# wolearyc/ramannoodle

Hardware: AMD Instinct MI355X
Metric: structures/sec (GNN polarizability eval) (higher is better)
Workload: dtype f32

## Files before the change

include/rn_potgnn.h:

```cpp
#ifndef RN_POTGNN_H
#define RN_POTGNN_H

#include <stddef.h>
#include <stdint.h>

#ifdef __cplusplus
extern "C" {
#endif

typedef enum rn_status {
  RN_OK = 0,
  RN_ERR_INVALID_ARGUMENT = -1,
  RN_ERR_UNSUPPORTED = -2,
  RN_ERR_NO_DEVICE = -3,
  RN_ERR_HIP = -4,
  RN_ERR_OUT_OF_MEMORY = -5
} rn_status;

typedef struct rn_potgnn rn_potgnn;

typedef struct rn_potgnn_config {
  int32_t num_atoms;
  int32_t num_edges;
  int32_t num_atom_types;
// ... 106 lines not shown
int rn_potgnn_gradient_buffer(rn_potgnn *h, void **device_ptr, size_t *count);
int rn_potgnn_adam_step(rn_potgnn *h, double lr, double beta1, double beta2, double eps,
                        double weight_decay, int64_t step);
int rn_potgnn_get_weights(rn_potgnn *h, float *weights, size_t num_weights);

int rn_potgnn_train_forward_f64(rn_potgnn *h, const double *positions, int64_t S, double *vec6,
                                double *batch_mean, double *batch_var);
int rn_potgnn_train_backward_f64(rn_potgnn *h, const double *dvec6, double *grads);

typedef int (*rn_potgnn_reduce_fn)(double *values, int64_t count, void *ctx);
int rn_potgnn_set_stat_reducer(rn_potgnn *h, rn_potgnn_reduce_fn fn, void *ctx);
double rn_potgnn_train_row_count(const rn_potgnn *h);


int rn_md_raman_intensities(const double *alpha, int64_t S, int device, double *intensities,
                            int64_t num_bins);
int rn_md_raman_intensities_device(const double *d_alpha, int64_t S, int device, double *intensities,
                                   int64_t num_bins, void *stream);

int rn_md_raman_polarized(const double *alpha, int64_t S, const double *weights, int64_t K, int device,
                          size_t workspace_limit, double *intensities, int64_t num_bins);
int rn_md_raman_polarized_device(const double *d_alpha, int64_t S, const double *weights, int64_t K, int device,
                                 size_t workspace_limit, double *intensities, int64_t num_bins, void *stream);

int rn_md_raman_partial(const double *increments, int64_t N, int G, const double *weights, int64_t K, int device,
                        size_t workspace_limit, double *intensities, int64_t num_bins);
int rn_md_raman_partial_device(const double *d_increments, int64_t N, int G, const double *weights, int64_t K,
                               int device, size_t workspace_limit, double *intensities, int64_t num_bins, void *stream);

int rn_md_raman_segments(const double *alpha, int64_t S, int64_t segment_steps, int64_t hop, const double *taper,
                         const double *weights, int64_t K, int average, int device, size_t workspace_limit,
                         double *intensities, int64_t num_bins);
int rn_md_raman_segments_device(const double *d_alpha, int64_t S, int64_t segment_steps, int64_t hop, const double *taper,
                                const double *weights, int64_t K, int average, int device, size_t workspace_limit,
                                double *intensities, int64_t num_bins, void *stream);

int rn_md_raman_segments_at(const double *alpha, int64_t S, int64_t segment_steps, const int64_t *starts, int64_t Q,
                            const double *taper, const double *weights, int64_t K, int average, int device,
                            size_t workspace_limit, double *intensities, int64_t num_bins);
int rn_md_raman_segments_at_device(const double *d_alpha, int64_t S, int64_t segment_steps, const int64_t *starts,
                                   int64_t Q, const double *taper, const double *weights, int64_t K, int average,
                                   int device, size_t workspace_limit, double *intensities, int64_t num_bins,
                                   void *stream);

int rn_md_raman_partial_segments(const double *increments, int64_t N, int G, int64_t segment_steps,
                                 const int64_t *starts, int64_t Q, const double *taper, const double *weights,
                                 int64_t K, int average, int device, size_t workspace_limit, double *intensities,
                                 int64_t num_bins);
int rn_md_raman_partial_segments_device(const double *d_increments, int64_t N, int G, int64_t segment_steps,
                                        const int64_t *starts, int64_t Q, const double *taper, const double *weights,
                                        int64_t K, int average, int device, size_t workspace_limit,
                                        double *intensities, int64_t num_bins, void *stream);

int rn_md_vdos(const double *positions, const double *lattices, int64_t num_lattices, int64_t S, int32_t N,
               const double *masses, const int32_t *labels, int G, int64_t segment_steps, const int64_t *starts,
               int64_t Q, const double *taper, int average, int device, size_t workspace_limit, double *densities,
               int64_t num_bins);
int rn_md_vdos_device(const double *d_positions, const double *d_lattices, int64_t num_lattices, int64_t S, int32_t N,
                      const double *masses, const int32_t *labels, int G, int64_t segment_steps, const int64_t *starts,
                      int64_t Q, const double *taper, int average, int device, size_t workspace_limit,
                      double *densities, int64_t num_bins, void *stream);
int rn_md_vdos_set_profiling(int enabled);
int rn_md_vdos_phase_times(double *millis);

int rn_md_mode_vdos(const double *positions, const double *lattices, int64_t num_lattices, int64_t S, int32_t N,
                    const double *masses, const double *vectors, int32_t M, int64_t segment_steps,
                    const int64_t *starts, int64_t Q, const double *taper, int average, int device,
                    size_t workspace_limit, double *densities, int64_t num_bins);
int rn_md_mode_vdos_device(const double *d_positions, const double *d_lattices, int64_t num_lattices, int64_t S,
                           int32_t N, const double *masses, const double *vectors, int32_t M, int64_t segment_steps,
                           const int64_t *starts, int64_t Q, const double *taper, int average, int device,
                           size_t workspace_limit, double *densities, int64_t num_bins, void *stream);
int rn_md_mode_vdos_set_profiling(int enabled);
int rn_md_mode_vdos_phase_times(double *millis);

int rn_potgnn_config_flags(const rn_potgnn *h);

int rn_potgnn_debug_ps_schedule(const int32_t *rb, const int32_t *re, int32_t num_destinations, int32_t back,
                                int32_t ring_tiles, int32_t *window);

int rn_potgnn_debug_plan(const rn_potgnn_config *cfg, const int32_t *edge_a, const int32_t *edge_b,
                         const int32_t *atom_types, int32_t num_cus, int32_t *out, size_t capacity, size_t *count);

int rn_potgnn_debug_plan_lds(const rn_potgnn_config *cfg, const int32_t *edge_a, const int32_t *edge_b,
                             const int32_t *atom_types, int32_t num_cus, int64_t *out, size_t capacity, size_t *count);

int rn_potgnn_debug_pack_weights(const rn_potgnn_config *cfg, const float *weights, size_t num_weights, float *packed,
                                 unsigned char *mask, unsigned char *writers, int32_t *flags, size_t capacity, size_t *count);

int rn_potgnn_debug_unpack_weights(const rn_potgnn_config *cfg, const float *packed, size_t num_packed, int buffers,
                                   float *out, size_t capacity, size_t *count);

int64_t rn_potgnn_num_triplets(const rn_potgnn *h);

int rn_potgnn_debug_triplets(rn_potgnn *h, int32_t *idx_i, int32_t *idx_j,
                             int32_t *idx_k, int32_t *slot5, int32_t *slot6);

int rn_potgnn_debug_stage(rn_potgnn *h, int stage, int index, float *out,
                          size_t out_capacity, int64_t *rows, int64_t *cols);

int rn_potgnn_set_profiling(rn_potgnn *h, int enabled);
int rn_potgnn_kernel_times(rn_potgnn *h, const char **names, double *millis,
                           int64_t *launches, int cap);

const char *rn_potgnn_last_error(const rn_potgnn *h);
const char *rn_potgnn_version(void);

#ifdef __cplusplus
}
#endif
#endif
```

ramannoodle_amd/_lib.py:

```python
from __future__ import annotations

import ctypes as C
import os

from ramannoodle_amd.exceptions import DeviceError

_LIB_PATH = os.environ.get(
    "RN_POTGNN_LIB", os.path.join(os.path.dirname(os.path.abspath(__file__)), "librn_potgnn.so"))

RN_OK = 0
RN_ERR_INVALID_ARGUMENT = -1
RN_ERR_UNSUPPORTED = -2
RN_ERR_NO_DEVICE = -3
RN_ERR_HIP = -4
RN_ERR_OUT_OF_MEMORY = -5


class Config(C.Structure):

    _fields_ = [
        ("num_atoms", C.c_int32),
        ("num_edges", C.c_int32),
        ("num_atom_types", C.c_int32),
        ("size_node_embedding", C.c_int32),
        ("size_edge_embedding", C.c_int32),
        ("num_message_passes", C.c_int32),
        ("gauss_coefficient", C.c_double),
        ("max_chunk_structures", C.c_int32),
        ("device", C.c_int32),
    ]


_P = C.c_void_p
SIGNATURES = {
    "rn_potgnn_radius_graph": (C.c_int, [_P, _P, C.c_int32, C.c_double, C.c_int, _P]),
    "rn_potgnn_config_flags": (C.c_int, [_P]),
    "rn_potgnn_set_stat_reducer": (C.c_int, [_P, _P, _P]),
    "rn_potgnn_train_row_count": (C.c_double, [_P]),
    "rn_potgnn_weight_count": (C.c_size_t, [C.POINTER(Config)]),
    "rn_potgnn_create": (C.c_int, [C.POINTER(Config), _P, _P, _P, _P, _P, C.c_size_t, _P, _P,
                                   C.POINTER(_P)]),
    "rn_potgnn_destroy": (None, [_P]),
    "rn_potgnn_calc_polarizabilities": (C.c_int, [_P, _P, C.c_int64, _P]),
    "rn_potgnn_calc_polarizabilities_f64": (C.c_int, [_P, _P, C.c_int64, _P]),
    "rn_potgnn_calc_polarizabilities_to_device": (C.c_int, [_P, _P, C.c_int64, _P, _P]),
    "rn_potgnn_calc_polarizabilities_cells": (C.c_int, [_P, _P, _P, C.c_int64, C.c_int, _P]),
    "rn_potgnn_calc_polarizabilities_cells_to_device": (C.c_int, [_P, _P, _P, C.c_int64, _P, _P]),
    "rn_potgnn_forward_cells_device": (C.c_int, [_P, _P, _P, C.c_int64, C.c_int, _P, _P, C.c_int]),
    "rn_potgnn_forward_device": (C.c_int, [_P, _P, C.c_int64, _P, _P, _P, C.c_int]),
    "rn_potgnn_forward_device_f64": (C.c_int, [_P, _P, C.c_int64, _P, _P, C.c_int]),
    "rn_potgnn_calc_polarizabilities_async": (C.c_int, [_P, _P, C.c_int64, _P]),
    "rn_potgnn_wait": (C.c_int, [_P]),
    "rn_host_buffer_alloc": (C.c_int, [C.c_size_t, C.c_int, C.POINTER(_P)]),
    "rn_host_buffer_free": (None, [_P]),
    "rn_potgnn_forward": (C.c_int, [_P, _P, C.c_int64, _P]),
    "rn_potgnn_forward_lattices": (C.c_int, [_P, _P, _P, C.c_int64, _P]),
    "rn_potgnn_forward_samples": (C.c_int, [_P, _P, _P, _P, C.c_int64, _P]),
    "rn_potgnn_forward_samples_f64": (C.c_int, [_P, _P, _P, _P, C.c_int64, _P]),
    "rn_potgnn_raman_tensors": (C.c_int, [_P, _P, _P, C.c_int64, C.c_double, _P]),
    "rn_potgnn_alpha_jacobian": (C.c_int, [_P, _P, C.c_int, _P]),
    "rn_potgnn_raman_tensors_analytic": (C.c_int, [_P, _P, _P, C.c_int64, _P]),
    "rn_potgnn_set_weights": (C.c_int, [_P, _P, C.c_size_t]),
    "rn_potgnn_train_forward": (C.c_int, [_P, _P, C.c_int64, _P, _P, _P]),
    "rn_potgnn_train_backward": (C.c_int, [_P, _P, _P]),
    "rn_potgnn_set_device_training": (C.c_int, [_P, C.c_int]),
    "rn_potgnn_train_backward_device": (C.c_int, [_P, _P]),
    "rn_potgnn_gradient_buffer": (C.c_int, [_P, C.POINTER(_P), C.POINTER(C.c_size_t)]),
    "rn_potgnn_adam_step": (C.c_int, [_P, C.c_double, C.c_double, C.c_double, C.c_double, C.c_double, C.c_int64]),
    "rn_potgnn_get_weights": (C.c_int, [_P, _P, C.c_size_t]),
    "rn_potgnn_train_forward_f64": (C.c_int, [_P, _P, C.c_int64, _P, _P, _P]),
    "rn_potgnn_train_forward_samples": (C.c_int, [_P, _P, _P, _P, C.c_int64, _P, _P, _P]),
    "rn_potgnn_train_forward_samples_f64": (C.c_int, [_P, _P, _P, _P, C.c_int64, _P, _P, _P]),
    "rn_potgnn_forward_samples_device": (C.c_int, [_P, _P, _P, _P, C.c_int64, _P, _P, C.c_int]),
    "rn_potgnn_train_forward_samples_device": (C.c_int, [_P, _P, _P, _P, C.c_int64, _P, _P]),
    "rn_potgnn_train_backward_samples_device": (C.c_int, [_P, _P, _P]),
    "rn_potgnn_train_backward_f64": (C.c_int, [_P, _P, _P]),
    "rn_potgnn_forward_vjp_device": (C.c_int, [_P, _P, _P, _P, C.c_int64, _P, C.c_int, _P, _P, _P]),
    "rn_potgnn_group_increments_device": (C.c_int, [_P, _P, C.c_int64, _P, C.c_int, C.c_int, C.c_size_t, _P, _P]),
    "rn_potgnn_group_increments_cells_device": (C.c_int, [_P, _P, _P, C.c_int64, _P, C.c_int, C.c_int, C.c_size_t, _P,
                                                          _P]),
    "rn_potgnn_partial_raman_tensors": (C.c_int, [_P, _P, _P, C.c_int64, _P, C.c_int, _P]),
    "rn_potgnn_train_backward_inputs": (C.c_int, [_P, _P, _P, _P, _P]),
    "rn_potgnn_train_backward_inputs_device": (C.c_int, [_P, _P, _P, _P, _P]),
    "rn_potgnn_num_triplets": (C.c_int64, [_P]),
    "rn_potgnn_debug_triplets": (C.c_int, [_P, _P, _P, _P, _P, _P]),
    "rn_potgnn_debug_ps_schedule": (C.c_int, [_P, _P, C.c_int32, C.c_int32, C.c_int32, _P]),
    "rn_potgnn_debug_plan": (C.c_int, [C.POINTER(Config), _P, _P, _P, C.c_int32, _P, C.c_size_t, C.POINTER(C.c_size_t)]),
    "rn_potgnn_debug_plan_lds": (C.c_int, [C.POINTER(Config), _P, _P, _P, C.c_int32, _P, C.c_size_t, C.POINTER(C.c_size_t)]),
    "rn_potgnn_debug_pack_weights": (C.c_int, [C.POINTER(Config), _P, C.c_size_t, _P, _P, _P, _P, C.c_size_t, C.POINTER(C.c_size_t)]),
    "rn_potgnn_debug_unpack_weights": (C.c_int, [C.POINTER(Config), _P, C.c_size_t, C.c_int, _P, C.c_size_t, C.POINTER(C.c_size_t)]),
    "rn_potgnn_debug_stage": (C.c_int, [_P, C.c_int, C.c_int, _P, C.c_size_t,
                                        C.POINTER(C.c_int64), C.POINTER(C.c_int64)]),
    "rn_potgnn_set_profiling": (C.c_int, [_P, C.c_int]),
    "rn_potgnn_kernel_times": (C.c_int, [_P, C.POINTER(C.c_char_p), C.POINTER(C.c_double),
                                         C.POINTER(C.c_int64), C.c_int]),
    "rn_potgnn_last_error": (C.c_char_p, [_P]),
    "rn_potgnn_version": (C.c_char_p, []),
    "rn_md_raman_intensities": (C.c_int, [_P, C.c_int64, C.c_int, _P, C.c_int64]),
    "rn_md_raman_intensities_device": (C.c_int, [_P, C.c_int64, C.c_int, _P, C.c_int64, _P]),
    "rn_md_raman_polarized": (C.c_int, [_P, C.c_int64, _P, C.c_int64, C.c_int, C.c_size_t, _P, C.c_int64]),
    "rn_md_raman_polarized_device": (C.c_int, [_P, C.c_int64, _P, C.c_int64, C.c_int, C.c_size_t, _P, C.c_int64,
                                               _P]),
    "rn_md_raman_partial": (C.c_int, [_P, C.c_int64, C.c_int, _P, C.c_int64, C.c_int, C.c_size_t, _P, C.c_int64]),
    "rn_md_raman_partial_device": (C.c_int, [_P, C.c_int64, C.c_int, _P, C.c_int64, C.c_int, C.c_size_t, _P,
                                             C.c_int64, _P]),
    "rn_md_raman_segments": (C.c_int, [_P, C.c_int64, C.c_int64, C.c_int64, _P, _P, C.c_int64, C.c_int, C.c_int,
                                       C.c_size_t, _P, C.c_int64]),
    "rn_md_raman_segments_device": (C.c_int, [_P, C.c_int64, C.c_int64, C.c_int64, _P, _P, C.c_int64, C.c_int, C.c_int,
                                              C.c_size_t, _P, C.c_int64, _P]),
    "rn_md_raman_segments_at": (C.c_int, [_P, C.c_int64, C.c_int64, _P, C.c_int64, _P, _P, C.c_int64, C.c_int, C.c_int,
                                          C.c_size_t, _P, C.c_int64]),
    "rn_md_raman_segments_at_device": (C.c_int, [_P, C.c_int64, C.c_int64, _P, C.c_int64, _P, _P, C.c_int64, C.c_int,
                                                 C.c_int, C.c_size_t, _P, C.c_int64, _P]),
    "rn_md_raman_partial_segments": (C.c_int, [_P, C.c_int64, C.c_int, C.c_int64, _P, C.c_int64, _P, _P, C.c_int64,
                                               C.c_int, C.c_int, C.c_size_t, _P, C.c_int64]),
    "rn_md_raman_partial_segments_device": (C.c_int, [_P, C.c_int64, C.c_int, C.c_int64, _P, C.c_int64, _P, _P,
                                                      C.c_int64, C.c_int, C.c_int, C.c_size_t, _P, C.c_int64, _P]),
    "rn_md_vdos": (C.c_int, [_P, _P, C.c_int64, C.c_int64, C.c_int32, _P, _P, C.c_int, C.c_int64, _P, C.c_int64, _P,
                             C.c_int, C.c_int, C.c_size_t, _P, C.c_int64]),
    "rn_md_vdos_device": (C.c_int, [_P, _P, C.c_int64, C.c_int64, C.c_int32, _P, _P, C.c_int, C.c_int64, _P, C.c_int64,
                                    _P, C.c_int, C.c_int, C.c_size_t, _P, C.c_int64, _P]),
    "rn_md_vdos_set_profiling": (C.c_int, [C.c_int]),
    "rn_md_vdos_phase_times": (C.c_int, [_P]),
    "rn_md_mode_vdos": (C.c_int, [_P, _P, C.c_int64, C.c_int64, C.c_int32, _P, _P, C.c_int32, C.c_int64, _P, C.c_int64,
                                  _P, C.c_int, C.c_int, C.c_size_t, _P, C.c_int64]),
    "rn_md_mode_vdos_device": (C.c_int, [_P, _P, C.c_int64, C.c_int64, C.c_int32, _P, _P, C.c_int32, C.c_int64, _P,
                                         C.c_int64, _P, C.c_int, C.c_int, C.c_size_t, _P, C.c_int64, _P]),
    "rn_md_mode_vdos_set_profiling": (C.c_int, [C.c_int]),
    "rn_md_mode_vdos_phase_times": (C.c_int, [_P]),
    "rn_xdatcar_open": (C.c_int, [C.c_char_p, C.POINTER(_P)]),
    "rn_xdatcar_close": (None, [_P]),
    "rn_xdatcar_info": (C.c_int, [_P, C.POINTER(C.c_int64), C.POINTER(C.c_int32), _P, C.POINTER(C.c_int32)]),
    "rn_xdatcar_species": (C.c_int, [_P, C.c_int32, C.c_char_p, C.POINTER(C.c_int32)]),
    "rn_xdatcar_read": (C.c_int, [_P, C.c_int64, C.c_int64, _P, _P, C.c_int]),
    "rn_xdatcar_variable_cell": (C.c_int, [_P]),
    "rn_xdatcar_read_lattices": (C.c_int, [_P, C.c_int64, C.c_int64, _P]),
    "rn_xdatcar_last_error": (C.c_char_p, [_P]),
    "rn_vasprun_open": (C.c_int, [C.c_char_p, C.POINTER(_P)]),
    "rn_vasprun_close": (None, [_P]),
    "rn_vasprun_info": (C.c_int, [_P, C.POINTER(C.c_int64), C.POINTER(C.c_int32)]),
    "rn_vasprun_read": (C.c_int, [_P, C.c_int64, C.c_int64, _P, C.c_int]),
    "rn_vasprun_timestep": (C.c_int, [_P, C.POINTER(C.c_double)]),
    "rn_vasprun_initial_num_atoms": (C.c_int64, [_P]),
    "rn_vasprun_initial_structure": (C.c_int, [_P, C.POINTER(C.c_int32), _P, _P, C.c_int64, _P, C.c_int64]),
    "rn_vasprun_last_error": (C.c_char_p, [_P]),
}

_lib = None


def library_path() -> str:
    return _LIB_PATH


def load() -> C.CDLL:
    global _lib
    if _lib is not None:
        return _lib
    if not os.path.exists(_LIB_PATH):
        raise DeviceError(
            f"{_LIB_PATH} not found: build it with ramannoodle_amd/csrc/build.sh "
            "(there is no CPU fallback for the PotGNN evaluation path)"
        )
    try:
        lib = C.CDLL(_LIB_PATH)
    except OSError as exc:
        raise DeviceError(f"cannot load {_LIB_PATH}: {exc}") from exc
    for name, (restype, argtypes) in SIGNATURES.items():
        fn = getattr(lib, name)
        fn.restype = restype
# ... 19 lines not shown
```

ramannoodle_amd/csrc/api.hip:

```cpp
#include <hip/hip_runtime.h>

#include <algorithm>
#include <chrono>
#include <cmath>
#include <cstdarg>
#include <cstdio>
#include <cstdlib>
#include <cstring>
#include <functional>
#include <memory>
#include <mutex>
#include <string>
#include <thread>
#include <vector>

#include "../../include/rn_potgnn.h"
#include "graph_plan.hpp"
#include "kernels.hpp"
#include "weight_layout.hpp"

using namespace rn;

namespace {

std::string g_create_error;

struct HipError {
  hipError_t code;
  const char *what;
};

#define HIP_TRY(expr)                                  \
  do {                                                 \
    hipError_t _e = (expr);                            \
    if (_e != hipSuccess) throw HipError{_e, #expr};   \
  } while (0)

struct DeviceBuf {
  void *p = nullptr;
  size_t bytes = 0;
  ~DeviceBuf() { release(); }
  void release() {
    if (p) (void)hipFree(p);
    p = nullptr;
    bytes = 0;
  }
  void ensure(size_t n) {
    if (n <= bytes) return;
    release();
    HIP_TRY(hipMalloc(&p, n));
    bytes = n;
  }
  template <typename T>
  T *as() const { return reinterpret_cast<T *>(p); }
};

enum KernelId {
  K_GEOM = 0, K_NODE_INIT, K_PROJ_NODE, K_PROJ_EDGE_C1, K_NODE_AGG, K_PROJ_EDGE_C3, K_PROJ_C2,
  K_EDGE_AGG, K_READOUT_MLP, K_READOUT_REDUCE, K_COUNT
};
const char *kKernelNames[K_COUNT] = {
    "geom_rbf", "node_init", "proj_node", "proj_edge_c1", "node_agg", "proj_edge_c3",
    "proj_c2", "edge_agg", "readout_mlp", "readout_reduce"};

template <typename T>
struct Lane {
  hipStream_t stream = nullptr;
  hipEvent_t done = nullptr;
  DeviceBuf unit4, node[2], edge[2], npc1, np3, bufA, bufB;
  DeviceBuf fbA, fbB;
};

template <typename T>
struct Precision {
  bool ready = false;
  DeviceBuf weights;
  DeviceBuf lattice;
  std::vector<PassW<T>> pass;
  ReadoutW<T> ro{};
  const T *offsets = nullptr, *node_table = nullptr, *ones = nullptr;
  Lane<T> lanes[2];
  std::vector<DeviceBuf> snap_node, snap_edge;
  std::vector<DeviceBuf> tape_node, tape_edge, tape_agg;
  DeviceBuf bw[18];
  hipStream_t side = nullptr;
  hipEvent_t ev_side[3] = {nullptr, nullptr, nullptr};
  DeviceBuf tn_arena;
  DeviceBuf tape_z1, bn_stats, grad, seeds, mv, type_sums;
  DeviceBuf in_dcart, in_lat, in_grads;
  DeviceBuf eye_seeds;
  int eye_frames = 0;
  bool tape_on = false;
};

struct TimedLaunch {
  int kid;
  hipEvent_t a, b;
};

}

struct rn_potgnn {
  mutable std::recursive_mutex lock;
  rn_potgnn_config cfg{};
  Dims d{};
  int chunk = 1;
  size_t f64_budget = 0;
  bool keep_stages = false;
  bool debug_sync = false;
  GraphPlan plan;
  bool split_projections = true;
  bool want_pair_rows = true;
  DeviceBuf step_seg, step_stage;
  float *step_host = nullptr;
  bool tape_ps = true;
  bool mfma_f16 = true;
  bool mfma_f16_requested = true;
  bool mfma_range_fallback = false;
  Graph g{};
  DeviceBuf g_ints;
  DeviceBuf ps_fail;
  double lattice[9], mean[9], stdv[9];
  DeviceBuf d_mean_std;
  std::vector<float> packed;
  PackedLayout lay;
  Precision<float> f32;
  Precision<double> f64;
  DeviceBuf io_pos, io_alpha, io_vec6, io_lat, io_types;
  struct Slot {
    DeviceBuf pos, alpha;
    hipEvent_t copied = nullptr, done = nullptr;
    bool busy = false;
  } slots[2];
  hipStream_t copy_stream = nullptr, exec_stream = nullptr;
  int next_slot = 0;
  struct HostStage {
    float *pin[2] = {nullptr, nullptr};
    size_t elems = 0;
    hipEvent_t copied[2] = {nullptr, nullptr};
    hipEvent_t done = nullptr;
    DeviceBuf pos;
    DeviceBuf lat;
    hipEvent_t caller = nullptr;
    char *out_pin = nullptr;
    size_t out_bytes = 0;
  } hstage;
  int last_chunk_structs = 0;
  int train_S = 0;
  int train_prec = 4;
  bool train_lat = false, train_types = false;
  bool tape_fused = true;
  bool device_training = false;
  bool grads_on_device = false;
  bool host_stale = false;
  DeviceBuf adam_m, adam_v, trainable_mask, derived_ops;
  int num_derived_ops = 0, derived_first_stage = 0;
  double bn_count = 0;
  rn_potgnn_reduce_fn reducer = nullptr;
  void *reducer_ctx = nullptr;
  bool last_was_f64 = false;
  bool last_in_order = false;
  int profiling = 0;
  std::vector<TimedLaunch> timed;
  double k_ms[K_COUNT] = {0};
  int64_t k_launches[K_COUNT] = {0};
  std::string error;
  hipEvent_t ev_start = nullptr;
  hipEvent_t ev_g[2] = {nullptr, nullptr};
  bool interleave = true;
  std::vector<int32_t> grp_labels;
  int grp_G = 0;
  DeviceBuf grp_csr, grp_jac, grp_disp, grp_out;
  DeviceBuf grp_jl, grp_lat, cells_lat;
};

namespace {

void set_error(rn_potgnn *h, const char *fmt, ...) {
  char buf[512];
  va_list ap;
  va_start(ap, fmt);
  vsnprintf(buf, sizeof(buf), fmt, ap);
  va_end(ap);
  if (h) {
    std::lock_guard<std::recursive_mutex> hold(h->lock);
    h->error = buf;
  } else {
    g_create_error = buf;
  }
}

bool lean_workspace(const rn_potgnn *h);
size_t per_structure_elems(const rn_potgnn *h, bool lean);
template <typename T>
int chunk_frames(const rn_potgnn *h) {
  if (sizeof(T) == 4) return h->chunk;
  const size_t budget = std::max(h->f64_budget, (size_t)h->chunk * per_structure_elems(h, lean_workspace(h)) * sizeof(float));
  const size_t per64 = per_structure_elems(h, false) * sizeof(double);
  return (int)std::max<size_t>(1, std::min<size_t>((size_t)h->chunk, budget / std::max<size_t>(per64, 1)));
}

template <typename T>
Precision<T> &prec(rn_potgnn *h);
template <>
Precision<float> &prec<float>(rn_potgnn *h) { return h->f32; }
template <>
Precision<double> &prec<double>(rn_potgnn *h) { return h->f64; }

void reduce_over_ranks(rn_potgnn *h, double *dev, size_t n, hipStream_t st) {
  if (!h->reducer) return;
  std::vector<double> host(n);
  HIP_TRY(hipStreamSynchronize(st));
  HIP_TRY(hipMemcpy(host.data(), dev, n * sizeof(double), hipMemcpyDeviceToHost));
  if (h->reducer(host.data(), (int64_t)n, h->reducer_ctx) != 0)
    throw HipError{hipErrorUnknown, "the statistics reducer (data-parallel training) failed"};
  HIP_TRY(hipMemcpy(dev, host.data(), n * sizeof(double), hipMemcpyHostToDevice));
}

bool lean_workspace(const rn_potgnn *h) {
  return (h->plan.use_fused && h->plan.use_node_fused && h->plan.use_readout_fused) || h->plan.use_narrow;
}
size_t bufA_width(const rn_potgnn *h, bool lean) {
  return lean ? 32 : std::max<size_t>(std::max(2 * h->d.FnP, 2 * h->d.FeP), 32);
}
size_t per_structure_elems(const rn_potgnn *h, bool lean) {
  const size_t N = h->cfg.num_atoms, E = h->cfg.num_edges;
  const size_t FnP = h->d.FnP, FeP = h->d.FeP;
  return E * 4 + 2 * N * FnP + 2 * E * FeP + N * 2 * FnP + N * 6 * FeP + E * bufA_width(h, lean) +
         (lean ? 0 : E * 4 * FeP);
}

void refresh_mfma_mode(rn_potgnn *h) {
  const bool ok = mfma_f16_range_ok(h->lay, h->packed.data(), h->host_stale);
  h->mfma_f16 = h->mfma_f16_requested && ok;
  h->mfma_range_fallback = h->mfma_f16_requested && !ok;
}

template <typename T>
void refresh_pass_flags(rn_potgnn *h) {
  Precision<T> &P = prec<T>(h);
  const bool off = getenv("RN_POTGNN_NO_FASTG") && atoi(getenv("RN_POTGNN_NO_FASTG")) != 0;
  for (size_t p = 0; p < h->lay.pass.size() && p < P.pass.size(); ++p) {
    const bool ok = !off && folded_gate_ok(h->lay, h->packed.data(), (int)p);
    P.pass[p].c3_fast = ok ? (h->plan.num_lanes == 1 ? 3 : 1) : 0;
  }
}

template <typename T>
T *stage(DeviceBuf &buf, const void *host, size_t bytes) {
  buf.ensure(bytes);
  HIP_TRY(hipMemcpy(buf.p, host, bytes, hipMemcpyHostToDevice));
  return buf.as<T>();
}

template <typename T>
T *upload_packed(rn_potgnn *h) {
  const std::vector<T> host(h->packed.begin(), h->packed.end());
  return stage<T>(prec<T>(h).weights, host.data(), host.size() * sizeof(T));
}

template <typename T>
void device_setup(rn_potgnn *h, T *w, hipStream_t st) {
  const PackedLayout &L = h->lay;
  launch_setup<T>(w + L.emb, w + L.W2, w + L.b2, w + L.W4, w + L.b4, h->cfg.num_atom_types, h->d,
                  w + L.node_table, w + L.b0, w + L.bn_w, w + L.bn_b, w + L.bn_rm, w + L.bn_rv,
                  w + L.scale0, w + L.shift0, st);
}

template <typename T>
void upload_weights(rn_potgnn *h) {
  Precision<T> &P = prec<T>(h);
  device_setup<T>(h, upload_packed<T>(h), P.lanes[0].stream);
  HIP_TRY(hipGetLastError());
  HIP_TRY(hipStreamSynchronize(P.lanes[0].stream));
  refresh_pass_flags<T>(h);
}

template <typename T>
void ensure_precision(rn_potgnn *h) {
  Precision<T> &P = prec<T>(h);
  if (P.ready) return;
  const PackedLayout &L = h->lay;
  T *w = upload_packed<T>(h);
  T lat[9];
  for (int i = 0; i < 9; ++i) lat[i] = (T)h->lattice[i];
  stage<T>(P.lattice, lat, sizeof(lat));
  WeightViews<T> v = bind_weights<T>(L, w);
  P.pass = std::move(v.pass);
  refresh_pass_flags<T>(h);
  P.ro = v.ro;
  P.offsets = v.offsets;
  P.node_table = v.node_table;
  P.ones = v.ones;

  const size_t N = h->cfg.num_atoms, E = h->cfg.num_edges, S = chunk_frames<T>(h);
  const size_t FnP = h->d.FnP, FeP = h->d.FeP;
  const bool lean = sizeof(T) == 4 && lean_workspace(h);
  const size_t bufA = bufA_width(h, lean);
  for (int l = 0; l < h->plan.num_lanes; ++l) {
    Lane<T> &ln = P.lanes[l];
    HIP_TRY(hipStreamCreateWithFlags(&ln.stream, hipStreamNonBlocking));
    HIP_TRY(hipEventCreateWithFlags(&ln.done, hipEventDisableTiming));
    ln.unit4.ensure(S * E * 4 * sizeof(T));
    for (int i = 0; i < 2; ++i) {
      ln.node[i].ensure(S * N * FnP * sizeof(T));
      ln.edge[i].ensure(S * E * FeP * sizeof(T));
    }
    ln.npc1.ensure(S * N * 2 * FnP * sizeof(T));
    ln.np3.ensure(S * N * 6 * FeP * sizeof(T));
    ln.bufA.ensure(S * E * bufA * sizeof(T));
    if (!lean) ln.bufB.ensure(S * E * 4 * FeP * sizeof(T));
  }
  if (h->keep_stages) {
    const int np = h->cfg.num_message_passes + 1;
    P.snap_node.resize(np);
    P.snap_edge.resize(np);
    for (int i = 0; i < np; ++i) {
      P.snap_node[i].ensure(S * N * FnP * sizeof(T));
      P.snap_edge[i].ensure(S * E * FeP * sizeof(T));
    }
  }
  device_setup<T>(h, w, P.lanes[0].stream);
  HIP_TRY(hipGetLastError());
  HIP_TRY(hipStreamSynchronize(P.lanes[0].stream));
  P.ready = true;
}

struct Timer {
  rn_potgnn *h;
  hipStream_t st;
  int kid;
  hipEvent_t a = nullptr, b = nullptr;
  bool on;
  Timer(rn_potgnn *h_, hipStream_t st_, int kid_) : h(h_), st(st_), kid(kid_) {
    on = h->profiling == 1 || (h->profiling >= 100 && h->profiling < 1000 && h->profiling - 100 == kid) ||
         (h->profiling >= 1000 && (((h->profiling - 1000) >> kid) & 1));
    if (on) {
      HIP_TRY(hipEventCreate(&a));
      HIP_TRY(hipEventCreate(&b));
      HIP_TRY(hipEventRecord(a, st));
    }
  }
  ~Timer() noexcept(false) {
    if (on) {
      (void)hipEventRecord(b, st);
      h->timed.push_back({kid, a, b});
    }
    if (h->debug_sync) {
      hipError_t e = hipGetLastError();
      if (e == hipSuccess) e = hipStreamSynchronize(st);
      if (e != hipSuccess) throw HipError{e, kKernelNames[kid]};
    }
  }
};

void resolve_timers(rn_potgnn *h) {
  for (auto &t : h->timed) {
    float ms = 0;
    if (hipEventSynchronize(t.b) == hipSuccess && hipEventElapsedTime(&ms, t.a, t.b) == hipSuccess) {
      h->k_ms[t.kid] += ms;
      h->k_launches[t.kid] += 1;
    }
    (void)hipEventDestroy(t.a);
    (void)hipEventDestroy(t.b);
  }
  h->timed.clear();
}

template <typename T>
struct ForwardIO {
  const double *pos = nullptr;
  const float *pos32 = nullptr;
  double *alpha = nullptr;
  float *vec6 = nullptr;
  double *alpha_raw = nullptr;
  const T *lat = nullptr;
  const int *types = nullptr;
  ForwardIO at(int64_t first, int N) const {
    auto from = [first](auto *p, int64_t stride) { return p ? p + first * stride : nullptr; };
    ForwardIO o;
    o.pos = from(pos, 3 * (int64_t)N);
    o.pos32 = from(pos32, 3 * (int64_t)N);
    o.alpha = from(alpha, 9);
    o.vec6 = from(vec6, 6);
    o.alpha_raw = from(alpha_raw, 9);
    o.lat = from(lat, 9);
    o.types = from(types, N);
    return o;
  }
};

template <typename T>
struct ChunkRun {
  rn_potgnn *h;
  Lane<T> *ln;
  ForwardIO<T> io;
  int S;
  int cur = 0;
  T *node[2], *edge[2], *unit4, *npc1, *np3, *bufA, *bufB;
  int64_t MN, ME;

  ChunkRun(rn_potgnn *h_, Lane<T> &l, const ForwardIO<T> &io_, int S_) : h(h_), ln(&l), io(io_), S(S_) {
    node[0] = l.node[0].template as<T>();
    node[1] = l.node[1].template as<T>();
    edge[0] = l.edge[0].template as<T>();
    edge[1] = l.edge[1].template as<T>();
    unit4 = l.unit4.template as<T>();
    npc1 = l.npc1.template as<T>();
    np3 = l.np3.template as<T>();
    bufA = l.bufA.template as<T>();
    bufB = l.bufB.template as<T>();
    MN = (int64_t)S * h->g.N;
    ME = (int64_t)S * h->g.E;
  }
  hipStream_t st() const { return ln->stream; }
  void target_tape(int slot, int which) {
    Precision<T> &P = prec<T>(h);
    if (!P.tape_on) return;
    node[which] = P.tape_node[slot].template as<T>();
    edge[which] = P.tape_edge[slot].template as<T>();
  }
  void snapshot(int p) {
    Precision<T> &P = prec<T>(h);
    if (!h->keep_stages) return;
    HIP_TRY(hipMemcpyAsync(P.snap_node[p].p, node[cur], (size_t)MN * h->d.FnP * sizeof(T),
                           hipMemcpyDeviceToDevice, st()));
    HIP_TRY(hipMemcpyAsync(P.snap_edge[p].p, edge[cur], (size_t)ME * h->d.FeP * sizeof(T),
                           hipMemcpyDeviceToDevice, st()));
  }

  void begin() {
    Precision<T> &P = prec<T>(h);
    target_tape(0, 0);
    {
      Timer t(h, st(), K_GEOM);
      bool done = false;
      const T *lat = io.lat ? io.lat : P.lattice.template as<T>();
      const int lat_stride = io.lat ? 9 : 0;
      const T gauss = (T)h->cfg.gauss_coefficient;
      if constexpr (sizeof(T) == 4) {
        if (io.pos32) {
          if (pair_rows()) launch_geom_rbf_pairs_pos32(io.pos32, S, h->g, lat, lat_stride, P.offsets, gauss, h->d, unit4, edge[0], st());
          else launch_geom_rbf_pos32(io.pos32, S, h->g, lat, lat_stride, P.offsets, gauss, h->d, unit4, edge[0], st(), narrow());
          done = true;
        } else if (pair_rows()) {
          launch_geom_rbf_pairs(io.pos, S, h->g, lat, lat_stride, P.offsets, gauss, h->d, unit4, edge[0], st());
          done = true;
        }
      }
      if (!done) launch_geom_rbf<T>(io.pos, S, h->g, lat, lat_stride, P.offsets, gauss, h->d, unit4, edge[0], st(), narrow());
      h->last_in_order = narrow();
    }
    {
      Timer t(h, st(), K_NODE_INIT);
      launch_node_init<T>(P.node_table, S, h->g, h->d, node[0], io.types, st());
    }
    cur = 0;
    snapshot(0);
  }

  void run_stages() {
    begin();
    for (int p = 0; p < h->cfg.num_message_passes; ++p) {
      stage_project(p);
      stage_aggregate(p);
    }
  }

  void project(const T *X, int64_t R, int K, const T *WT, int NOUT, T *Y, const T *bias, int amode, const T *nd) {
    if constexpr (sizeof(T) == 4) {
      if (h->mfma_f16 && h->split_projections &&
          launch_rowgemm_split(X, K, K, R, WT, NOUT, Y, false, bias, amode, nd, h->g, st()))
        return;
    }
    launch_rowgemm<T>(X, R, K, WT, NOUT, Y, nullptr, bias, false, amode, nd, h->g, st());
  }

  void stage_project(int p) {
    const PassW<T> &w = prec<T>(h).pass[p];
    const Graph &g = h->g;
    const Dims d = h->d;
    const int nxt = cur ^ 1;
    target_tape(p + 1, nxt);
    if constexpr (sizeof(T) == 4) {
      if (narrow()) {
        Timer t(h, st(), K_NODE_AGG);
        launch_node_narrow(edge[cur], node[cur], node[nxt], S, g, d, w, st());
        return;
      }
    }
    {
      Timer t(h, st(), K_PROJ_NODE);
      if (node_centred()) project(node[cur], MN, d.FnP, w.c1_WnT_c, 2 * d.FnP, npc1, w.c1_bias_c, 0, nullptr);
      else project(node[cur], MN, d.FnP, w.c1_WnT, 2 * d.FnP, npc1, w.c1_bias, 0, nullptr);
    }
    bool node_fused = false;
    if constexpr (sizeof(T) == 4) {
      if (fused() && h->plan.use_node_fused) {
        Timer t(h, st(), K_NODE_AGG);
        if (node_centred() && g.na_num > 0) launch_node_atom(edge[cur], node[cur], npc1, node[nxt], S, g, d, w, st(), pair_rows());
        else launch_node_fused(edge[cur], node[cur], npc1, node[nxt], S, g, d, w, h->mfma_f16, node_centred(), st());
        node_fused = true;
      }
    }
    if (!node_fused) {
      {
        Timer t(h, st(), K_PROJ_EDGE_C1);
        project(edge[cur], ME, d.FeP, w.c1_WeT, 2 * d.FnP, bufA, nullptr, 0, nullptr);
      }
      {
        Timer t(h, st(), K_NODE_AGG);
        launch_node_agg<T>(npc1, bufA, node[cur], node[nxt], S, g, d, w, st());
      }
    }
    {
      Timer t(h, st(), K_PROJ_NODE);
      if (role_split(w)) project(node[nxt], MN, d.FnP, w.c3_WnT_c, 6 * d.FeP, np3, w.c3_nshift_c, 0, nullptr);
      else project(node[nxt], MN, d.FnP, w.c3_WnT, 6 * d.FeP, np3, w.c3_nshift, 0, nullptr);
    }
    if (!fused()) {
      {
        Timer t(h, st(), K_PROJ_EDGE_C3);
        project(edge[cur], ME, d.FeP, w.c3_WeT, 4 * d.FeP, bufB, nullptr, 0, nullptr);
      }
      {
        Timer t(h, st(), K_PROJ_C2);
        project(nullptr, ME, d.FnP, w.c2_WT, 2 * d.FeP, bufA, w.c2_bias, 1, node[nxt]);
      }
    }
  }

  void stage_aggregate(int p) {
    const PassW<T> &w = prec<T>(h).pass[p];
    const int nxt = cur ^ 1;
    {
      Timer t(h, st(), K_EDGE_AGG);
      if constexpr (sizeof(T) == 4) {
        if (narrow()) launch_edge_narrow(edge[cur], edge[nxt], node[nxt], S, h->g, h->d, w, st());
        else if (role_split(w)) launch_edge_ps(edge[cur], edge[nxt], node[nxt], np3, tape_agg(p), S, h->g, h->d, w, h->ps_fail.as<int>(), st(), pair_rows(), h->mfma_f16);
        else if (fused()) edge_unfused_in_blocks(p);
        else HIP_TRY(launch_edge_agg<T>(bufB, np3, bufA, edge[cur], edge[nxt], S, h->g, h->d, w, tape_agg(p), st()));
      } else {
        HIP_TRY(launch_edge_agg<T>(bufB, np3, bufA, edge[cur], edge[nxt], S, h->g, h->d, w, tape_agg(p), st()));
      }
    }
    cur = nxt;
    snapshot(p + 1);
  }

  void edge_unfused_in_blocks(int p) {
    const PassW<T> &w = prec<T>(h).pass[p];
    const Graph &g = h->g;
    const Dims d = h->d;
    const int nxt = cur ^ 1;
    const size_t per_frame = (size_t)g.E * (size_t)(6 * d.FeP) * sizeof(T);
    int block = (int)std::max<size_t>(1, std::min<size_t>((size_t)S, ((size_t)1 << 30) / std::max<size_t>(per_frame, 1)));
    if (const char *e = getenv("RN_POTGNN_UNFUSED_BLOCK_FRAMES")) block = std::max(1, std::min(block, atoi(e)));
    ln->fbA.ensure((size_t)block * g.E * 2 * d.FeP * sizeof(T));
    ln->fbB.ensure((size_t)block * g.E * 4 * d.FeP * sizeof(T));
    T *fa = ln->fbA.template as<T>(), *fb = ln->fbB.template as<T>();
    T *agg = tape_agg(p);
    for (int s0 = 0; s0 < S; s0 += block) {
      const int sb = std::min(block, S - s0);
      const int64_t rows = (int64_t)sb * g.E;
      const T *e_in = edge[cur] + (size_t)s0 * g.E * d.FeP, *nd = node[nxt] + (size_t)s0 * g.N * d.FnP;
      project(e_in, rows, d.FeP, w.c3_WeT, 4 * d.FeP, fb, nullptr, 0, nullptr);
      project(nullptr, rows, d.FnP, w.c2_WT, 2 * d.FeP, fa, w.c2_bias, 1, nd);
      HIP_TRY(launch_edge_agg<T>(fb, np3 + (size_t)s0 * g.N * 6 * d.FeP, fa, e_in, edge[nxt] + (size_t)s0 * g.E * d.FeP, sb, g, d, w,
                                 agg ? agg + (size_t)s0 * g.E * d.FeP : nullptr, st()));
    }
  }

  void finish() {
    Precision<T> &P = prec<T>(h);
    const Graph &g = h->g;
    const Dims d = h->d;
    if constexpr (sizeof(T) == 4) {
      if (narrow()) {
        Timer t(h, st(), K_READOUT_MLP);
        const double *ms = h->d_mean_std.as<double>();
        launch_readout_narrow(edge[cur], unit4, S, g, d, P.ro, ms, ms + 9, io.vec6, io.alpha, io.alpha_raw,
                              h->keep_stages ? bufA : nullptr, st());
        HIP_TRY(hipGetLastError());
        return;
      }
    }
    int pol_stride = 32;
    {
      Timer t(h, st(), K_READOUT_MLP);
      const int HP = std::max(d.FeP, 32);
      bool done = false;
      if constexpr (sizeof(T) == 4) {
        if (fused() && h->plan.use_readout_fused) {
          pol_stride = h->keep_stages ? 32 : 16;
          launch_readout_fused(edge[cur], ME, P.ro, bufA, h->mfma_f16, st(), pair_rows(), pol_stride);
          done = true;
        }
      }
      if (!done) {
        launch_rowgemm<T>(edge[cur], ME, d.FeP, P.ro.W0T, HP, bufA, P.ro.scale0, P.ro.shift0, true, 0,
                          nullptr, g, st());
        launch_rowgemm<T>(bufA, ME, HP, P.ro.W3T, HP, bufB, P.ones, P.ro.b3, true, 0, nullptr, g, st());
        launch_rowgemm<T>(bufB, ME, HP, P.ro.W5T, 32, bufA, nullptr, P.ro.b5, false, 0, nullptr, g,
                          st());
      }
    }
    {
      Timer t(h, st(), K_READOUT_REDUCE);
      const double *ms = h->d_mean_std.as<double>();
      launch_readout_reduce<T>(bufA, unit4, S, g, ms, ms + 9, io.vec6, io.alpha, io.alpha_raw, st(), pol_stride);
    }
    HIP_TRY(hipGetLastError());
  }
  bool fused() const { return sizeof(T) == 4 && h->plan.use_fused && (!prec<T>(h).tape_on || h->tape_fused); }
  bool narrow() const { return sizeof(T) == 4 && h->plan.use_narrow && !prec<T>(h).tape_on; }
  bool node_centred() const {
    static const bool on = !(getenv("RN_POTGNN_NODE_CENTRED") && atoi(getenv("RN_POTGNN_NODE_CENTRED")) == 0);
    return sizeof(T) == 4 && on && fused() && h->plan.use_node_fused && h->mfma_f16 && (!prec<T>(h).tape_on || h->tape_ps);
  }
  bool role_split(const PassW<T> &w) const {
    return sizeof(T) == 4 && fused() && h->plan.use_ps && (w.c3_fast & 1) != 0 && (!prec<T>(h).tape_on || h->tape_ps);
  }
  bool pair_rows() const {
    if (sizeof(T) != 4 || !h->want_pair_rows || h->keep_stages || prec<T>(h).tape_on || !node_centred() || h->g.na_num <= 0 || !h->plan.use_readout_fused) return false;
    for (const auto &w : prec<T>(h).pass)
      if (!role_split(w)) return false;
    return true;
  }
  T *tape_agg(int p) {
    Precision<T> &P = prec<T>(h);
    return P.tape_on ? P.tape_agg[p].template as<T>() : nullptr;
  }
};

template <typename T>
void run_chunk(ChunkRun<T> c) {
  c.run_stages();
  c.finish();
}

template <typename T>
void run_pair(rn_potgnn *h, ChunkRun<T> &a, ChunkRun<T> &b) {
  const int P = h->cfg.num_message_passes;
  a.begin();
  b.begin();
  for (int p = 0; p < P; ++p) {
    if (p > 0) HIP_TRY(hipStreamWaitEvent(a.st(), h->ev_g[1], 0));
    a.stage_project(p);
    HIP_TRY(hipEventRecord(h->ev_g[0], a.st()));
    a.stage_aggregate(p);
    HIP_TRY(hipStreamWaitEvent(b.st(), h->ev_g[0], 0));
    b.stage_project(p);
    HIP_TRY(hipEventRecord(h->ev_g[1], b.st()));
    b.stage_aggregate(p);
  }
  a.finish();
  b.finish();
}

void check_ps_fail(rn_potgnn *h) {
  if (!h->plan.use_ps || !h->ps_fail.p) return;
  int fail = 0;
  HIP_TRY(hipMemcpy(&fail, h->ps_fail.p, sizeof(int), hipMemcpyDeviceToHost));
#ifdef RN_PS_TIMING
  {
    long long t[40];
    HIP_TRY(hipMemcpy(t, (const char *)h->ps_fail.p + 64, sizeof(t), hipMemcpyDeviceToHost));
    HIP_TRY(hipMemset((char *)h->ps_fail.p + 64, 0, sizeof(t)));
    static const char *names[20] = {"P sched+dma_wait", "P loads+split", "P split sync", "P seeds", "P request", "P guard",
                                    "P P'+c2", "P Q' (product, loads landed + finish)", "P norm sync+publish", "P ring guard", "C ready wait", "C prologue", "C loop",
                                    "C epilogue+done", "", "", "C(set B) ready wait", "C(set B) prologue", "C(set B) loop", "C(set B) epilogue+done"};
    for (int i = 0; i < 20; ++i)
      if (t[2 * i + 1]) fprintf(stderr, "[ps timing] %-22s %10.1f cycles x %lld\n", names[i], (double)t[2 * i] / (double)t[2 * i + 1], t[2 * i + 1]);
  }
#endif
#ifdef RN_PS_GRAM_DEBUG
  {
    int cnt = 0;
    HIP_TRY(hipMemcpy(&cnt, (const char *)h->ps_fail.p + 127 * 4, sizeof(int), hipMemcpyDeviceToHost));
    float dbg[144];
    HIP_TRY(hipMemcpy(dbg, (const char *)h->ps_fail.p + 128 * 4, sizeof(dbg), hipMemcpyDeviceToHost));
    fprintf(stderr, "[gram debug] %d mismatches\n", cnt);
    for (int k = 0; k < std::min(cnt, 12); ++k)
      fprintf(stderr, "  ref %g tab %g parts %g %g %g %g  d %g er %g tl %g urow %g r %g gr %g\n", dbg[12 * k], dbg[12 * k + 1], dbg[12 * k + 2],
              dbg[12 * k + 3], dbg[12 * k + 4], dbg[12 * k + 5], dbg[12 * k + 6], dbg[12 * k + 7], dbg[12 * k + 8], dbg[12 * k + 9],
              dbg[12 * k + 10], dbg[12 * k + 11]);
    HIP_TRY(hipMemset((char *)h->ps_fail.p + 127 * 4, 0, 4 + sizeof(dbg)));
  }
#endif
  if (fail == 0) return;
  HIP_TRY(hipMemset(h->ps_fail.p, 0, sizeof(int)));
  static const char *const which[7] = {
      "role-specialised EdgeBlock: a wait between producer and consumer waves timed out",
      "role-specialised EdgeBlock: the producers' split sync timed out",
      "role-specialised EdgeBlock: a producer's wait for the consumers to take the rows of an earlier round timed out",
      "role-specialised EdgeBlock: a producer's wait for the consumers to finish an earlier round (ring rows) timed out",
      "role-specialised EdgeBlock: a consumer's wait for its round timed out",
      "role-specialised EdgeBlock: a wait between producer and consumer waves timed out",
      "role-specialised EdgeBlock: a consumer's round-ordered wait before releasing its ring rows (c_rd) timed out"};
  throw HipError{hipErrorLaunchFailure, which[fail >= 0 && fail <= 6 ? fail : 0]};
}

template <typename T>
void behind_caller(rn_potgnn *h, hipStream_t user, Lane<T> *lanes, int n) {
  HIP_TRY(hipEventRecord(h->ev_start, user));
  for (int l = 0; l < n; ++l) HIP_TRY(hipStreamWaitEvent(lanes[l].stream, h->ev_start, 0));
}
template <typename T>
void hand_back(rn_potgnn *h, hipStream_t user, Lane<T> *lanes, int n, bool sync, bool timers = false) {
  for (int l = 0; l < n; ++l) {
    HIP_TRY(hipEventRecord(lanes[l].done, lanes[l].stream));
    HIP_TRY(hipStreamWaitEvent(user, lanes[l].done, 0));
  }
  if (!sync) return;
  HIP_TRY(hipStreamSynchronize(user));
  if (timers) resolve_timers(h);
  check_ps_fail(h);
}

template <typename T>
void forward_device(rn_potgnn *h, const ForwardIO<T> &io, int64_t S, hipStream_t user, bool sync) {
  ensure_precision<T>(h);
  Precision<T> &P = prec<T>(h);
  const int N = h->cfg.num_atoms;
  const int lanes = h->plan.num_lanes;
  behind_caller(h, user, P.lanes, lanes);
  auto make = [&](int lane, int64_t first, int s) { return ChunkRun<T>(h, P.lanes[lane], io.at(first, N), s); };
  int64_t done = 0;
  const int capacity = chunk_frames<T>(h);
  const int64_t pieces = (S + capacity - 1) / capacity;
  const int chunk = (int)std::max<int64_t>(1, std::min<int64_t>(capacity, (S + pieces - 1) / std::max<int64_t>(pieces, 1)));
  h->train_S = 0;
  while (done < S) {
    const int64_t left = S - done;
    if (lanes == 2 && h->interleave && !h->keep_stages && left > 1) {
      const int64_t both = std::min<int64_t>(left, 2 * (int64_t)chunk);
      const int sa = (int)((both + 1) / 2), sb = (int)(both - sa);
      ChunkRun<T> a = make(0, done, sa), b = make(1, done + sa, sb);
      run_pair<T>(h, a, b);
      h->last_chunk_structs = sa;
      done += both;
    } else {
      const int s = (int)std::min<int64_t>(chunk, left);
      run_chunk(make(0, done, s));
      h->last_chunk_structs = s;
      done += s;
    }
  }
  h->last_was_f64 = sizeof(T) == 8;
  hand_back(h, user, P.lanes, lanes, sync, true);
}

template <typename T>
struct Reverse {
  int S, B;
  const T *d_dout6;
  double *d_dpos;
  T *grad;
  bool train_bn;
  double *in_dpos = nullptr;
  double *in_dlat = nullptr;
};

enum { DE0, DE1, DN0, DN1, DNX, DPQ, DNP3, DC2, DPROD, DBC1, DNPC1, DPOL, DUNIT, DH, POL, DOUT, DPROD2, BWN };

template <typename T>
void reverse_pass(rn_potgnn *h, ChunkRun<T> &c, const Reverse<T> &rv) {
  Precision<T> &P = prec<T>(h);
  const PackedLayout &L = h->lay;
  const Graph &g = h->g;
  const Dims d = h->d;
  const int N = g.N, E = g.E, NP = h->cfg.num_message_passes;
  const int S = rv.S, B = rv.B, C = S * B;
  const int HP = std::max(d.FeP, 32);
  hipStream_t st = c.st();
  const size_t ce = (size_t)C * E, cn = (size_t)C * N, fe = (size_t)S * E, fn = (size_t)S * N;
  const size_t sizes[BWN] = {ce * d.FeP, ce * d.FeP, cn * d.FnP, cn * d.FnP, cn * d.FnP,
                             ce * 4 * d.FeP, cn * 6 * d.FeP, ce * std::max(2 * d.FeP, HP), ce * d.FnP,
                             ce * 2 * d.FnP, cn * 2 * d.FnP, ce * 32, ce * 4, ce * HP, fe * 32,
                             (size_t)C * 6, rv.grad ? fe * d.FnP : 0};
  T *b[BWN];
  for (int i = 0; i < BWN; ++i) {
    P.bw[i].ensure(sizes[i] * sizeof(T));
    b[i] = P.bw[i].template as<T>();
  }
  T *bufA = c.bufA, *bufB = c.bufB, *unit4 = c.unit4;
  T *G = rv.grad;
  T *Wd = P.weights.template as<T>();
  const bool split_gemm = sizeof(T) == 4 && h->mfma_f16;
  auto back_gemm = [&](const T *dY, int64_t R, int N, size_t w_off, size_t t_off, int K, T *dX,
                       bool accumulate) {
    if constexpr (sizeof(T) == 4) {
      if (split_gemm && launch_rowgemm_split(dY, N, N, R, Wd + t_off, K, dX, accumulate, nullptr, 0, nullptr, g, st)) return;
      if (launch_rowgemm_blocks(dY, N, N, R, Wd + t_off, K, dX, accumulate, g, st)) return;
    }
    launch_gemm_nt<T>(dY, R, N, Wd + w_off, N, K, dX, accumulate, st);
  };
  auto project = [&](const T *X, int64_t R, int K, const T *WT, int NOUT, T *Y, const T *bias, int amode, const T *node) {
    if constexpr (sizeof(T) == 4) {
      if (split_gemm && launch_rowgemm_split(X, K, K, R, WT, NOUT, Y, false, bias, amode, node, g, st)) return;
    }
    launch_rowgemm<T>(X, R, K, WT, NOUT, Y, nullptr, bias, false, amode, node, g, st);
  };

  TnDeferred tn_store, *tn = nullptr;
  if constexpr (sizeof(T) == 4) {
    static const bool tn_atomic = getenv("RN_POTGNN_TN_ATOMIC") && atoi(getenv("RN_POTGNN_TN_ATOMIC")) != 0;
    if (G && !tn_atomic) {
      size_t need = tn_partial_elems(ce, HP, 32) + tn_partial_elems(ce, HP, HP) + tn_partial_elems(ce, d.FeP, HP);
      const size_t per_pass = tn_partial_elems(ce, d.FeP, 4 * d.FeP) + tn_partial_elems(cn, d.FnP, 6 * d.FeP) +
                              tn_partial_elems(ce, d.FnP, 2 * d.FeP) + tn_partial_elems(ce, d.FeP, 2 * d.FnP) +
                              tn_partial_elems(cn, d.FnP, 2 * d.FnP);
      need += per_pass * (size_t)NP;
      P.tn_arena.ensure(need * sizeof(float));
      tn_store.arena = P.tn_arena.template as<float>();
      tn_store.capacity = need;
      tn = &tn_store;
    }
// ... 626 lines not shown

enum TrainKind { kHostF32, kHostF64, kDeviceF32 };

Checked check_train_batch(rn_potgnn *h, int64_t S, std::initializer_list<const void *> needed, const char *name,
                          TrainKind kind) {
  const bool f64 = kind == kHostF64, device = kind == kDeviceF32;
  bool ok = h && S > 0;
  for (const void *p : needed) ok = ok && p;
  if (!ok) {
    set_error(h, "invalid arguments to %s", name);
    return {RN_ERR_INVALID_ARGUMENT, {}};
  }
  Checked c{kGo, std::unique_lock<std::recursive_mutex>(h->lock)};
  if (device && !h->device_training) {
    set_error(h, "%s needs device-resident training (rn_potgnn_set_device_training)", name);
    c.rc = RN_ERR_INVALID_ARGUMENT;
  } else if (f64 && S > chunk_frames<double>(h)) {
    set_error(h, "training batch of %lld frames exceeds the float64 chunk of %d frames", (long long)S, chunk_frames<double>(h));
    c.rc = RN_ERR_INVALID_ARGUMENT;
  } else if (!f64 && S > h->chunk) {
    set_error(h, "training batch of %lld frames exceeds max_chunk_structures = %d", (long long)S, h->chunk);
    c.rc = RN_ERR_INVALID_ARGUMENT;
  }
  return c;
}

Checked check_pending(rn_potgnn *h, bool args_ok, const char *name, TrainKind kind, const char *text) {
  const int prec_bytes = kind == kHostF64 ? 8 : 4;
  const bool device = kind == kDeviceF32;
  if (!h || !args_ok) {
    set_error(h, "invalid arguments to %s", name);
    return {RN_ERR_INVALID_ARGUMENT, {}};
  }
  Checked c{kGo, std::unique_lock<std::recursive_mutex>(h->lock)};
  if ((device && !h->device_training) || h->train_S <= 0 || h->train_prec != prec_bytes) c.rc = refuse(h, text);
  return c;
}

void lazy_stream(hipStream_t &s) {
  if (!s) HIP_TRY(hipStreamCreateWithFlags(&s, hipStreamNonBlocking));
}
void lazy_event(hipEvent_t &e) {
  if (!e) HIP_TRY(hipEventCreateWithFlags(&e, hipEventDisableTiming));
}

template <typename F>
void with_precision(rn_potgnn *h, bool use_float64, F fn) {
  if (use_float64) {
    sync_host(h);
    fn(double{});
  } else {
    fn(float{});
  }
}
}

extern "C" {

const char *rn_potgnn_version(void) { return "ramannoodle_amd-potgnn 0.1 (gfx950)"; }

size_t rn_potgnn_weight_count(const rn_potgnn_config *c) {
  try {
    return state_dict_count(c);
  } catch (const std::exception &) {
    return 0;
  }
}

const char *rn_potgnn_last_error(const rn_potgnn *h) {
  return h ? h->error.c_str() : g_create_error.c_str();
}

static Graph upload(const GraphPlan &plan, DeviceBuf &buf) {
  std::vector<int> ints;
  auto push = [&](const std::vector<int> &v) {
    size_t o = ints.size();
    ints.insert(ints.end(), v.begin(), v.end());
    while (ints.size() % 4) ints.push_back(0);
    return o;
  };
  const size_t o_a = push(plan.edge_a), o_b = push(plan.edge_b), o_op = push(plan.out_ptr),
               o_ip = push(plan.in_ptr), o_ie = push(plan.in_edge), o_at = push(plan.atom_type),
               o_tb = push(plan.tile.begin), o_to = push(plan.trip_off), o_rv = push(plan.rev_edge),
               o_nt = push(plan.nt.begin), o_bt = push(plan.bt.begin), o_pt = push(plan.pt.begin), o_ipos = push(plan.in_pos);
  buf.ensure(ints.size() * sizeof(int));
  HIP_TRY(hipMemcpy(buf.p, ints.data(), ints.size() * sizeof(int), hipMemcpyHostToDevice));
  const int *base = buf.as<int>();
  Graph g = plan.scalars();
  g.edge_a = base + o_a;
  g.edge_b = base + o_b;
  g.out_ptr = base + o_op;
  g.in_ptr = base + o_ip;
  g.in_edge = base + o_ie;
  g.in_pos = base + o_ipos;
  g.atom_type = base + o_at;
  g.rev_edge = base + o_rv;
  g.tile_begin = base + o_tb;
  g.trip_off = base + o_to;
  g.nt_begin = base + o_nt;
  g.pt_begin = base + o_pt;
  g.bt_begin = base + o_bt;
  return g;
}

static void size_chunk(rn_potgnn *h) {
  int chunk = h->cfg.max_chunk_structures;
  if (const char *e = getenv("RN_POTGNN_CHUNK")) chunk = atoi(e);
  if (chunk <= 0) {
    const size_t per = per_structure_elems(h, lean_workspace(h)) * sizeof(float);
    size_t budget = (h->plan.use_fused || h->plan.use_narrow) ? ((size_t)8192 << 20) : ((size_t)1536 << 20);
    size_t free_b = 0, total_b = 0;
    if (hipMemGetInfo(&free_b, &total_b) == hipSuccess && free_b > 0)
      budget = std::min(budget, std::max<size_t>(free_b / 8 / (size_t)h->plan.num_lanes, (size_t)64 << 20));
    chunk = (int)std::max<size_t>(1, budget / std::max<size_t>(per, 1));
    chunk = std::min(chunk, 4096);
    h->f64_budget = (size_t)24 << 30;
    if (free_b > 0) h->f64_budget = std::min(h->f64_budget, std::max<size_t>(free_b / 8 / (size_t)h->plan.num_lanes, (size_t)64 << 20));
  }
  h->chunk = chunk;
}

int rn_potgnn_create(const rn_potgnn_config *cfg, const int32_t *edge_a, const int32_t *edge_b,
                     const int32_t *atom_types, const double *lattice, const float *weights,
                     size_t num_weights, const double *mean, const double *stddev,
                     rn_potgnn **out) {
  if (!out) return RN_ERR_INVALID_ARGUMENT;
  *out = nullptr;
  std::string invalid;
  int rc = validate_create_args(cfg, edge_a, edge_b, atom_types, !lattice || !weights || !mean || !stddev, &num_weights, invalid);
  if (rc != RN_OK) {
    set_error(nullptr, "%s", invalid.c_str());
    return rc;
  }

  int ndev = 0;
  if (hipGetDeviceCount(&ndev) != hipSuccess || ndev <= 0 || cfg->device < 0 ||
      cfg->device >= ndev) {
    set_error(nullptr, "no usable HIP device (count=%d, requested=%d)", ndev, cfg->device);
    return RN_ERR_NO_DEVICE;
  }
  int cus = 256;
  {
    hipDeviceProp_t prop;
    if (hipGetDeviceProperties(&prop, cfg->device) == hipSuccess && prop.multiProcessorCount > 0) cus = prop.multiProcessorCount;
  }

  std::unique_ptr<rn_potgnn> h(new rn_potgnn());
  h->cfg = *cfg;
  std::memcpy(h->lattice, lattice, sizeof(h->lattice));
  std::memcpy(h->mean, mean, sizeof(h->mean));
  std::memcpy(h->stdv, stddev, sizeof(h->stdv));
  h->keep_stages = getenv("RN_POTGNN_KEEP_STAGES") && atoi(getenv("RN_POTGNN_KEEP_STAGES")) != 0;
  h->debug_sync = getenv("RN_POTGNN_DEBUG_SYNC") && atoi(getenv("RN_POTGNN_DEBUG_SYNC")) != 0;
  if (const char *e = getenv("RN_POTGNN_INTERLEAVE")) h->interleave = atoi(e) != 0;
  if (const char *e = getenv("RN_POTGNN_MFMA")) h->mfma_f16_requested = !(e[0] == 'f' && e[1] == '3');
  h->mfma_f16 = h->mfma_f16_requested;
  if (const char *e = getenv("RN_POTGNN_TAPE_FUSED")) h->tape_fused = atoi(e) != 0;
  if (const char *e = getenv("RN_POTGNN_TAPE_PS")) h->tape_ps = atoi(e) != 0;
  h->split_projections = getenv("RN_POTGNN_SPLIT_PROJ") ? atoi(getenv("RN_POTGNN_SPLIT_PROJ")) != 0 : true;
  h->want_pair_rows = !(getenv("RN_POTGNN_PAIR_ROWS") && atoi(getenv("RN_POTGNN_PAIR_ROWS")) == 0);

  const PlanKnobs knobs = read_plan_knobs();
  h->d = plan_dims(*cfg, knobs);
  h->plan = plan_graph(*cfg, h->d, edge_a, edge_b, atom_types, cus, knobs);

  rn_potgnn *hp = h.get();
  rc = guarded(nullptr, [&]() {
    HIP_TRY(hipSetDevice(cfg->device));
    HIP_TRY(hipEventCreateWithFlags(&hp->ev_start, hipEventDisableTiming));
    HIP_TRY(hipEventCreateWithFlags(&hp->ev_g[0], hipEventDisableTiming));
    HIP_TRY(hipEventCreateWithFlags(&hp->ev_g[1], hipEventDisableTiming));
    hp->g = upload(hp->plan, hp->g_ints);
    double ms[18];
    std::memcpy(ms, hp->mean, sizeof(hp->mean));
    std::memcpy(ms + 9, hp->stdv, sizeof(hp->stdv));
    hp->d_mean_std.ensure(sizeof(ms));
    HIP_TRY(hipMemcpy(hp->d_mean_std.p, ms, sizeof(ms), hipMemcpyHostToDevice));
    hp->lay = layout_weights(hp->cfg, hp->d);
    pack_weights(hp->lay, weights, hp->packed);
    refresh_mfma_mode(hp);
    hp->ps_fail.ensure(2048);
    HIP_TRY(hipMemset(hp->ps_fail.p, 0, 2048));
    size_chunk(hp);
    ensure_precision<float>(hp);
  });
  if (rc != RN_OK) return rc;
  *out = h.release();
  return RN_OK;
}

int rn_potgnn_debug_plan(const rn_potgnn_config *cfg, const int32_t *edge_a, const int32_t *edge_b,
                         const int32_t *atom_types, int32_t num_cus, int32_t *out, size_t capacity, size_t *count) {
  if (!count || num_cus <= 0) return RN_ERR_INVALID_ARGUMENT;
  *count = 0;
  std::string invalid;
  const int rc = validate_create_args(cfg, edge_a, edge_b, atom_types, false, nullptr, invalid);
  if (rc != RN_OK) {
    set_error(nullptr, "%s", invalid.c_str());
    return rc;
  }
  try {
    const PlanKnobs knobs = read_plan_knobs();
    const std::vector<int32_t> flat = plan_graph(*cfg, plan_dims(*cfg, knobs), edge_a, edge_b, atom_types, num_cus, knobs).flat();
    *count = flat.size();
    if (!out || capacity < flat.size()) {
      set_error(nullptr, "out holds %zu values, the plan has %zu", out ? capacity : (size_t)0, flat.size());
      return RN_ERR_INVALID_ARGUMENT;
    }
    std::memcpy(out, flat.data(), flat.size() * sizeof(int32_t));
    return RN_OK;
  } catch (const std::bad_alloc &) {
    set_error(nullptr, "host allocation failed");
    return RN_ERR_OUT_OF_MEMORY;
  }
}

int rn_potgnn_debug_plan_lds(const rn_potgnn_config *cfg, const int32_t *edge_a, const int32_t *edge_b,
                             const int32_t *atom_types, int32_t num_cus, int64_t *out, size_t capacity, size_t *count) {
  if (!count || num_cus <= 0) return RN_ERR_INVALID_ARGUMENT;
  *count = 0;
  std::string invalid;
  const int rc = validate_create_args(cfg, edge_a, edge_b, atom_types, false, nullptr, invalid);
  if (rc != RN_OK) {
    set_error(nullptr, "%s", invalid.c_str());
    return rc;
  }
  try {
    const PlanKnobs knobs = read_plan_knobs();
    const std::vector<int64_t> lds = plan_graph(*cfg, plan_dims(*cfg, knobs), edge_a, edge_b, atom_types, num_cus, knobs).lds_requests();
    *count = lds.size();
    if (!out || capacity < lds.size()) {
      set_error(nullptr, "out holds %zu values, the table has %zu", out ? capacity : (size_t)0, lds.size());
      return RN_ERR_INVALID_ARGUMENT;
    }
    std::memcpy(out, lds.data(), lds.size() * sizeof(int64_t));
    return RN_OK;
  } catch (const std::bad_alloc &) {
    set_error(nullptr, "host allocation failed");
    return RN_ERR_OUT_OF_MEMORY;
  }
}

static int debug_layout(const rn_potgnn_config *cfg, bool others_null, const size_t *num_weights, PackedLayout &L) {
  std::string invalid;
  const int rc = validate_config(cfg, others_null, num_weights, invalid);
  if (rc != RN_OK) {
    set_error(nullptr, "%s", invalid.c_str());
    return rc;
  }
  L = layout_weights(*cfg, plan_dims(*cfg, read_plan_knobs()));
  return RN_OK;
}
static int debug_failed(const std::exception &e) {
  const bool memory = dynamic_cast<const std::bad_alloc *>(&e) != nullptr;
  set_error(nullptr, memory ? "host allocation failed" : "internal error: %s", e.what());
  return memory ? RN_ERR_OUT_OF_MEMORY : RN_ERR_HIP;
}

int rn_potgnn_debug_pack_weights(const rn_potgnn_config *cfg, const float *weights, size_t num_weights, float *packed,
                                 unsigned char *mask, unsigned char *writers, int32_t *flags, size_t capacity, size_t *count) {
  if (!count) return RN_ERR_INVALID_ARGUMENT;
  *count = 0;
  try {
    PackedLayout L;
    if (const int rc = debug_layout(cfg, !weights, &num_weights, L); rc != RN_OK) return rc;
    *count = L.total;
    if (!packed || !mask || !flags || capacity < L.total) {
      set_error(nullptr, "out holds %zu values, the packed blob has %zu", packed && mask && flags ? capacity : (size_t)0, L.total);
      return RN_ERR_INVALID_ARGUMENT;
    }
    std::vector<float> o;
    pack_weights(L, weights, o);
    std::memcpy(packed, o.data(), o.size() * sizeof(float));
    const std::vector<unsigned char> m = trainable_mask(L);
    std::memcpy(mask, m.data(), m.size());
    if (writers) {
      const std::vector<unsigned char> w = packed_writers(L);
      std::memcpy(writers, w.data(), w.size());
    }
    flags[0] = mfma_f16_range_ok(L, o.data(), false);
    for (int p = 0; p < L.P; ++p) {
      flags[1 + p] = folded_gate_ok(L, o.data(), p);
      (void)L.c3_norm_1(p), (void)L.mfma_scales(p);
    }
    (void)L.readout();
    return RN_OK;
  } catch (const std::exception &e) {
    return debug_failed(e);
  }
// ... 769 lines not shown
    h->host_stale = true;
    refresh_pass_flags<float>(h);
    refresh_mfma_mode(h);
    check_ps_fail(h);
  });
}

int rn_potgnn_get_weights(rn_potgnn *h, float *weights, size_t num_weights) {
  if (!h || !weights || num_weights != h->lay.weight_count()) {
    set_error(h, "invalid arguments to get_weights");
    return RN_ERR_INVALID_ARGUMENT;
  }
  return guarded(h, [&]() {
    sync_host(h);
    unpack_weights<float>(h->lay, h->packed.data(), weights, true);
  });
}

int rn_potgnn_set_stat_reducer(rn_potgnn *h, rn_potgnn_reduce_fn fn, void *ctx) {
  if (!h) return RN_ERR_INVALID_ARGUMENT;
  std::lock_guard<std::recursive_mutex> hold(h->lock);
  h->reducer = fn;
  h->reducer_ctx = ctx;
  return RN_OK;
}

double rn_potgnn_train_row_count(const rn_potgnn *h) {
  if (!h) return 0.0;
  std::lock_guard<std::recursive_mutex> hold(h->lock);
  return h->bn_count;
}

int rn_potgnn_train_backward(rn_potgnn *h, const float *dvec6, float *grads) {
  const Checked c = check_pending(h, dvec6 && grads, "train_backward", kHostF32,
                                  "train_backward needs a preceding train_forward (an evaluation or Jacobian call in "
                                  "between discards its tape)");
  if (c.rc != kGo) return c.rc;
  return guarded(h, [&]() { train_backward<float>(h, dvec6, grads); });
}

int rn_potgnn_radius_graph(const double *lattice, const double *positions, int32_t num_atoms,
                           double cutoff, int device, uint8_t *adjacency) {
  if (!lattice || !positions || !adjacency || num_atoms <= 0 || !(cutoff > 0)) {
    set_error(nullptr, "invalid arguments to radius_graph");
    return RN_ERR_INVALID_ARGUMENT;
  }
  int ndev = 0;
  if (hipGetDeviceCount(&ndev) != hipSuccess || device < 0 || device >= ndev) {
    set_error(nullptr, "no usable HIP device (count=%d, requested=%d)", ndev, device);
    return RN_ERR_NO_DEVICE;
  }
  return guarded(nullptr, [&]() {
    HIP_TRY(hipSetDevice(device));
    const size_t n = (size_t)num_atoms;
    DeviceBuf lat, pos, adj;
    lat.ensure(9 * sizeof(double));
    pos.ensure(n * 3 * sizeof(double));
    adj.ensure(n * n);
    HIP_TRY(hipMemcpy(lat.p, lattice, 9 * sizeof(double), hipMemcpyHostToDevice));
    HIP_TRY(hipMemcpy(pos.p, positions, n * 3 * sizeof(double), hipMemcpyHostToDevice));
    launch_radius_graph(lat.as<double>(), pos.as<double>(), num_atoms, (float)cutoff,
                        adj.as<unsigned char>(), nullptr);
    HIP_TRY(hipGetLastError());
    HIP_TRY(hipDeviceSynchronize());
    HIP_TRY(hipMemcpy(adjacency, adj.p, n * n, hipMemcpyDeviceToHost));
  });
}

int rn_potgnn_config_flags(const rn_potgnn *h) {
  if (!h) return -1;
  std::lock_guard<std::recursive_mutex> hold(h->lock);
  int flags = (h->plan.use_fused ? 1 : 0) | ((h->plan.use_fused && h->mfma_f16) ? 4 : 0) | (h->plan.use_narrow ? 8 : 0) |
              ((h->plan.use_fused && h->mfma_range_fallback) ? 16 : 0);
  {
    bool ps = h->plan.use_fused && h->plan.use_ps && !h->f32.pass.empty();
    for (const auto &p : h->f32.pass) ps = ps && (p.c3_fast & 1);
    flags |= ps ? 256 : 0;
  }
  {
    static const bool centred = !(getenv("RN_POTGNN_NODE_CENTRED") && atoi(getenv("RN_POTGNN_NODE_CENTRED")) == 0);
    const bool atom = h->plan.use_fused && h->plan.use_node_fused && h->mfma_f16 && centred && h->g.na_num > 0;
    flags |= atom ? 512 : 0;
    flags |= (atom && (flags & 256) && h->plan.use_readout_fused && h->want_pair_rows && !h->keep_stages) ? 1024 : 0;
  }
  bool fast = !h->f32.pass.empty();
  for (const auto &p : h->f32.pass) fast = fast && !h->plan.use_narrow && (p.c3_fast & (h->plan.use_fused ? 1 : 2));
  return flags | (fast ? 2 : 0);
}

int rn_potgnn_debug_ps_schedule(const int32_t *rb, const int32_t *re, int32_t num_destinations, int32_t back, int32_t ring_tiles,
                                int32_t *window) {
  if (!rb || !re || num_destinations < 0 || back < 1 || back > 8 || ring_tiles < 1 || ring_tiles > 64) return RN_ERR_INVALID_ARGUMENT;
  int w = 0;
  const bool ok = edge_ps_tile_ok(rb, re, num_destinations, back, ring_tiles, &w);
  if (window) *window = w;
  return ok ? 1 : 0;
}

int64_t rn_potgnn_num_triplets(const rn_potgnn *h) { return h ? h->g.T : -1; }

int rn_potgnn_debug_triplets(rn_potgnn *h, int32_t *idx_i, int32_t *idx_j, int32_t *idx_k,
                             int32_t *slot5, int32_t *slot6) {
  if (!h || !idx_i || !idx_j || !idx_k || !slot5 || !slot6) return RN_ERR_INVALID_ARGUMENT;
  return guarded(h, [&]() {
    const size_t T = (size_t)h->g.T;
    if (T == 0) return;
    DeviceBuf buf;
    buf.ensure(5 * T * sizeof(int));
    int *p = buf.as<int>();
    launch_enum_triplets(h->g, p, p + T, p + 2 * T, p + 3 * T, p + 4 * T, nullptr);
    HIP_TRY(hipGetLastError());
    HIP_TRY(hipDeviceSynchronize());
    int32_t *outs[5] = {idx_i, idx_j, idx_k, slot5, slot6};
    for (int k = 0; k < 5; ++k)
      HIP_TRY(hipMemcpy(outs[k], p + k * T, T * sizeof(int), hipMemcpyDeviceToHost));
  });
}

int rn_potgnn_debug_stage(rn_potgnn *h, int stage, int index, float *out, size_t out_capacity,
                          int64_t *rows, int64_t *cols) {
  if (!h || !out || !rows || !cols) return RN_ERR_INVALID_ARGUMENT;
  std::lock_guard<std::recursive_mutex> hold(h->lock);
  if (h->last_was_f64) {
    set_error(h, "debug_stage only reads the float32 path");
    return RN_ERR_UNSUPPORTED;
  }
  const int S = h->last_chunk_structs;
  Precision<float> &P = h->f32;
  return guarded(h, [&]() {
    HIP_TRY(hipDeviceSynchronize());
    const float *src = nullptr;
    int64_t r = 0, c = 0, ld = 0;
    const int64_t ME = (int64_t)S * h->g.E, MN = (int64_t)S * h->g.N;
    if (stage == 0) {
      src = P.lanes[0].unit4.as<float>(); r = ME; c = 4; ld = 4;
    } else if (stage == 1 || stage == 2) {
      if (!h->keep_stages || index < 0 || index > h->cfg.num_message_passes)
        throw HipError{hipErrorInvalidValue, "stage snapshots need RN_POTGNN_KEEP_STAGES=1"};
      if (stage == 1) { src = P.snap_node[index].as<float>(); r = MN; c = h->d.Fn; ld = h->d.FnP; }
      else { src = P.snap_edge[index].as<float>(); r = ME; c = h->d.Fe; ld = h->d.FeP; }
    } else if (stage == 3) {
      src = P.lanes[0].bufA.as<float>(); r = ME; c = 12; ld = 32;
    } else {
      throw HipError{hipErrorInvalidValue, "unknown stage"};
    }
    if ((size_t)(r * c) > out_capacity) throw HipError{hipErrorInvalidValue, "out_capacity too small"};
    HIP_TRY(hipMemcpy2D(out, c * sizeof(float), src, ld * sizeof(float), c * sizeof(float), r,
                        hipMemcpyDeviceToHost));
    if (h->last_in_order && r == ME && stage != 1) {
      std::vector<float> tmp(out, out + r * c);
      const int E = h->g.E;
      for (int64_t s = 0; s < S; ++s)
        for (int e = 0; e < E; ++e)
          std::memcpy(out + (s * E + e) * c, tmp.data() + (s * E + h->plan.in_pos[e]) * c, (size_t)c * sizeof(float));
    }
    *rows = r;
    *cols = c;
  });
}

int rn_potgnn_set_profiling(rn_potgnn *h, int enabled) {
  if (!h) return RN_ERR_INVALID_ARGUMENT;
  std::lock_guard<std::recursive_mutex> hold(h->lock);
  resolve_timers(h);
  h->profiling = enabled;
  for (int k = 0; k < K_COUNT; ++k) {
    h->k_ms[k] = 0;
    h->k_launches[k] = 0;
  }
  return RN_OK;
}

int rn_potgnn_kernel_times(rn_potgnn *h, const char **names, double *millis, int64_t *launches,
                           int cap) {
  if (!h || !names || !millis || !launches) return RN_ERR_INVALID_ARGUMENT;
  std::lock_guard<std::recursive_mutex> hold(h->lock);
  (void)hipSetDevice(h->cfg.device);
  resolve_timers(h);
  int n = 0;
  for (int k = 0; k < K_COUNT && n < cap; ++k, ++n) {
    names[n] = kKernelNames[k];
    millis[n] = h->k_ms[k];
    launches[n] = h->k_launches[k];
  }
  return n;
}

}
```

ramannoodle_amd/csrc/graph_plan.hip:

```cpp
#include "graph_plan.hpp"

#include <algorithm>
#include <cstdarg>
#include <cstdio>
#include <cstdlib>

namespace rn {

namespace {

std::string format(const char *fmt, ...) {
  char buf[512];
  va_list ap;
  va_start(ap, fmt);
  vsnprintf(buf, sizeof(buf), fmt, ap);
  va_end(ap);
  return buf;
}

const char *knob(const char *name) { return getenv(name); }
bool knob_flag(const char *name, bool otherwise) { return knob(name) ? atoi(knob(name)) != 0 : otherwise; }

void widen_for_fused(Dims &d, int widen) {
  if (widen == 0) return;
// ... 163 lines not shown
      bool ok = true;
      for (int t = 0; t < ntiles && ok; ++t) {
        const int eo0 = g.out_ptr[p.begin[t]];
        rb.clear();
        re.clear();
        int longest = 0;
        for (int i = g.in_ptr[p.begin[t]]; i < g.in_ptr[p.begin[t + 1]]; ++i) {
          const int bd = g.edge_b[g.in_edge[i]];
          rb.push_back(g.out_ptr[bd] - eo0);
          re.push_back(g.out_ptr[bd + 1] - eo0);
          longest = std::max(longest, re.back() - rb.back());
        }
        int window = 0;
        ok = edge_ps_tile_ok(rb.data(), re.data(), (int)rb.size(), v.back, edge_ps_ring_tiles(v.gram), &window);
        if (v.gram) ok = ok && window <= edge_ps_gram_window() && longest <= 32;
      }
      if (!ok || edge_ps_lds_bytes(p.max_out_rows, p.max_in_rows, v.gram) > (size_t)160 * 1024) continue;
      const int max_rounds = std::max(1, (p.max_in_rows + 15) / 16);
      const double groups = ntiles <= cus ? (double)(cus / ntiles) : 1.0 / (double)((ntiles + cus - 1) / cus);
      const double cost = (double)max_rounds / groups * v.factor;
      if (chosen.begin.empty() || cost < best * 0.999) {
        best = cost;
        chosen = p;
        *pt_back = v.back;
        *pt_gram = v.gram ? 1 : 0;
      }
      break;
    }
    if (p.max_out_rows >= g.E) break;
  }
  return chosen;
}

void choose_node_atom(GraphPlan &g, const PlanKnobs &k) {
  const int N = g.N;
  int max_deg = 0;
  long rounds_atom = 0, rounds_row = 0;
  for (int n0 = 0; n0 < N; n0 += 16) {
    int m = 0;
    for (int n = n0; n < std::min(N, n0 + 16); ++n) m = std::max(m, g.in_ptr[n + 1] - g.in_ptr[n]);
    rounds_atom += m;
    max_deg = std::max(max_deg, m);
  }
  for (int t = 0; t < g.nt.num(); ++t) rounds_row += (g.in_ptr[g.nt.begin[t + 1]] - g.in_ptr[g.nt.begin[t]] + 15) / 16;
  bool ok = !g.nt_narrow && g.d.FnP == 64 && g.d.FeP == 64 && node_atom_lds_bytes(max_deg) <= (size_t)40 * 1024 &&
            (double)rounds_atom <= 1.2 * (double)rounds_row;
  if (k.node_atom >= 0) ok = k.node_atom != 0 && g.d.FnP == 64 && g.d.FeP == 64 && node_atom_lds_bytes(max_deg) <= (size_t)64 * 1024;
  g.na_num = ok ? (N + 15) / 16 : 0;
  g.na_max_deg = max_deg;
}

void build_index_arrays(GraphPlan &g) {
  const int N = g.N, E = g.E;
  const int *edge_a = g.edge_a.data(), *edge_b = g.edge_b.data();
  g.out_ptr.assign(N + 1, 0);
  g.in_ptr.assign(N + 1, 0);
  for (int e = 0; e < E; ++e) {
    g.out_ptr[edge_a[e] + 1]++;
    g.in_ptr[edge_b[e] + 1]++;
  }
  for (int n = 0; n < N; ++n) {
    g.out_ptr[n + 1] += g.out_ptr[n];
    g.in_ptr[n + 1] += g.in_ptr[n];
  }
  g.in_edge.assign(E, 0);
  {
    std::vector<int> fill(g.in_ptr.begin(), g.in_ptr.end() - 1);
    for (int e = 0; e < E; ++e) g.in_edge[fill[edge_b[e]]++] = e;
  }
  g.in_pos.assign(E, 0);
  for (int i = 0; i < E; ++i) g.in_pos[g.in_edge[i]] = i;
  g.trip_off.assign(E + 1, 0);
  g.rev_edge.assign(E, -1);
  for (int e = 0; e < E; ++e) {
    const int bd = edge_b[e], ad = edge_a[e];
    int cnt = 0;
    for (int o = g.out_ptr[bd]; o < g.out_ptr[bd + 1]; ++o) cnt += edge_b[o] != ad;
    g.trip_off[e + 1] = g.trip_off[e] + cnt;
    const int *lo = edge_b + g.out_ptr[bd], *hi = edge_b + g.out_ptr[bd + 1];
    const int *it = std::lower_bound(lo, hi, ad);
    if (it != hi && *it == ad) g.rev_edge[e] = (int)(it - edge_b);
  }
  g.T = g.trip_off[E];
}

}

PlanKnobs read_plan_knobs() {
  PlanKnobs k;
  static const int widen = knob("RN_POTGNN_WIDEN") ? atoi(knob("RN_POTGNN_WIDEN")) : 2;
  k.widen = widen;
  k.vpl8 = knob("RN_POTGNN_VPL") && atoi(knob("RN_POTGNN_VPL")) == 8;
  k.want_fused = knob_flag("RN_POTGNN_FUSED", true);
  k.want_narrow = knob_flag("RN_POTGNN_NARROW", true);
  if (const char *e = knob("RN_POTGNN_TILE_KB")) k.tile_kb_set = true, k.tile_kb = atoi(e);
  if (const char *e = knob("RN_POTGNN_NARROW_TILE_ROWS")) k.narrow_tile_rows = std::max(1, atoi(e));
  k.bwd_tiles = knob_flag("RN_POTGNN_BWD_TILES", true);
  if (const char *e = knob("RN_POTGNN_NODE_TILE_ROWS")) k.node_tile_rows_set = true, k.node_tile_rows = atoi(e);
  if (const char *e = knob("RN_POTGNN_NODE_TILE_KB")) k.node_tile_kb = std::max(1, atoi(e));
  k.want_ps = knob_flag("RN_POTGNN_EDGE_PS", true);
  if (const char *e = knob("RN_POTGNN_PS_TILE_ROWS")) k.ps_tile_rows = atoi(e);
  if (const char *e = knob("RN_POTGNN_PS_BACK")) k.ps_back = atoi(e);
  k.want_gram = knob_flag("RN_POTGNN_PS_GRAM", false);
  if (const char *e = knob("RN_POTGNN_NODE_ATOM")) k.node_atom = atoi(e) != 0;
  k.want_node_fused = knob_flag("RN_POTGNN_NODE_FUSED", true);
  k.want_readout_fused = knob_flag("RN_POTGNN_READOUT_FUSED", true);
  if (const char *e = knob("RN_POTGNN_LANES")) k.lanes = std::max(1, std::min(2, atoi(e)));
  return k;
}

int pad_pow2(int f) {
  int p = 16;
  while (p < f) p *= 2;
  return p;
}

Dims plan_dims(const rn_potgnn_config &cfg, const PlanKnobs &knobs) {
  Dims d = {cfg.size_node_embedding, cfg.size_edge_embedding, pad_pow2(cfg.size_node_embedding),
            pad_pow2(cfg.size_edge_embedding)};
  widen_for_fused(d, knobs.widen);
  return d;
}

size_t max_out_degree(Dims d) {
  size_t deg = 0;
  while (edge_agg_f64_lds_bytes(d, (int)deg + 1, (int)deg + 1, 1) <= kCuLdsBytes) ++deg;
  return deg;
}

int validate_config(const rn_potgnn_config *cfg_in, bool others_null, const size_t *num_weights, std::string &error) {
  if (!cfg_in || others_null) {
    error = "null argument";
    return RN_ERR_INVALID_ARGUMENT;
  }
  const rn_potgnn_config &cfg = *cfg_in;
  const int N = cfg.num_atoms, E = cfg.num_edges;
  if (N <= 0 || E < 0 || cfg.num_atom_types <= 0 || cfg.size_node_embedding <= 0 ||
      cfg.size_edge_embedding <= 0 || cfg.num_message_passes <= 0) {
    error = "invalid configuration (non-positive size)";
    return RN_ERR_INVALID_ARGUMENT;
  }
  if (E == 0) {
    error = "reference graph has no edges: the per-structure mean over edges "
            "(_gnn.py:662-664) is undefined";
    return RN_ERR_INVALID_ARGUMENT;
  }
  if (cfg.size_node_embedding > 128 || cfg.size_edge_embedding > 128) {
    error = format("embedding sizes above 128 are not supported (Fn=%d, Fe=%d)", cfg.size_node_embedding,
                   cfg.size_edge_embedding);
    return RN_ERR_UNSUPPORTED;
  }
  if (num_weights && *num_weights != rn_potgnn_weight_count(&cfg)) {
    error = format("weights has %zu floats, expected %zu", *num_weights, rn_potgnn_weight_count(&cfg));
    return RN_ERR_INVALID_ARGUMENT;
  }
  return RN_OK;
}

int validate_create_args(const rn_potgnn_config *cfg_in, const int32_t *edge_a, const int32_t *edge_b, const int32_t *atom_types,
                         bool others_null, const size_t *num_weights, std::string &error) {
  const bool graph_null = !atom_types || (cfg_in && cfg_in->num_edges > 0 && (!edge_a || !edge_b));
  if (const int rc = validate_config(cfg_in, others_null || graph_null, num_weights, error); rc != RN_OK) return rc;
  const rn_potgnn_config &cfg = *cfg_in;
  const int N = cfg.num_atoms, E = cfg.num_edges;
  for (int e = 0; e < E; ++e) {
    if (edge_a[e] < 0 || edge_a[e] >= N || edge_b[e] < 0 || edge_b[e] >= N || edge_a[e] == edge_b[e]) {
      error = format("edge %d = (%d,%d) is out of range or a self loop", e, edge_a[e], edge_b[e]);
      return RN_ERR_INVALID_ARGUMENT;
    }
    if (e > 0 && (edge_a[e] < edge_a[e - 1] || (edge_a[e] == edge_a[e - 1] && edge_b[e] <= edge_b[e - 1]))) {
      error = format("edges must be strictly sorted by (a, b); violated at edge %d", e);
      return RN_ERR_INVALID_ARGUMENT;
    }
  }
  for (int n = 0; n < N; ++n)
    if (atom_types[n] < 0 || atom_types[n] >= cfg.num_atom_types) {
      error = format("atom %d has type %d outside [0,%d)", n, atom_types[n], cfg.num_atom_types);
      return RN_ERR_INVALID_ARGUMENT;
    }
  const Dims d = plan_dims(cfg, read_plan_knobs());
  const size_t cap = max_out_degree(d);
  std::vector<int> deg(N, 0), deg_in(N, 0);
  for (int e = 0; e < E; ++e) deg[edge_a[e]]++, deg_in[edge_b[e]]++;
  for (int n = 0; n < N; ++n)
    if ((size_t)deg[n] > cap) {
      error = format("atom %d has %d outgoing edges; more than %zu per atom is unsupported "
                     "for size_edge_embedding=%d", n, deg[n], cap, cfg.size_edge_embedding);
      return RN_ERR_UNSUPPORTED;
    }
  const int max_out = *std::max_element(deg.begin(), deg.end()), max_in = *std::max_element(deg_in.begin(), deg_in.end());
  const size_t need = edge_agg_f64_lds_bytes(d, max_out, max_in, 1);
  if (need > kCuLdsBytes) {
    error = format("an atom with %d outgoing edges beside one with %d incoming edges needs %zu bytes of LDS per tile in "
                   "float64 (%zu available) for size_edge_embedding=%d", max_out, max_in, need, kCuLdsBytes, cfg.size_edge_embedding);
    return RN_ERR_UNSUPPORTED;
  }
  return RN_OK;
}

GraphPlan plan_graph(const rn_potgnn_config &cfg, Dims d, const int32_t *edge_a, const int32_t *edge_b,
                     const int32_t *atom_types, int num_cus, const PlanKnobs &k) {
  GraphPlan g;
  g.N = cfg.num_atoms;
  g.E = cfg.num_edges;
  g.d = d;
  g.edge_a.assign(edge_a, edge_a + g.E);
  g.edge_b.assign(edge_b, edge_b + g.E);
  g.atom_type.assign(atom_types, atom_types + g.N);
  build_index_arrays(g);

  const bool fused_mode = k.want_fused && d.FnP == 64 && d.FeP == 64;
  const bool narrow_mode = k.want_narrow && narrow_supported(d);
  g.tile = edge_tiles(g, k, fused_mode, narrow_mode);
  if (edge_agg_f64_lds_bytes(d, g.tile.max_out_rows, g.tile.max_in_rows, g.tile.max_nodes) > kCuLdsBytes) g.tile = one_atom_tiles(g);
  if (k.bwd_tiles) g.bt = reverse_tiles(g);
  if (narrow_mode) g.nt = node_tiles_narrow(g, k);
  g.nt_narrow = g.nt.num() > 0;
  if (!g.nt_narrow) g.nt = node_tiles_wide(g, k);
  if (fused_mode && k.want_ps) g.pt = ps_tiles(g, k, num_cus, &g.pt_back, &g.pt_gram);
  choose_node_atom(g, k);

  const Graph s = g.scalars();
  g.use_fused = k.want_fused && edge_fused_supported(s, d);
  g.use_ps = g.use_fused && g.pt.num() > 0;
  g.use_narrow = narrow_mode && edge_narrow_lds_bytes(d.Fn, d.Fe, g.tile.max_out_rows, g.tile.max_in_rows) <= (size_t)64 * 1024;
  g.use_node_fused = g.use_fused && k.want_node_fused && node_fused_lds_bytes(s) <= 64 * 1024;
  g.use_readout_fused = g.use_fused && k.want_readout_fused;
  g.num_lanes = k.lanes > 0 ? k.lanes : ((g.use_fused || g.use_narrow) ? 1 : 2);
  return g;
}

Graph GraphPlan::scalars() const {
  Graph s{};
  s.N = N, s.E = E, s.T = T;
  s.num_tiles = tile.num(), s.max_tile_out_rows = tile.max_out_rows, s.max_tile_in_rows = tile.max_in_rows, s.max_tile_nodes = tile.max_nodes;
  s.nt_num = nt.num(), s.nt_max_in_rows = nt.max_in_rows, s.nt_max_nodes = nt.max_nodes, s.nt_narrow = nt_narrow ? 1 : 0;
  s.na_num = na_num, s.na_max_deg = na_max_deg;
  s.pt_num = pt.num(), s.pt_max_out_rows = pt.max_out_rows, s.pt_max_in_rows = pt.max_in_rows, s.pt_back = pt_back, s.pt_gram = pt_gram;
  s.bt_num = bt.num(), s.bt_max_out_rows = bt.max_out_rows, s.bt_max_in_rows = bt.max_in_rows, s.bt_max_nodes = bt.max_nodes;
  return s;
}

std::vector<int64_t> GraphPlan::lds_requests() const {
  const Graph s = scalars();
  const bool node_fused = use_fused && use_node_fused;
  std::vector<int64_t> o;
  auto add = [&o](size_t f32, size_t f64) { o.insert(o.end(), {(int64_t)f32, (int64_t)f64}); };
  add(edge_agg_lds_bytes(s, d, sizeof(float)), edge_agg_lds_bytes(s, d, sizeof(double)));
  add(edge_bwd_lds_bytes(s, d.FeP, sizeof(float)), edge_bwd_lds_bytes(s, d.FeP, sizeof(double)));
  add(use_narrow ? edge_narrow_lds_bytes(d.Fn, d.Fe, tile.max_out_rows, tile.max_in_rows) : 0, 0);
  add(use_narrow && nt_narrow ? node_tiled_lds_bytes(d.Fn, d.Fe, nt.max_in_rows, nt.max_nodes) : 0, 0);
  add(use_ps ? edge_ps_lds_bytes(pt.max_out_rows, pt.max_in_rows, pt_gram != 0) : 0, 0);
  add(node_fused && na_num > 0 ? node_atom_lds_bytes(na_max_deg) : 0, 0);
  add(node_fused ? node_fused_lds_bytes(s) : 0, 0);
  return o;
}

std::vector<int32_t> GraphPlan::flat() const {
  std::vector<int32_t> o = {d.FnP, d.FeP};
  const Partition reserved;
  for (const Partition *p : {&tile, &nt, &reserved, &bt, &pt}) {
    o.push_back((int32_t)p->begin.size());
    o.insert(o.end(), p->begin.begin(), p->begin.end());
    o.insert(o.end(), {p->max_out_rows, p->max_in_rows, p->max_nodes});
  }
  o.insert(o.end(), {nt_narrow ? 1 : 0, na_num, na_max_deg, pt_back, pt_gram, (int32_t)T});
  o.insert(o.end(), {use_fused, 0 , 0 , use_ps, use_narrow, use_node_fused, use_readout_fused, num_lanes});
  for (const std::vector<int> *v : {&out_ptr, &in_ptr, &in_edge, &in_pos, &rev_edge, &trip_off}) o.insert(o.end(), v->begin(), v->end());
  return o;
}

}
```

ramannoodle_amd/csrc/graph_plan.hpp:

```cpp
#pragma once

#include <string>
#include <vector>

#include "../../include/rn_potgnn.h"
#include "kernels.hpp"

namespace rn {

struct PlanKnobs {
  int widen = 2;
  bool vpl8 = false;
  bool want_fused = true;
  bool want_narrow = true;
  bool tile_kb_set = false;
  int tile_kb = 64;
  int narrow_tile_rows = 0;
  bool bwd_tiles = true;
  bool node_tile_rows_set = false;
  int node_tile_rows = 0;
  int node_tile_kb = 12;
  bool want_ps = true;
  int ps_tile_rows = 0;
  int ps_back = 5;
  bool want_gram = false;
  int node_atom = -1;
  bool want_node_fused = true;
  bool want_readout_fused = true;
  int lanes = 0;
};
PlanKnobs read_plan_knobs();

int pad_pow2(int f);
Dims plan_dims(const rn_potgnn_config &cfg, const PlanKnobs &knobs);
size_t max_out_degree(Dims d);

int validate_config(const rn_potgnn_config *cfg, bool others_null, const size_t *num_weights, std::string &error);
int validate_create_args(const rn_potgnn_config *cfg, const int32_t *edge_a, const int32_t *edge_b, const int32_t *atom_types,
                         bool others_null, const size_t *num_weights, std::string &error);

struct Partition {
  std::vector<int> begin;
  int max_out_rows = 0, max_in_rows = 0, max_nodes = 0;
  int num() const { return begin.empty() ? 0 : (int)begin.size() - 1; }
};

struct GraphPlan {
  int N = 0, E = 0;
  Dims d{};
  std::vector<int> edge_a, edge_b, atom_type;
  std::vector<int> out_ptr, in_ptr;
  std::vector<int> in_edge, in_pos;
  std::vector<int> rev_edge;
  std::vector<int> trip_off;
  int64_t T = 0;
  Partition tile, nt, bt, pt;
  bool nt_narrow = false;
  int na_num = 0, na_max_deg = 0;
  int pt_back = 2, pt_gram = 0;
  bool use_fused = false;
  bool use_ps = false;
  bool use_narrow = false;
  bool use_node_fused = false;
  bool use_readout_fused = false;
  int num_lanes = 2;

  Graph scalars() const;
  std::vector<int64_t> lds_requests() const;
  std::vector<int32_t> flat() const;
};

GraphPlan plan_graph(const rn_potgnn_config &cfg, Dims d, const int32_t *edge_a, const int32_t *edge_b,
                     const int32_t *atom_types, int num_cus, const PlanKnobs &knobs);

}
```

ramannoodle_amd/csrc/kernels.hpp:

```cpp
#pragma once
#include <hip/hip_runtime.h>
#include <algorithm>
#include <cstddef>
#include <cstdint>

namespace rn {

struct Graph {
  int N, E;
  const int *edge_a;
  const int *edge_b;
  const int *out_ptr;
  const int *in_ptr;
  const int *in_edge;
  const int *in_pos;
  const int *atom_type;
  const int *rev_edge;
  int num_tiles;
  const int *tile_begin;
  int max_tile_out_rows;
  int max_tile_in_rows;
  int max_tile_nodes;
  int nt_num;
  const int *nt_begin;
  int nt_max_in_rows, nt_max_nodes;
  int nt_narrow;
  int na_num;
  int na_max_deg;
  int pt_num;
  const int *pt_begin;
  int pt_max_out_rows, pt_max_in_rows;
  int pt_back;
  int pt_gram;
  int bt_num;
  const int *bt_begin;
  int bt_max_out_rows, bt_max_in_rows, bt_max_nodes;
  const int *trip_off;
  int64_t T;
};

template <typename T>
struct Ln {
  const T *g, *b;
};

template <typename T>
struct PassW {
  const T *c1_WnT;
  const T *c1_WeT;
  const T *c1_bias;
  Ln<T> c1_norm;
  Ln<T> final_norm;
  const T *c2_WT;
  const T *c2_bias;
  Ln<T> c2_norm_1;
  Ln<T> c2_norm_2;
  const T *c3_WnT;
  const T *c3_nshift;
  const T *c3_WeT;
  Ln<T> c3_norm_1;
  Ln<T> c3_norm_2;
  Ln<T> c3_norm_1s;
  Ln<T> c2_norm_1s;
  Ln<T> c1_norm_s;
  const T *mfma_scale;
  const T *c3_WeT_c;
  const T *c3_WnT_c;
  const T *c3_nshift_c;
  const T *c2_WT_c;
  const T *c2_bias_c;
  const T *c1_WnT_c;
  const T *c1_WeT_c;
  const T *c1_bias_c;
  const T *mfma_scale_c;
  int c3_fast;
};

template <typename T>
struct ReadoutW {
  const T *W0T;
  const T *scale0, *shift0;
  const T *W3T;
  const T *b3;
  const T *W5T;
  const T *b5;
  const T *mfma_scale;
};

__host__ __device__ inline float mfma_prescale(float m) {
  union { float f; unsigned u; } b;
  b.f = m;
  const unsigned ex = (b.u >> 23) & 0xffu;
  if (!(m > 0.0f) || ex == 0xffu) return 1.0f;
  int e = (int)ex - 127;
  if (e < -126) e = -126;
  int se = 12 - e;
  se = se < -126 ? -126 : (se > 126 ? 126 : se);
  b.u = (unsigned)(se + 127) << 23;
  return b.f;
}
// ... 79 lines not shown
void launch_prod_fwd(const T *node, T *prod, int64_t rows, const Graph &g, Dims d, hipStream_t st);
template <typename T>
void launch_prod_bwd(const T *dprod, const T *node, T *dnode, int C, int B, const Graph &g, Dims d,
                     hipStream_t st);
template <typename T>
void launch_node_bwd(const T *npc1, const T *bc1, const T *node_next, const T *dnode_next,
                     T *dnode_prev, T *dbc1, T *dnpc1, int C, int B, const Graph &g, Dims d,
                     const PassW<T> &w, const PassW<T> *grad_w, hipStream_t st);
struct TnReduceOp {
  const float *part;
  float *dst, *dbias;
  int nblk, K, N, ldw;
};
struct TnReduceTable {
  static constexpr int MAX_OPS = 32;
  TnReduceOp ops[MAX_OPS];
  int wg_begin[MAX_OPS + 1];
  int num;
};
struct TnDeferred {
  float *arena = nullptr;
  size_t capacity = 0, used = 0;
  TnReduceTable table{};
};
size_t tn_partial_elems(int64_t R, int K, int N);
void launch_tn_reduce(TnDeferred &df, hipStream_t st);
template <typename T>
void launch_gemm_tn(const T *X, int ldx, const T *dY, int ldy, int64_t R, int K, int N, T *dWT,
                    int ldw, T *dbias, int amode, const T *node, const Graph &g, hipStream_t st,
                    TnDeferred *defer = nullptr);
template <typename T>
void launch_bn_col_sums(const T *z, int64_t R, int W, double *stats, hipStream_t st);
template <typename T>
void launch_bn_train_apply(const T *z, int64_t R, int W, int F, const double *stats, double count,
                           const T *gamma, const T *beta, T *h, T *mv, hipStream_t st);
template <typename T>
void launch_bn_bwd_sums(const T *d, const T *z, int64_t R, int W, int F, const double *stats, double count,
                        double *sums, hipStream_t st);
template <typename T>
void launch_bn_bwd_apply(T *d, const T *z, int64_t R, int W, int F, const double *stats, double count,
                         const double *sums, const double *own_sums, const T *gamma, T *dgamma, T *dbeta,
                         hipStream_t st);
template <typename T>
void launch_node_embed_bwd(const T *dnode0, int S, const Graph &g, Dims d, int K, const T *emb,
                           const T *W2, const T *b2, const T *W4, T *demb, T *dW2, T *db2, T *dW4,
                           T *db4, T *type_sums_scratch,
                           const int *types , hipStream_t st);
template <typename T>
void launch_geom_bwd(const T *dedge0, const T *dunit, const T *unit4, const T *lat, const T *offs,
                     T coef, int C, int B, const Graph &g, Dims d, double *dpos, hipStream_t st);
template <typename T>
void launch_geom_input_bwd(const T *dedge0, const T *dunit, const T *unit4, const double *pos, const T *lat,
                           int lat_stride, const T *offs, T coef, int C, int B, const Graph &g, Dims d, double *dcart,
                           double *dpos, double *dlat, hipStream_t st);
template <typename T>
void launch_cast_from_f64(const double *src, T *dst, int64_t n, hipStream_t st);
constexpr int kMaxGroups = 16;

void launch_group_increments(const double *jac, int64_t jac_stride, const double *pos, const double *disp,
                             double disp_scale, int64_t steps, int N, const int *perm, const int *gptr, int G,
                             const double *sigma, double *out, hipStream_t st, int out_groups = 0);
void launch_cell_increments(const double *jl, const double *lat, int64_t steps, int channel, int out_groups,
                            const double *sigma, double *out, hipStream_t st);

constexpr size_t kFusedLdsBudget = 80 * 1024;
size_t edge_fused_lds_bytes(const Graph &g);
size_t edge_fused_lds_bytes(int tile_out_rows, int tile_in_rows, int tile_nodes);
bool edge_fused_supported(const Graph &g, Dims d);
size_t node_fused_lds_bytes(const Graph &g);
size_t node_fused_lds_bytes(int tile_in_rows, int tile_nodes);
void launch_readout_fused(const float *edge, int64_t M, const ReadoutW<float> &w, float *pol, bool f16,
                          hipStream_t st, bool pair_rows = false, int pol_stride = 32 );
size_t node_atom_lds_bytes(int max_deg);
void launch_node_atom(const float *edge, const float *node_in, const float *npc1, float *node_out, int S, const Graph &g,
                      Dims d, const PassW<float> &w, hipStream_t st, bool pair_rows = false);
void launch_node_fused(const float *edge, const float *node_in, const float *npc1, float *node_out, int S,
                       const Graph &g, Dims d, const PassW<float> &w, bool f16, bool centred, hipStream_t st);
size_t edge_ps_lds_bytes(int tile_out_rows, int tile_in_rows, bool gram);
int edge_ps_ring_tiles(bool gram);
int edge_ps_gram_window();
bool edge_ps_tile_ok(const int *rb, const int *re, int D, int back, int ring, int *window);
void launch_edge_ps(const float *edge_in, float *edge_out, const float *node, const float *np3, float *agg_out, int S,
                    const Graph &g, Dims d, const PassW<float> &w, int *fail, hipStream_t st, bool pair_rows = false,
                    bool f16 = true );

struct DerivedOp {
  int kind;
  int K, N;
  float scale;
  size_t src, dst;
  int Fe = 0, FeP = 0;
};
void launch_adam(float *w, const float *g, float *m, float *v, const unsigned char *trainable, size_t n,
                 double lr, double beta1, double beta2, double eps, double weight_decay, int64_t step,
                 hipStream_t st, const int *poisoned = nullptr );
void launch_refresh_derived(float *w, const DerivedOp *ops, int num_ops, hipStream_t st);
void launch_gather_segments(const float *w, const long long *seg, int nseg, float *staging, hipStream_t st);
void launch_bn_running(float *running_mean, float *running_var, const float *batch_mean, const float *batch_var,
                       int F, double momentum, double unbias, hipStream_t st);

bool narrow_supported(Dims d);
size_t edge_narrow_lds_bytes(int fn, int fe, int tile_out_rows, int tile_in_rows);
size_t node_tiled_lds_bytes(int fn, int fe, int tile_in_rows, int tile_nodes);
void launch_node_narrow(const float *edge, const float *node_in, float *node_out, int S, const Graph &g, Dims d,
                        const PassW<float> &w, hipStream_t st);
void launch_edge_narrow(const float *edge_in, float *edge_out, const float *node, int S, const Graph &g, Dims d,
                        const PassW<float> &w, hipStream_t st);
void launch_readout_narrow(const float *edge, const float *unit4, int S, const Graph &g, Dims d,
                           const ReadoutW<float> &w, const double *mean9, const double *std9, float *vec6,
                           double *alpha, double *alpha_raw, float *pol , hipStream_t st);

}
```

ramannoodle_amd/csrc/kernels_edge_ps.hip:

```cpp
#include <algorithm>
#include <vector>

#include "fused_common.hpp"

namespace rn {

struct EdgePsArgs {
  const float *edge_in;
  float *edge_out;
  const float *node;
  const float *np3;
  float *agg_out;
  int *fail;
  int S;
  Graph g;
  Dims d;
  PassW<float> w;
};

#ifndef RN_PS_TIMING
#define RN_PS_TIMING 0
#endif
#ifndef RN_PS_PROBE
#define RN_PS_PROBE 0
#endif
#ifndef RN_PS_SLEEP
#define RN_PS_SLEEP 1
#endif
#ifndef RN_PS_PRIO
#define RN_PS_PRIO 3
#endif
#ifndef RN_PS_CPRIO
#define RN_PS_CPRIO 2
#endif
#ifndef RN_PS_LG8
#define RN_PS_LG8 1
#endif
#ifndef RN_PS_TICKET
#define RN_PS_TICKET 1
#endif
#ifndef RN_PS_LPRIO
#define RN_PS_LPRIO 1
#endif
#if RN_PS_TIMING
#define PS_T0() long long _t = (long long)__builtin_readcyclecounter(); ++tn
#define PS_TICK(i)                                                                       \
  do {                                                                                   \
    const long long _n = (long long)__builtin_readcyclecounter();                        \
    tl[(i) & 15] += (unsigned)(_n - _t);                                                 \
    _t = (long long)__builtin_readcyclecounter();                                        \
  } while (0)
#define PS_TFLUSH(first, last, shift)                                                    \
  do {                                                                                   \
    if (timed)                                                                           \
      for (int _i = (first); _i <= (last); ++_i) {                                       \
        tacc[2 * (_i + (shift))] += (long long)tl[_i & 15];                              \
        tacc[2 * (_i + (shift)) + 1] += (long long)tn;                                   \
      }                                                                                  \
  } while (0)
#else
#define PS_T0() do {} while (0)
#define PS_TICK(i) do {} while (0)
#define PS_TFLUSH(first, last, shift) do {} while (0)
#endif

namespace {
constexpr int PS_THREADS = 768;
constexpr int PS_PROD = 4;
constexpr int PS_ND = 16;
#ifndef RN_PS_NRT
#define RN_PS_NRT 8
#endif
constexpr int PS_NRT = RN_PS_NRT;
constexpr int PS_NRT_GRAM = 7;
constexpr int PS_GW = 3;
constexpr int PS_GSTRIDE = PS_GW * 16 * 16;
constexpr int PS_MAXNEW = 2;
constexpr int PS_TILE = 16 * FP;
constexpr int PS_BUF = (2 + PS_MAXNEW) * PS_TILE;

constexpr int PS_CSET = 4;
constexpr unsigned PS_FAILBIT = 0x80000000u;

enum { C_SPLIT = 0, C_NORM = 16, C_READY = 32, C_FREE0 = 48, C_FREE1 = 64, C_RD0 = 80, C_RD1 = 96, C_TICKET = 112 };

struct PsLds {
  size_t ring, qnp, bufP, bufC, atile, lnp, ints, sync, gram, total;
};
__host__ __device__ inline PsLds ps_lds(int maxR, int maxD, bool gram) {
  auto up = [](size_t b) { return (b + 15) & ~size_t(15); };
  const size_t maxR16 = ((size_t)maxR + 15) & ~size_t(15), rounds = ((size_t)maxD + PS_ND - 1) / PS_ND;
  PsLds L;
  size_t off = 0;
  const size_t ring_rows = (size_t)(gram ? PS_NRT_GRAM : PS_NRT) * 16;
  L.ring = off; off += ring_rows * LDQ * 4;
  L.qnp = off; off += ring_rows * 4 * 4;
// ... 61 lines not shown
    st.has_dest = 0;
    st.u = st.r = st.g = 0;
    st.ubs = 0;
    ps_sched_take(s, st, miss < PS_MAXNEW ? miss : PS_MAXNEW);
    return true;
  }
  const int need_now = s.u * s.nrt + s.hc + 1;
  int u2 = s.u, r2 = s.r + 1;
  if (r2 == s.nrounds) { r2 = 0; ++u2; }
  const int h2 = r2 == 0 ? s.h0 : hi(r2);
  const int need_next = u2 < s.nunits ? u2 * s.nrt + h2 + 1 : need_now;
  int n = need_next - s.P;
  n = n < 0 ? 0 : (n > PS_MAXNEW ? PS_MAXNEW : n);
  if (n < need_now - s.P) n = need_now - s.P;
  st.has_dest = 1;
  st.u = s.u;
  st.r = s.r;
  st.g = s.g;
  st.ubs = s.ubs;
  ps_sched_take(s, st, n);
  if (u2 != s.u) {
    int b = s.ubs + s.nrt % s.ring;
    s.ubs = ps_wrap(b, s.ring);
  }
  s.u = u2;
  s.r = r2;
  s.hc = h2;
  ++s.g;
  return true;
}

__device__ __forceinline__ unsigned ps_wait_ge(unsigned word, unsigned target, unsigned ready_word, int *fail, int code) {
  for (unsigned spins = 0;; ++spins) {
    unsigned v;
    asm volatile("ds_read_b32 %0, %1\n\ts_waitcnt lgkmcnt(0)" : "=v"(v) : "v"(word) : "memory");
    v = (unsigned)__builtin_amdgcn_readfirstlane((int)v);
    if (v >= target) return v;
    bool give_up = spins > (1u << 21);
    if ((spins & 1023u) == 1023u && !give_up) {
      unsigned rv;
      asm volatile("ds_read_b32 %0, %1\n\ts_waitcnt lgkmcnt(0)" : "=v"(rv) : "v"(ready_word) : "memory");
      give_up = ((unsigned)__builtin_amdgcn_readfirstlane((int)rv) & PS_FAILBIT) != 0;
    }
    if (give_up) {
      *fail = code;
      asm volatile("ds_or_b32 %0, %1\n\ts_waitcnt vmcnt(0) lgkmcnt(0)" ::"v"(ready_word), "v"(PS_FAILBIT) : "memory");
      return v | PS_FAILBIT;
    }
#if RN_PS_SLEEP
    __builtin_amdgcn_s_sleep(RN_PS_SLEEP);
#endif
  }
}
__device__ __forceinline__ void ps_arrive(unsigned word, int lane) {
  asm volatile("s_waitcnt lgkmcnt(0)" ::: "memory");
  if (lane == 0) asm volatile("ds_add_u32 %0, %1" ::"v"(word), "v"(1u) : "memory");
}
__device__ __forceinline__ unsigned ps_arrive_ticket(unsigned word, int lane) {
  asm volatile("s_waitcnt lgkmcnt(0)" ::: "memory");
  unsigned old = 0;
  if (lane == 0) asm volatile("ds_add_rtn_u32 %0, %1, %2\n\ts_waitcnt lgkmcnt(0)" : "=&v"(old) : "v"(word), "v"(1u) : "memory");
  return (unsigned)__builtin_amdgcn_readfirstlane((int)old);
}
typedef __bf16 bf16x8 __attribute__((ext_vector_type(8)));
typedef __bf16 bf16x2 __attribute__((ext_vector_type(2)));
__device__ __forceinline__ void split_bf16x8(const f32x4 &x0, const f32x4 &x1, bf16x8 &hi, bf16x8 &lo) {
#pragma unroll
  for (int j = 0; j < 4; ++j) {
    const f32x2 v = j < 2 ? f32x2{x0[2 * j], x0[2 * j + 1]} : f32x2{x1[2 * j - 4], x1[2 * j - 3]};
    const bf16x2 h = __builtin_convertvector(v, bf16x2);
    const bf16x2 l = __builtin_convertvector(v - __builtin_convertvector(h, f32x2), bf16x2);
    hi[2 * j] = h[0];
    hi[2 * j + 1] = h[1];
    lo[2 * j] = l[0];
    lo[2 * j + 1] = l[1];
  }
}
__device__ __forceinline__ void ps_publish(unsigned word, unsigned value, int lane) {
  asm volatile("s_waitcnt lgkmcnt(0)" ::: "memory");
  if (lane == 0) asm volatile("ds_max_u32 %0, %1" ::"v"(word), "v"(value) : "memory");
}
}

template <bool PAD, bool PRE, bool GRAM, bool F16 = true>
__global__ __launch_bounds__(PS_THREADS) void edge_block_ps_kernel(EdgePsArgs a) {
  static_assert(F16 || (!PRE && !GRAM), "the exact-f32 instantiation keeps float32 rows and the in-loop cross term");
  extern __shared__ __attribute__((aligned(16))) unsigned char smem_raw[];
  constexpr int NRT = GRAM ? PS_NRT_GRAM : PS_NRT, RING = NRT * 16;
  constexpr bool LG8 = RN_PS_LG8 && !GRAM;
  constexpr unsigned CPR = LG8 ? 2u : (unsigned)PS_CSET;
  auto wrap_row = [](unsigned x) -> unsigned {
    if constexpr ((RING & (RING - 1)) == 0) return x & (unsigned)(RING - 1);
    else return min(x, x - (unsigned)RING);
  };
  const Graph &g = a.g;
  const PsLds L = ps_lds(g.pt_max_out_rows, g.pt_max_in_rows, GRAM);
  auto wsc = [&](int i) { return F16 ? a.w.mfma_scale_c[i] : 1.0f; };
  float *ring = reinterpret_cast<float *>(smem_raw + L.ring);
  float *qnp = reinterpret_cast<float *>(smem_raw + L.qnp);
  float *bufP = reinterpret_cast<float *>(smem_raw + L.bufP);
  float *bufC = reinterpret_cast<float *>(smem_raw + L.bufC);
  float *atile = reinterpret_cast<float *>(smem_raw + L.atile);
  float *na_tile = atile + 2 * PS_BUF;
  float *lnp = reinterpret_cast<float *>(smem_raw + L.lnp);
  float *s_c2b = lnp, *s_g3q = lnp + 2 * FP, *s_igp = lnp + 4 * FP;
  float *s_g3p = lnp + 6 * FP, *s_c21g = lnp + 8 * FP, *s_c21b = lnp + 10 * FP, *s_c22g = lnp + 12 * FP, *s_c22b = lnp + 13 * FP,
        *s_c3g = lnp + 14 * FP, *s_c3b = lnp + 15 * FP;
  int *ints = reinterpret_cast<int *>(smem_raw + L.ints);
  unsigned *sync = reinterpret_cast<unsigned *>(smem_raw + L.sync);
  const unsigned sync_a = lds_addr(sync);
  const unsigned atile_a = lds_addr(atile), lnp_a = lds_addr(lnp), qnp_a = lds_addr(qnp), ints_a = lds_addr(ints);
  const unsigned bufP_a = lds_addr(bufP), ring_a = lds_addr(ring);
  float *gram_f = reinterpret_cast<float *>(smem_raw + L.gram);
  const int maxD = g.pt_max_in_rows, maxR16 = (g.pt_max_out_rows + 15) & ~15;
  int *qb = ints;
  int *d_edge = qb + maxR16, *d_a = d_edge + maxD, *d_b = d_a + maxD, *d_rb = d_b + maxD, *d_cnt = d_rb + maxD,
      *d_skip = d_cnt + maxD, *d_re = d_skip + maxD;
  int *hi_t = d_re + maxD;
  int *lo_t = hi_t + (maxD + PS_ND - 1) / PS_ND;
  int *misc = lo_t + (maxD + PS_ND - 1) / PS_ND;
  const int hi_off = maxR16 + 7 * maxD;
  const int lo_off = hi_off + (maxD + PS_ND - 1) / PS_ND;

  const int tid = threadIdx.x, lane = tid & 63;
  const int wave = __builtin_amdgcn_readfirstlane(tid >> 6);
  const int l15 = lane & 15, quad = lane >> 4;

  int logical = blockIdx.x;
  if ((gridDim.x & 7) == 0) logical = (blockIdx.x & 7) * (gridDim.x >> 3) + (blockIdx.x >> 3);
  const int tile = logical % g.pt_num;
  const int sg = logical / g.pt_num, nsg = gridDim.x / g.pt_num;
  const int j0 = g.pt_begin[tile], j1 = g.pt_begin[tile + 1];
  const int eo0 = g.out_ptr[j0], R = g.out_ptr[j1] - eo0;
  const int di0 = g.in_ptr[j0], D = g.in_ptr[j1] - di0;
  const int nrounds = (D + PS_ND - 1) / PS_ND;
  const int back = g.pt_back;

  for (int c = tid; c < 2 * FP; c += PS_THREADS) {
    s_c2b[c] = a.w.c2_bias_c[c] * wsc(4);
    const float gam = a.w.c3_norm_1s.g[c];
    s_g3q[c] = gam * wsc(3);
    s_igp[c] = ((c % FP) < a.d.Fe) ? wsc(1) / gam * (1.0f / (float)a.d.Fe) : 0.0f;
    if constexpr (!GRAM) {
      s_g3p[c] = gam * wsc(1);
      s_c21g[c] = a.w.c2_norm_1.g[c];
      s_c21b[c] = a.w.c2_norm_1.b[c];
      if (c < FP) {
        s_c22g[c] = a.w.c2_norm_2.g[c];
        s_c22b[c] = a.w.c2_norm_2.b[c];
        s_c3g[c] = a.w.c3_norm_2.g[c];
        s_c3b[c] = a.w.c3_norm_2.b[c];
      }
    }
  }
  for (int r = tid; r < maxR16; r += PS_THREADS) qb[r] = g.edge_b[eo0 + min(r, max(R - 1, 0))];
  for (int i = tid; i < D; i += PS_THREADS) {
    const int dst = g.in_edge[di0 + i];
    const int ad = g.edge_a[dst], bd = g.edge_b[dst];
    const int rb = g.out_ptr[bd] - eo0, re = g.out_ptr[bd + 1] - eo0;
    const int rev = g.rev_edge[dst];
    d_edge[i] = dst;
    d_a[i] = ad;
    d_b[i] = bd;
    d_rb[i] = rb;
    d_cnt[i] = (re - rb) - (rev >= 0 ? 1 : 0);
    d_skip[i] = rev >= 0 ? rev - eo0 : re;
    d_re[i] = re;
  }
  if (tid < 32) sync[tid] = 0u;
  __syncthreads();
  if (tid < nrounds) {
    int top = 0, first = 1 << 30;
    const int last = min((tid + 1) * PS_ND, D);
    for (int i = 0; i < last; ++i) {
      top = max(top, d_re[i]);
      if (i >= tid * PS_ND && d_re[i] > d_rb[i]) first = min(first, d_rb[i]);
    }
    hi_t[tid] = (top + 15) / 16 - 1;
    lo_t[tid] = first == (1 << 30) ? (top + 15) / 16 : first / 16;
  }
  __syncthreads();
  if (tid == 0) misc[0] = max(hi_t[nrounds > 0 ? nrounds - 1 : 0] + 1, 1);
  __syncthreads();
  if (D == 0 || sg >= a.S) return;
  const int nrt = __builtin_amdgcn_readfirstlane(misc[0]);
  const int nunits = (a.S - sg + nsg - 1) / nsg;

  if (wave < PS_PROD) {
    __builtin_amdgcn_s_setprio(RN_PS_PRIO);
    const int colbase = wave * 32;
    auto uni = [](float v) { return __int_as_float(__builtin_amdgcn_readfirstlane(__float_as_int(v))); };
    const float s4 = uni(wsc(0));
    const float s5 = uni(wsc(2)), inv5 = uni(wsc(3));
    const float sc2 = uni(wsc(4));
    WaveB<F16> bW4, bW5, bWc;
    bW4.load(a.w.c3_WeT_c, 4 * FP, colbase, l15, quad, s4);
    bW5.load(a.w.c3_WeT_c + 2 * FP, 4 * FP, colbase, l15, quad, s5);
    bWc.load(a.w.c2_WT_c, 2 * FP, colbase, l15, quad, sc2);
    const float qscale = uni(inv5 * inv5 / (float)(2 * a.d.Fe));

    auto request = [&](const PsStep &st, int buf, int ln) {
      const int row = 4 * wave + (ln >> 4);
      const int piece = ((ln & 15) ^ row) & 15;
      float *dst = atile + buf * PS_BUF + wave * 256;
      const unsigned ia = ints_a + (unsigned)(maxR16 + min(st.r * PS_ND + row, D - 1)) * 4u;
      int de, da, db;
      lds_read1x3(ia, ia + (unsigned)maxD * 4u, ia + 2u * (unsigned)maxD * 4u, de, da, db);
      const int s = sg + st.u * nsg;
      const float *eb = a.edge_in + (int64_t)s * g.E * FP, *nb = a.node + (int64_t)s * g.N * FP;
      const float *eb0 = a.edge_in + (int64_t)(sg + min(st.tu0, nunits - 1) * nsg) * g.E * FP;
      const float *eb1 = a.edge_in + (int64_t)(sg + min(st.tu1, nunits - 1) * nsg) * g.E * FP;
      const unsigned r0 = (unsigned)(eo0 + min(st.tt0 * 16 + row, R - 1)), r1 = (unsigned)(eo0 + min(st.tt1 * 16 + row, R - 1));
      dma16(eb + ((unsigned)de * FP + 4 * piece), dst);
      dma16(nb + ((unsigned)db * FP + 4 * piece), dst + PS_TILE);
      dma16(nb + ((unsigned)da * FP + 4 * piece), na_tile + wave * 256);
      dma16(eb0 + (r0 * FP + 4 * piece), dst + 2 * PS_TILE);
      dma16(eb1 + (r1 * FP + 4 * piece), dst + 3 * PS_TILE);
    };
    auto split_landed = [&](int buf, int ln) {
      const int row = 4 * wave + (ln >> 4), phys = ln & 15;
      const unsigned tb = atile_a + (unsigned)(buf * PS_BUF) * 4u;
      const unsigned sa = tb + (unsigned)(wave * 256 + ln * 4) * 4u;
      f32x4 u, v, w;
      if constexpr (!PRE && F16) {
        lds_read3(sa, sa + 2 * PS_TILE * 4, sa + 3 * PS_TILE * 4, u, v, w);
        write_pair(tb, row, phys, u);
        write_pair(tb + 2 * PS_TILE * 4, row, phys, v);
        write_pair(tb + 3 * PS_TILE * 4, row, phys, w);
      }
      lds_read2(sa + PS_TILE * 4, atile_a + (unsigned)(2 * PS_BUF + wave * 256 + ln * 4) * 4u, u, v);
      if constexpr (F16) {
        write_pair(tb + PS_TILE * 4, row, phys, u * v);
      } else {
        const f32x4 pr = u * v;
        lds_write4(sa + PS_TILE * 4, float4{pr[0], pr[1], pr[2], pr[3]});
      }
    };
    static_assert(PS_MAXNEW == 2, "split_landed / request are written for two source tiles per step");

    auto hi = [&](int r) { return __builtin_amdgcn_readfirstlane(lds_read1(ints_a + (unsigned)(hi_off + r) * 4u)); };
    PsSched sched;
    ps_sched_init(sched, nrounds, nrt, nunits, __builtin_amdgcn_readfirstlane(hi_t[0]), NRT);
    PsStep cur, nxt;
    bool have = ps_sched_next(sched, hi, cur);
    if (have) request(cur, 0, lane);
#if RN_PS_TIMING
    long long *tacc = reinterpret_cast<long long *>(a.fail + 16);
    const bool timed = blockIdx.x == 0 && wave == 0 && lane == 0;
    unsigned tl[16] = {0, 0, 0, 0, 0, 0, 0, 0, 0, 0, 0, 0, 0, 0, 0, 0}, tn = 0;
#endif
    for (unsigned k = 0; have; ++k) {
      PS_T0();
      const int buf = (int)(k & 1u);
      int ln = launder(lane);
      dma_wait();
      PS_TICK(0);
      f32x4 kP[2], jP[2], qS[2];
      const float *q_src;
      int ringrow0;
      {
        const int l15 = ln & 15, mycol = colbase + 4 * (ln >> 4);
        const float *np3_s = a.np3 + (int64_t)(sg + cur.u * nsg) * g.N * (6 * FP);
        const int i = min(cur.r * PS_ND + l15, D - 1);
        const unsigned ok = (unsigned)d_a[i] * (6 * FP) + 4 * FP + mycol, oj = (unsigned)d_b[i] * (6 * FP) + 2 * FP + mycol;
        const float *np3_q = a.np3 + (int64_t)(sg + min(cur.tu0, nunits - 1) * nsg) * g.N * (6 * FP);
        const unsigned oq = (unsigned)qb[min(cur.tt0 * 16 + l15, R - 1)] * (6 * FP) + mycol;
#pragma unroll
        for (int t = 0; t < 2; ++t) {
          if (RN_PS_PROBE & 8) {
            kP[t] = jP[t] = f32x4{0.f, 0.f, 0.f, 0.f} + (float)(ok + oj);
          } else {
            asm volatile("global_load_dwordx4 %0, %1, off" : "=v"(kP[t]) : "v"(np3_s + ok + 16 * t) : "memory");
            asm volatile("global_load_dwordx4 %0, %1, off" : "=v"(jP[t]) : "v"(np3_s + oj + 16 * t) : "memory");
          }
        }
        q_src = np3_q + oq;
        ringrow0 = cur.slot0 * 16 + l15;
      }
      const bool have_next = ps_sched_next(sched, hi, nxt);
      if (!(RN_PS_PROBE & 16)) split_landed(buf, ln);
      PS_TICK(1);
      ps_arrive(sync_a + C_SPLIT, ln);
      if (!(RN_PS_PROBE & 64)) ps_wait_ge(sync_a + C_SPLIT, 4u * (k + 1u), sync_a + C_READY, a.fail, 1);
      PS_TICK(2);
      PS_TICK(3);
      ln = launder(ln);
      if (!(RN_PS_PROBE & 32)) request(have_next ? nxt : cur, buf ^ 1, ln);
      auto seeds_landed = [&](f32x4 (&acc)[2]) {
        if (RN_PS_PROBE & 32)
          asm volatile("s_waitcnt vmcnt(0)" : "+v"(kP[0]), "+v"(kP[1]), "+v"(jP[0]), "+v"(jP[1]), "+v"(acc[0]), "+v"(acc[1])::"memory");
        else
          asm volatile("s_waitcnt vmcnt(5)" : "+v"(kP[0]), "+v"(kP[1]), "+v"(jP[0]), "+v"(jP[1]), "+v"(acc[0]), "+v"(acc[1])::"memory");
      };
      PS_TICK(4);
      if (cur.has_dest)
        ps_wait_ge(sync_a + ((cur.g & 1) ? C_FREE1 : C_FREE0), CPR * (unsigned)(cur.g >> 1), sync_a + C_READY, a.fail, 2);
      PS_TICK(5);
      ln = launder(ln);
      const int l15 = ln & 15, quad = ln >> 4, mycol = colbase + 4 * quad;
      const unsigned tb_a = atile_a + (unsigned)(buf * PS_BUF) * 4u;
      const int slot0 = (cur.g & 1) * PS_ND;
      {
        f32x4 accP[2] = {{0.f, 0.f, 0.f, 0.f}, {0.f, 0.f, 0.f, 0.f}};
        if (cur.has_dest) {
          if constexpr (F16) {
            f16x8 ah[2], al[2];
            load_pair_a(tb_a, l15, quad, ah, al);
            if (!(RN_PS_PROBE & 2)) bW4.product_split(ah, al, accP);
          } else {
            float af[KS];
            f32x4 unused0, unused1;
            load_f32_a2(tb_a, l15, quad, af, lnp_a, lnp_a, unused0, unused1);
            if (!(RN_PS_PROBE & 2)) bW4.product(af, accP);
          }
        }
        seeds_landed(accP);
        if (cur.has_dest) {
#pragma unroll
          for (int t = 0; t < 2; ++t)
            *reinterpret_cast<f32x4 *>(bufP + (slot0 + l15) * LDQ + mycol + 16 * t) = (kP[t] + jP[t]) * s4 + accP[t];
        }
      }
      if (RN_PS_PROBE & 8) {
        qS[0] = qS[1] = f32x4{0.f, 0.f, 0.f, 0.f};
      } else {
        asm volatile("global_load_dwordx4 %0, %1, off" : "=v"(qS[0]) : "v"(q_src) : "memory");
        asm volatile("global_load_dwordx4 %0, %1, off" : "=v"(qS[1]) : "v"(q_src + 16) : "memory");
      }
      if (cur.has_dest) {
        f32x4 accC[2];
        if constexpr (F16) {
          f16x8 ah[2], al[2];
          load_pair_a2(tb_a + PS_TILE * 4, l15, quad, ah, al, lnp_a + (unsigned)mycol * 4u, lnp_a + (unsigned)(mycol + 16) * 4u,
                       accC[0], accC[1]);
          if (!(RN_PS_PROBE & 2)) bWc.product_split(ah, al, accC);
        } else {
          float af[KS];
          load_f32_a2(tb_a + PS_TILE * 4, l15, quad, af, lnp_a + (unsigned)mycol * 4u, lnp_a + (unsigned)(mycol + 16) * 4u, accC[0], accC[1]);
          if (!(RN_PS_PROBE & 2)) bWc.product(af, accC);
        }
#pragma unroll
        for (int t = 0; t < 2; ++t)
          *reinterpret_cast<f32x4 *>(bufC + (slot0 + l15) * LDQ + mycol + 16 * t) = accC[t];
      }
      PS_TICK(6);
      const int ntl = (RN_PS_PROBE & 128) ? 0 : cur.ntiles;
      auto q_tile_finish = [&](f32x4 (&accQ)[2], const f32x4 (&g3v)[2], int ringrow) {
#pragma unroll
        for (int t = 0; t < 2; ++t) accQ[t] = qS[t] * s5 + accQ[t];
        float ss = 0.f;
#pragma unroll
        for (int t = 0; t < 2; ++t)
#pragma unroll
          for (int e = 0; e < 4; ++e) ss = fmaf(accQ[t][e], accQ[t][e], ss);
        ss = sum_xor32(sum_xor16(ss));
#pragma unroll
        for (int t = 0; t < 2; ++t) *reinterpret_cast<f32x4 *>(ring + ringrow * LDQ + mycol + 16 * t) = accQ[t] * g3v[t];
        if (quad == 0) qnp[ringrow * 4 + wave] = ss * qscale;
      };
      {
        f32x4 accQ[2] = {{0.f, 0.f, 0.f, 0.f}, {0.f, 0.f, 0.f, 0.f}}, g3v[2] = {{0.f, 0.f, 0.f, 0.f}, {0.f, 0.f, 0.f, 0.f}};
        if (ntl > 0) {
          if constexpr (F16) {
            f16x8 ah[2], al[2];
            load_pair_a2(tb_a + (unsigned)(2 * PS_TILE) * 4u, l15, quad, ah, al, lnp_a + (unsigned)(2 * FP + mycol) * 4u,
                         lnp_a + (unsigned)(2 * FP + mycol + 16) * 4u, g3v[0], g3v[1]);
            if (!(RN_PS_PROBE & 2)) bW5.product_split(ah, al, accQ);
          } else {
            float af[KS];
            load_f32_a2(tb_a + (unsigned)(2 * PS_TILE) * 4u, l15, quad, af, lnp_a + (unsigned)(2 * FP + mycol) * 4u,
                        lnp_a + (unsigned)(2 * FP + mycol + 16) * 4u, g3v[0], g3v[1]);
            if (!(RN_PS_PROBE & 2)) bW5.product(af, accQ);
          }
        }
        asm volatile("s_waitcnt vmcnt(0)" : "+v"(qS[0]), "+v"(qS[1]), "+v"(accQ[0]), "+v"(accQ[1])::"memory");
        PS_TICK(7);
        if (cur.has_dest && cur.g > back) {
          const int gdone = cur.g - back - 1;
          ps_wait_ge(sync_a + ((gdone & 1) ? C_RD1 : C_RD0), CPR * (unsigned)((gdone >> 1) + 1), sync_a + C_READY, a.fail, 3);
        }
        PS_TICK(9);
        if (ntl > 0) q_tile_finish(accQ, g3v, ringrow0);
      }
      if (ntl > 1) {
        const float *np3_q = a.np3 + (int64_t)(sg + min(cur.tu1, nunits - 1) * nsg) * g.N * (6 * FP);
        const unsigned oq = (unsigned)lds_read1(ints_a + (unsigned)min(cur.tt1 * 16 + l15, R - 1) * 4u) * (6 * FP) + mycol;
#pragma unroll
        for (int t = 0; t < 2; ++t) qS[t] = *reinterpret_cast<const f32x4 *>(np3_q + oq + 16 * t);
        f32x4 accQ[2] = {{0.f, 0.f, 0.f, 0.f}, {0.f, 0.f, 0.f, 0.f}}, g3v[2];
        if constexpr (F16) {
          f16x8 ah[2], al[2];
          load_pair_a2(tb_a + (unsigned)(3 * PS_TILE) * 4u, l15, quad, ah, al, lnp_a + (unsigned)(2 * FP + mycol) * 4u,
                       lnp_a + (unsigned)(2 * FP + mycol + 16) * 4u, g3v[0], g3v[1]);
          if (!(RN_PS_PROBE & 2)) bW5.product_split(ah, al, accQ);
        } else {
          float af[KS];
          load_f32_a2(tb_a + (unsigned)(3 * PS_TILE) * 4u, l15, quad, af, lnp_a + (unsigned)(2 * FP + mycol) * 4u,
                      lnp_a + (unsigned)(2 * FP + mycol + 16) * 4u, g3v[0], g3v[1]);
          if (!(RN_PS_PROBE & 2)) bW5.product(af, accQ);
        }
        q_tile_finish(accQ, g3v, cur.slot1 * 16 + l15);
      }
      if constexpr (GRAM) {
        if (cur.has_dest) {
          const unsigned prow_a = bufP_a + (unsigned)((slot0 + l15) * LDQ + mycol) * 4u;
          const unsigned ig_a = lnp_a + (unsigned)(4 * FP + mycol) * 4u;
          const int lo = __builtin_amdgcn_readfirstlane(lds_read1(ints_a + (unsigned)(lo_off + cur.r) * 4u));
          const int hiw = __builtin_amdgcn_readfirstlane(lds_read1(ints_a + (unsigned)(hi_off + cur.r) * 4u));
          unsigned qa[PS_GW];
#pragma unroll
          for (int k = 0; k < PS_GW; ++k) {
            int sl = cur.ubs + min(lo + k, max(hiw, lo));
// ... 53 lines not shown
    const float eps_c2 = 1e-5f * wsc(4) * wsc(4);
    int nval[2];
#pragma unroll
    for (int j = 0; j < 2; ++j) nval[j] = min(max(a.d.Fe - (4 * l7 + 32 * j), 0), 4);
    f32x2 bf2[2][2], bc2[2][2];
#pragma unroll
    for (int j = 0; j < 2; ++j) {
      const Vec4<float> bf = load4<float>(a.w.c3_norm_1s.b + 4 * l7 + 32 * j), bc = load4<float>(a.w.c3_norm_1s.b + FP + 4 * l7 + 32 * j);
      bf2[j][0] = f32x2{bf.v[0], bf.v[1]};
      bf2[j][1] = f32x2{bf.v[2], bf.v[3]};
      bc2[j][0] = f32x2{bc.v[0], bc.v[1]};
      bc2[j][1] = f32x2{bc.v[2], bc.v[3]};
      asm volatile("s_waitcnt vmcnt(0)" : "+v"(bf2[j][0]), "+v"(bf2[j][1]), "+v"(bc2[j][0]), "+v"(bc2[j][1]));
    }
    const float *ringc = ring + 4 * l7;
    const int sdelta = 2 * FP - 4 * l7;
    const unsigned total_rounds = (unsigned)nunits * (unsigned)nrounds;
    auto ln64 = [&](const Vec4<float> (&x)[2], const float *gt, const float *bt, Vec4<float> (&y)[2]) {
      float sum = 0.f;
#pragma unroll
      for (int j = 0; j < 2; ++j) sum += (x[j].v[0] + x[j].v[1]) + (x[j].v[2] + x[j].v[3]);
      const float mean = lg_sum<8>(sum) * invn;
      float dv[2][4], qq = 0.f;
#pragma unroll
      for (int j = 0; j < 2; ++j)
#pragma unroll
        for (int k = 0; k < 4; ++k) {
          dv[j][k] = x[j].v[k] - mean;
          if (PAD && k >= nval[j]) dv[j][k] = 0.f;
          qq = fmaf(dv[j][k], dv[j][k], qq);
        }
      const float rstd = fast_rsq(lg_sum<8>(qq) * invn + 1e-5f);
#pragma unroll
      for (int j = 0; j < 2; ++j) {
        const Vec4<float> gv = load4<float>(gt + 4 * l7 + 32 * j), bv = load4<float>(bt + 4 * l7 + 32 * j);
#pragma unroll
        for (int k = 0; k < 4; ++k) y[j].v[k] = dv[j][k] * rstd * gv.v[k] + bv.v[k];
      }
    };
    bool poisoned = false;
#if RN_PS_TIMING
    long long *tacc = reinterpret_cast<long long *>(a.fail + 16);
    const bool timed = blockIdx.x == 0 && (cw & 3) == 0 && lane == 0;
    unsigned tl[16] = {0, 0, 0, 0, 0, 0, 0, 0, 0, 0, 0, 0, 0, 0, 0, 0}, tn = 0;
#endif
    for (;;) {
      PS_T0();
      const unsigned tk = ps_arrive_ticket(sync_a + C_TICKET, lane);
      const unsigned gr = tk >> 1;
      if (gr >= total_rounds) break;
      const int slot = 8 * (int)(tk & 1u) + grp;
      const int u = (int)(gr / (unsigned)nrounds), r = (int)(gr - (unsigned)u * (unsigned)nrounds);
      const int ub = (int)(((unsigned)u * (unsigned)(nrt % NRT)) % (unsigned)NRT) * 16;
      poisoned |= (ps_wait_ge(sync_a + C_READY, gr + 1u, sync_a + C_READY, a.fail, 4) & PS_FAILBIT) != 0;
      PS_TICK(10);
      const int64_t erow0 = (int64_t)(sg + u * nsg) * g.E;
      const bool active = r * PS_ND + slot < D;
      const int i = min(r * PS_ND + slot, D - 1);
      const int64_t drow = erow0 + d_edge[i];
      f32x2 pf2[2][2], pc2[2][2], pdf2[2][2], pdc2[2][2];
      float spe;
      {
        const float *prow = bufP + ((int)(gr & 1u) * PS_ND + slot) * LDQ;
        float sp = 0.f;
#pragma unroll
        for (int j = 0; j < 2; ++j) {
          const int cj = 4 * l7 + 32 * j;
          const Vec4<float> xf = load4<float>(prow + cj), xc = load4<float>(prow + FP + cj);
          const Vec4<float> gf = load4<float>(s_g3p + cj), gc = load4<float>(s_g3p + FP + cj);
          const Vec4<float> jf = load4<float>(s_igp + cj), jc = load4<float>(s_igp + FP + cj);
#pragma unroll
          for (int k = 0; k < 4; ++k) sp += xf.v[k] * xf.v[k] + xc.v[k] * xc.v[k];
#pragma unroll
          for (int hh = 0; hh < 2; ++hh) {
            pdf2[j][hh] = f32x2{xf.v[2 * hh] * jf.v[2 * hh], xf.v[2 * hh + 1] * jf.v[2 * hh + 1]};
            pdc2[j][hh] = f32x2{xc.v[2 * hh] * jc.v[2 * hh], xc.v[2 * hh + 1] * jc.v[2 * hh + 1]};
            pf2[j][hh] = f32x2{xf.v[2 * hh] * gf.v[2 * hh], xf.v[2 * hh + 1] * gf.v[2 * hh + 1]};
            pc2[j][hh] = f32x2{xc.v[2 * hh] * gc.v[2 * hh], xc.v[2 * hh + 1] * gc.v[2 * hh + 1]};
          }
        }
        spe = lg_sum<8>(sp) * spscale + 1e-5f;
      }
      Vec4<float> c2v[2];
      {
        const float *crow = bufC + ((int)(gr & 1u) * PS_ND + slot) * LDQ;
        Vec4<float> xf[2], xc[2];
        float q = 0.f;
#pragma unroll
        for (int j = 0; j < 2; ++j) {
          xf[j] = load4<float>(crow + 4 * l7 + 32 * j);
          xc[j] = load4<float>(crow + FP + 4 * l7 + 32 * j);
#pragma unroll
          for (int k = 0; k < 4; ++k) q += xf[j].v[k] * xf[j].v[k] + xc[j].v[k] * xc[j].v[k];
        }
        const float rstd2 = fast_rsq(lg_sum<8>(q) * inv2n + eps_c2);
        Vec4<float> g2[2];
#pragma unroll
        for (int j = 0; j < 2; ++j) {
          const int cj = 4 * l7 + 32 * j;
          const Vec4<float> gf = load4<float>(s_c21g + cj), bf = load4<float>(s_c21b + cj);
          const Vec4<float> gc = load4<float>(s_c21g + FP + cj), bc = load4<float>(s_c21b + FP + cj);
#pragma unroll
          for (int k = 0; k < 4; ++k)
            g2[j].v[k] = (RN_PS_PROBE & 4) ? xf[j].v[k] + xc[j].v[k]
                                           : gate(xf[j].v[k] * rstd2 * gf.v[k] + bf.v[k], xc[j].v[k] * rstd2 * gc.v[k] + bc.v[k]);
        }
        if (RN_PS_PROBE & 4) {
          c2v[0] = g2[0];
          c2v[1] = g2[1];
        } else {
          ln64(g2, s_c22g, s_c22b, c2v);
        }
      }
      const int rb = d_rb[i], cnt = active ? d_cnt[i] : 0, rskip = d_skip[i];
      const int rbase = (int)wrap_row(wrap_row((unsigned)(ub + rb)));
      ps_arrive(sync_a + ((gr & 1u) ? C_FREE1 : C_FREE0), lane);
      PS_TICK(11);
      float acc[8] = {0.f, 0.f, 0.f, 0.f, 0.f, 0.f, 0.f, 0.f};
      {
        auto triplet = [&](const float *qr, float (&sumk)[8]) {
          f32x2 qf2[2][2], qc2[2][2];
#pragma unroll
          for (int j = 0; j < 2; ++j) {
            const float4 qfv = *reinterpret_cast<const float4 *>(qr + 32 * j), qcv = *reinterpret_cast<const float4 *>(qr + FP + 32 * j);
            qf2[j][0] = f32x2{qfv.x, qfv.y};
            qf2[j][1] = f32x2{qfv.z, qfv.w};
            qc2[j][0] = f32x2{qcv.x, qcv.y};
            qc2[j][1] = f32x2{qcv.z, qcv.w};
          }
          const float qs = qr[sdelta];
          f32x2 d2 = pdf2[0][0] * qf2[0][0], d3 = pdc2[0][0] * qc2[0][0];
          d2 = __builtin_elementwise_fma(pdf2[0][1], qf2[0][1], d2);
          d3 = __builtin_elementwise_fma(pdc2[0][1], qc2[0][1], d3);
          d2 = __builtin_elementwise_fma(pdf2[1][0], qf2[1][0], d2);
          d3 = __builtin_elementwise_fma(pdc2[1][0], qc2[1][0], d3);
          d2 = __builtin_elementwise_fma(pdf2[1][1], qf2[1][1], d2);
          d3 = __builtin_elementwise_fma(pdc2[1][1], qc2[1][1], d3);
          d2 += d3;
          const float dot = lg_sum<8>(d2.x + d2.y);
          float ve = dot + (spe + qs);
          ve = ve > 1e-5f ? ve : 1e-5f;
          const float rstd = fast_rsq(ve);
          const f32x2 rstd2 = {rstd, rstd}, one2 = {1.0f, 1.0f};
#pragma unroll
          for (int j = 0; j < 2; ++j)
#pragma unroll
            for (int hh = 0; hh < 2; ++hh) {
              const f32x2 xf2 = __builtin_elementwise_fma(pf2[j][hh] + qf2[j][hh], rstd2, bf2[j][hh]);
              const f32x2 xc2 = __builtin_elementwise_fma(pc2[j][hh] + qc2[j][hh], rstd2, bc2[j][hh]);
              const f32x2 e1 = {fast_exp2(xf2.x), fast_exp2(xf2.y)}, e2 = {fast_exp2(xc2.x), fast_exp2(xc2.y)};
              const f32x2 t2 = e2 + one2;
              const f32x2 den = __builtin_elementwise_fma(e1, t2, t2);
              const f32x2 rd = {fast_rcp(den.x), fast_rcp(den.y)};
              f32x2 sk = {sumk[4 * j + 2 * hh], sumk[4 * j + 2 * hh + 1]};
              sk = __builtin_elementwise_fma(e2 - one2, rd, sk);
              sumk[4 * j + 2 * hh] = sk.x;
              sumk[4 * j + 2 * hh + 1] = sk.y;
            }
        };
#if RN_PS_CPRIO
        __builtin_amdgcn_s_setprio(0);
#endif
        float acc2[8] = {0.f, 0.f, 0.f, 0.f, 0.f, 0.f, 0.f, 0.f};
        const int tskip = rskip - rb;
        auto row_of = [&](int t) { return ringc + __umul24(wrap_row((unsigned)(rbase + t + (t >= tskip ? 1 : 0))), (unsigned)LDQ); };
        int t = (RN_PS_PROBE & 1) ? cnt : 0;
        const int tmid = RN_PS_LPRIO ? ((cnt >> 1) & ~1) : 0;
        for (; t + 1 < tmid; t += 2) {
          triplet(row_of(t), acc);
          triplet(row_of(t + 1), acc2);
        }
#if RN_PS_LPRIO
        __builtin_amdgcn_s_setprio(RN_PS_LPRIO);
#endif
        for (; t + 1 < cnt; t += 2) {
          triplet(row_of(t), acc);
          triplet(row_of(t + 1), acc2);
        }
        if (t < cnt) triplet(row_of(t), acc);
#pragma unroll
        for (int k = 0; k < 8; ++k) acc[k] += acc2[k];
      }
      PS_TICK(12);
#if RN_PS_CPRIO
      __builtin_amdgcn_s_setprio(RN_PS_CPRIO);
#endif
      f32x4 old4[2];
#pragma unroll
      for (int j = 0; j < 2; ++j) {
        const int cj = 4 * l7 + 32 * j;
        if constexpr (PRE) {
          const char *pp = reinterpret_cast<const char *>(a.edge_in + drow * FP + (cj >> 3) * 8) + (cj & 7) * 2;
          const f16x4 hh = *reinterpret_cast<const f16x4 *>(pp), ll = *reinterpret_cast<const f16x4 *>(pp + 16);
#pragma unroll
          for (int k = 0; k < 4; ++k) old4[j][k] = (float)hh[k] + (float)ll[k];
        } else {
          old4[j] = *reinterpret_cast<const f32x4 *>(a.edge_in + drow * FP + cj);
        }
      }
      poisoned |= (ps_wait_ge(sync_a + ((gr & 1u) ? C_RD1 : C_RD0), CPR * (gr >> 1), sync_a + C_READY, a.fail, 6) & PS_FAILBIT) != 0;
      ps_arrive(sync_a + ((gr & 1u) ? C_RD1 : C_RD0), lane);
      if (active) {
        Vec4<float> a4[2], c3[2];
#pragma unroll
        for (int j = 0; j < 2; ++j) {
          a4[j] = Vec4<float>{{acc[4 * j], acc[4 * j + 1], acc[4 * j + 2], acc[4 * j + 3]}};
          if (a.agg_out) store4(a.agg_out + drow * FP + 4 * l7 + 32 * j, a4[j]);
        }
        if (RN_PS_PROBE & 4) {
          c3[0] = a4[0];
          c3[1] = a4[1];
        } else {
          ln64(a4, s_c3g, s_c3b, c3);
        }
#pragma unroll
        for (int j = 0; j < 2; ++j) {
          const int cj = 4 * l7 + 32 * j;
          f32x4 y;
#pragma unroll
          for (int k = 0; k < 4; ++k) {
            y[k] = (RN_PS_PROBE & 4) ? old4[j][k] + c2v[j].v[k] + c3[j].v[k] : fast_tanh(old4[j][k] + c2v[j].v[k] + c3[j].v[k]);
            if (poisoned) y[k] = __int_as_float(0x7fc00000);
          }
          if constexpr (PRE) {
            char *pp = reinterpret_cast<char *>(a.edge_out + drow * FP + (cj >> 3) * 8) + (cj & 7) * 2;
            f16x4 hh, ll;
#pragma unroll
            for (int k = 0; k < 4; ++k) {
              hh[k] = (_Float16)y[k];
              ll[k] = (_Float16)(y[k] - (float)hh[k]);
            }
            *reinterpret_cast<f16x4 *>(pp) = hh;
            *reinterpret_cast<f16x4 *>(pp + 16) = ll;
          } else {
            *reinterpret_cast<f32x4 *>(a.edge_out + drow * FP + cj) = y;
          }
        }
      }
      PS_TICK(13);
    }
    PS_TFLUSH(10, 13, (cw >> 2) ? 6 : 0);
    return;
  }
  const int cset = cw >> 2;
  const int c0 = 4 * l15;
  const int nvalid = min(max(a.d.Fe - c0, 0), 4);
  const float inv2n = 1.0f / (float)(2 * a.d.Fe), invn = 1.0f / (float)a.d.Fe;
  const float spscale = wsc(1) * wsc(1) * inv2n;
  const float eps_c2 = 1e-5f * wsc(4) * wsc(4);
  f32x2 bf2[2], bc2[2];
  {
    const Vec4<float> bf = load4<float>(a.w.c3_norm_1s.b + c0), bc = load4<float>(a.w.c3_norm_1s.b + FP + c0);
    bf2[0] = f32x2{bf.v[0], bf.v[1]};
    bf2[1] = f32x2{bf.v[2], bf.v[3]};
    bc2[0] = f32x2{bc.v[0], bc.v[1]};
    bc2[1] = f32x2{bc.v[2], bc.v[3]};
    asm volatile("s_waitcnt vmcnt(0)" : "+v"(bf2[0]), "+v"(bf2[1]), "+v"(bc2[0]), "+v"(bc2[1]));
  }
  LnParams<float> k_c3 = {load4<float>(a.w.c3_norm_2.g + c0), load4<float>(a.w.c3_norm_2.b + c0)};
  LnParams<float> k_c21f = {load4<float>(a.w.c2_norm_1.g + c0), load4<float>(a.w.c2_norm_1.b + c0)};
  LnParams<float> k_c21c = {load4<float>(a.w.c2_norm_1.g + FP + c0), load4<float>(a.w.c2_norm_1.b + FP + c0)};
  LnParams<float> k_c22 = {load4<float>(a.w.c2_norm_2.g + c0), load4<float>(a.w.c2_norm_2.b + c0)};
  Vec4<float> g3f = load4<float>(a.w.c3_norm_1s.g + c0), g3c = load4<float>(a.w.c3_norm_1s.g + FP + c0);
  {
    auto pin = [](Vec4<float> &x) { asm volatile("s_waitcnt vmcnt(0)" : "+v"(x.v[0]), "+v"(x.v[1]), "+v"(x.v[2]), "+v"(x.v[3])); };
    pin(k_c3.g); pin(k_c3.b); pin(k_c21f.g); pin(k_c21f.b); pin(k_c21c.g); pin(k_c21c.b); pin(k_c22.g); pin(k_c22.b);
    pin(g3f); pin(g3c);
  }
#pragma unroll
  for (int k = 0; k < 4; ++k) {
    g3f.v[k] *= wsc(1);
    g3c.v[k] *= wsc(1);
  }
  Vec4<float> igf = load4<float>(s_igp + c0), igc = load4<float>(s_igp + FP + c0);
  const float *ringc = ring + c0;
  const int sdelta = 2 * FP - c0;
  const unsigned total_rounds = (unsigned)nunits * (unsigned)nrounds;
  auto locate = [&](unsigned gr, int &u, int &r, int &ub) {
    u = (int)(gr / (unsigned)nrounds);
    r = (int)(gr - (unsigned)u * (unsigned)nrounds);
    ub = (int)(((unsigned)u * (unsigned)(nrt % NRT)) % (unsigned)NRT) * 16;
// ... 176 lines not shown
#pragma unroll
      for (int k = 0; k < 4; ++k) acc[k] += acc2[k];
    }
    PS_TICK(12);
#if RN_PS_CPRIO
    __builtin_amdgcn_s_setprio(RN_PS_CPRIO);
#endif
    poisoned |= (ps_wait_ge(sync_a + ((gr & 1u) ? C_RD1 : C_RD0), CPR * (gr >> 1), sync_a + C_READY, a.fail, 6) & PS_FAILBIT) != 0;
    ps_arrive(sync_a + ((gr & 1u) ? C_RD1 : C_RD0), lane);
    if (active) {
      const Vec4<float> a4 = {{acc[0], acc[1], acc[2], acc[3]}};
      if (a.agg_out) store4(a.agg_out + drow * FP + c0, a4);
      const Vec4<float> c3 = (RN_PS_PROBE & 4) ? a4 : ln_row<LG, PAD, float>(a4, k_c3, invn, nvalid);
      f32x4 y;
#pragma unroll
      for (int k = 0; k < 4; ++k) {
        y[k] = (RN_PS_PROBE & 4) ? old4[k] + c2v.v[k] + c3.v[k] : fast_tanh(old4[k] + c2v.v[k] + c3.v[k]);
        if (poisoned) y[k] = __int_as_float(0x7fc00000);
      }
      if constexpr (PRE) {
        char *pp = reinterpret_cast<char *>(a.edge_out + drow * FP + (c0 >> 3) * 8) + (c0 & 7) * 2;
        f16x4 hh, ll;
#pragma unroll
        for (int k = 0; k < 4; ++k) {
          hh[k] = (_Float16)y[k];
          ll[k] = (_Float16)(y[k] - (float)hh[k]);
        }
        *reinterpret_cast<f16x4 *>(pp) = hh;
        *reinterpret_cast<f16x4 *>(pp + 16) = ll;
      } else {
        *reinterpret_cast<f32x4 *>(a.edge_out + drow * FP + c0) = y;
      }
    }
    PS_TICK(13);
  }
  PS_TFLUSH(10, 13, cset ? 6 : 0);
}

size_t edge_ps_lds_bytes(int rows, int in_rows, bool gram) { return ps_lds(rows, in_rows, gram).total; }
int edge_ps_ring_tiles(bool gram) { return gram ? PS_NRT_GRAM : PS_NRT; }
int edge_ps_gram_window() { return PS_GW; }

bool edge_ps_tile_ok(const int *rb, const int *re, int D, int back, int ring, int *window) {
  if (D <= 0) return true;
  const int nrounds = (D + PS_ND - 1) / PS_ND;
  std::vector<int> hi(nrounds), lo(nrounds);
  int top = 0;
  for (int r = 0; r < nrounds; ++r) {
    const int last = std::min((r + 1) * PS_ND, D);
    int first_row = 1 << 30;
    for (int i = r * PS_ND; i < last; ++i) {
      top = std::max(top, re[i]);
      if (re[i] > rb[i]) first_row = std::min(first_row, rb[i]);
    }
    hi[r] = (top + 15) / 16 - 1;
    lo[r] = first_row == (1 << 30) ? (hi[r] + 1) : first_row / 16;
  }
  const int nrt = std::max(hi[nrounds - 1] + 1, 1);
  if (nrt > 2 * ring) return false;
  const int units = 3 + back;
  PsSched s;
  if (window) {
    int w = 0;
    for (int r = 0; r < nrounds; ++r) w = std::max(w, hi[r] - std::min(lo[r], hi[r] + 1) + 1);
    *window = w;
  }
  ps_sched_init(s, nrounds, nrt, units, hi[0], ring);
  PsStep st;
  auto hif = [&](int r) { return hi[r]; };
  while (ps_sched_next(s, hif, st)) {
    if (st.ntiles > PS_MAXNEW) return false;
    if (!st.has_dest) {
      if (st.tile0 + st.ntiles > ring) return false;
      continue;
    }
    const int g1 = std::max(st.g - back, 0), u1 = g1 / nrounds, r1 = g1 % nrounds;
    const int oldest = u1 * nrt + std::min(lo[r1], hi[r1] + 1);
    if (st.tile0 + st.ntiles - oldest > ring) return false;
    if (st.u * nrt + hi[st.r] + 1 > st.tile0 + st.ntiles) return false;
  }
  return true;
}

void launch_edge_ps(const float *edge_in, float *edge_out, const float *node, const float *np3, float *agg_out, int S,
                    const Graph &g, Dims d, const PassW<float> &w, int *fail, hipStream_t st, bool pair_rows, bool f16) {
  if (S == 0 || g.E == 0) return;
  EdgePsArgs a{edge_in, edge_out, node, np3, agg_out, fail, S, g, d, w};
  const bool gram = g.pt_gram != 0 && f16;
  if (!f16) pair_rows = false;
  const size_t lds = ps_lds(g.pt_max_out_rows, g.pt_max_in_rows, gram).total;
  const bool pad = d.Fe != d.FeP;
  auto kern = !f16 ? (pad ? &edge_block_ps_kernel<true, false, false, false> : &edge_block_ps_kernel<false, false, false, false>)
              : gram ? (pair_rows ? (pad ? &edge_block_ps_kernel<true, true, true> : &edge_block_ps_kernel<false, true, true>)
                                  : (pad ? &edge_block_ps_kernel<true, false, true> : &edge_block_ps_kernel<false, false, true>))
                     : (pair_rows ? (pad ? &edge_block_ps_kernel<true, true, false> : &edge_block_ps_kernel<false, true, false>)
                                  : (pad ? &edge_block_ps_kernel<true, false, false> : &edge_block_ps_kernel<false, false, false>));
  (void)hipFuncSetAttribute(reinterpret_cast<const void *>(kern), hipFuncAttributeMaxDynamicSharedMemorySize, (int)lds);
  static int cus = 0;
  if (cus == 0) {
    int dev = 0;
    hipDeviceProp_t prop;
    if (hipGetDevice(&dev) == hipSuccess && hipGetDeviceProperties(&prop, dev) == hipSuccess)
      cus = prop.multiProcessorCount;
    if (cus <= 0) cus = 256;
  }
  int nsg = cus / g.pt_num;
  nsg = nsg < 1 ? 1 : (nsg > S ? S : nsg);
  kern<<<(unsigned)nsg * (unsigned)g.pt_num, PS_THREADS, lds, st>>>(a);
}

}
```

ramannoodle_amd/pmodel/potgnn.py:

```python
from __future__ import annotations

import ctypes as C
from collections import OrderedDict

import numpy as np
import torch
from numpy.typing import NDArray
from torch.autograd.function import once_differentiable

from ramannoodle_amd import _lib
from ramannoodle_amd.abstract import PolarizabilityModel
from ramannoodle_amd.constants import RAMAN_TENSOR_CENTRAL_DIFFERENCE
from ramannoodle_amd.exceptions import verify_ndarray_shape
from ramannoodle_amd.pmodel import graph as graph_utils

_VEC_TO_TENSOR = np.array([[0, 3, 4], [3, 1, 5], [4, 5, 2]])


def polarizability_vectors_to_tensors(vectors):
    if vectors.ndim != 2 or vectors.shape[1] != 6:
        raise ValueError(f"polarizability_vectors has wrong size: {list(vectors.shape)} != [_,6]")
    return vectors[:, _VEC_TO_TENSOR]


# ... 821 lines not shown
            if tuple(out.shape) != shape:
                raise ValueError(f"out has shape {tuple(out.shape)}, the increments are {shape}")
            if not out.is_contiguous():
                raise ValueError("out must be contiguous")
        self.eval()
        handle = self._ensure_handle()
        stream = torch.cuda.current_stream(positions.device).cuda_stream
        if lattices is not None:
            rc = _lib.load().rn_potgnn_group_increments_cells_device(
                handle, C.c_void_p(positions.data_ptr()), C.c_void_p(lattices.data_ptr()), s, _ptr(labels), num_groups,
                int(float64), int(workspace_limit), C.c_void_p(out.data_ptr()), C.c_void_p(stream))
            _lib.check(rc, handle, "rn_potgnn_group_increments_cells_device")
            return out
        rc = _lib.load().rn_potgnn_group_increments_device(
            handle, C.c_void_p(positions.data_ptr()), s, _ptr(labels), num_groups, int(float64), int(workspace_limit),
            C.c_void_p(out.data_ptr()), C.c_void_p(stream))
        _lib.check(rc, handle, "rn_potgnn_group_increments_device")
        return out

    def calc_group_increments(self, positions_ts, groups, float64: bool = True, lattices=None) -> NDArray[np.float64]:
        verify_ndarray_shape("positions_ts", positions_ts, (None, self.num_atoms, 3))
        device = f"cuda:{self.device_index}"
        if lattices is not None:
            from ramannoodle_amd.dynamics import verify_lattices
            lattices = torch.tensor(verify_lattices(lattices, len(positions_ts)), device=device)
        positions = torch.tensor(np.asarray(positions_ts, dtype=np.float64), device=device)
        return self.calc_group_increments_device(positions, groups, float64=float64, lattices=lattices).cpu().numpy()

    def calc_partial_raman_tensors(self, ref_positions, displacements, groups) -> NDArray[np.float64]:
        self._check_raman_arguments(ref_positions, displacements, method="analytic")
        labels, num_groups = self._group_labels(groups)
        ref = np.ascontiguousarray(ref_positions, dtype=np.float64)
        disp = np.ascontiguousarray(displacements, dtype=np.float64)
        out = np.empty((disp.shape[0], num_groups, 3, 3), dtype=np.float64)
        self.eval()
        handle = self._ensure_handle()
        rc = _lib.load().rn_potgnn_partial_raman_tensors(handle, _ptr(ref), _ptr(disp), disp.shape[0], _ptr(labels),
                                                         num_groups, _ptr(out))
        _lib.check(rc, handle, "rn_potgnn_partial_raman_tensors")
        return out

    @property
    def num_triplets(self) -> int:
        return int(_lib.load().rn_potgnn_num_triplets(self._ensure_handle()))

    def triplets(self):
        handle = self._ensure_handle()
        lib = _lib.load()
        t = int(lib.rn_potgnn_num_triplets(handle))
        arrs = [np.empty(t, dtype=np.int32) for _ in range(5)]
        rc = lib.rn_potgnn_debug_triplets(handle, *[_ptr(a) for a in arrs])
        _lib.check(rc, handle, "rn_potgnn_debug_triplets")
        idx_i, idx_j, idx_k, slot5, slot6 = [a.astype(np.int64) for a in arrs]
        order = np.lexsort((idx_k, slot6))
        return (self._ref_edge_indexes[2].copy(), self._ref_edge_indexes[1].copy(),
                idx_i[order], idx_j[order], idx_k[order], slot5[order], slot6[order])

    def device_triplets_raw(self):
        handle = self._ensure_handle()
        lib = _lib.load()
        t = int(lib.rn_potgnn_num_triplets(handle))
        arrs = [np.empty(t, dtype=np.int32) for _ in range(5)]
        _lib.check(lib.rn_potgnn_debug_triplets(handle, *[_ptr(a) for a in arrs]), handle,
                   "rn_potgnn_debug_triplets")
        return arrs

    def debug_stage(self, stage: int, index: int = 0) -> np.ndarray:
        handle = self._ensure_handle()
        lib = _lib.load()
        cap = 64 * 1024 * 1024
        buf = np.empty(cap, dtype=np.float32)
        rows, cols = C.c_int64(), C.c_int64()
        rc = lib.rn_potgnn_debug_stage(handle, stage, index, _ptr(buf), cap, C.byref(rows),
                                       C.byref(cols))
        _lib.check(rc, handle, "rn_potgnn_debug_stage")
        return buf[: rows.value * cols.value].reshape(rows.value, cols.value).copy()

    def config_flags(self) -> dict:
        flags = _lib.load().rn_potgnn_config_flags(self._ensure_handle())
        return {"fused_edge_block": bool(flags & 1), "folded_gate_scale": bool(flags & 2),
                "split_f16_mfma": bool(flags & 4), "narrow_kernels": bool(flags & 8),
                "mfma_range_fallback": bool(flags & 16),
                "role_split_edge_block": bool(flags & 256), "atom_owning_node_block": bool(flags & 512),
                "split_f16_pair_rows": bool(flags & 1024)}

    def set_profiling(self, mode: int) -> None:
        self._profiling = int(mode)
        if self._handle is not None:
            _lib.load().rn_potgnn_set_profiling(self._handle, self._profiling)

    def kernel_times(self) -> dict:
        handle = self._ensure_handle()
        lib = _lib.load()
        names = (C.c_char_p * 16)()
        ms = (C.c_double * 16)()
        launches = (C.c_int64 * 16)()
        n = lib.rn_potgnn_kernel_times(handle, names, ms, launches, 16)
        return {names[i].decode(): (ms[i], launches[i]) for i in range(max(n, 0))}


def _requires_grad(value) -> bool:
    return isinstance(value, torch.Tensor) and value.requires_grad


def _as_input_grad(grad, like: torch.Tensor):
    if grad is None:
        return None
    return grad.reshape(like.shape).to(device=like.device, dtype=like.dtype)


class _EvalInputGrad(torch.autograd.Function):

    @staticmethod
    def forward(ctx, model, lattice, atomic_numbers, positions):
        ctx.model = model
        ctx.atomic_numbers = atomic_numbers
        lat_t = lattice if isinstance(lattice, torch.Tensor) else torch.as_tensor(lattice)
        pos_t = positions if isinstance(positions, torch.Tensor) else torch.as_tensor(positions)
        ctx.save_for_backward(lat_t, pos_t)
        return model.forward(lattice, atomic_numbers, positions)

    @staticmethod
    @once_differentiable
    def backward(ctx, grad_out):
        lat_t, pos_t = ctx.saved_tensors
        want_lat, want_pos = ctx.needs_input_grad[1], ctx.needs_input_grad[3]
        dpos, dlat = ctx.model._input_gradients(lat_t, ctx.atomic_numbers, pos_t, grad_out, want_pos, want_lat)
        return (None, _as_input_grad(dlat, lat_t) if want_lat else None, None,
                _as_input_grad(dpos, pos_t) if want_pos else None)


class _TrainStep(torch.autograd.Function):

    @staticmethod
    def forward(ctx, model, pos, extra, pos_t, lat_t, *params):
        ctx.model = model
        ctx.inputs = (pos_t.detach(), lat_t.detach())
        return torch.from_numpy(model._train_forward(pos, *extra))

    @staticmethod
    @once_differentiable
    def backward(ctx, grad_out):
        dvec6 = np.ascontiguousarray(grad_out.detach().cpu().numpy(), dtype=np.float32)
        want_pos, want_lat = ctx.needs_input_grad[3], ctx.needs_input_grad[4]
        s = dvec6.shape[0]
        dpos = np.empty((s, ctx.model.num_atoms, 3), dtype=np.float64) if want_pos else None
        dlat = np.empty((s, 9), dtype=np.float64) if want_lat else None
        if ctx.model._device_training:
            ctx.model._train_backward_device(dvec6, dpos, dlat)
            params = []
        else:
            grads = ctx.model._train_backward(dvec6, dpos, dlat)
            params = [g.to(device=p.device, dtype=p.dtype)
                      for g, p in zip(grads, [p for _, p in torch.nn.Module.named_parameters(ctx.model)])]
        pos_t, lat_t = ctx.inputs
        din = (_as_input_grad(None if dpos is None else torch.from_numpy(dpos), pos_t),
               _as_input_grad(None if dlat is None else torch.from_numpy(dlat), lat_t))
        if ctx.model._device_training:
            return (None, None, None, *din, None)
        return (None, None, None, *din, *params)


class _TrainStepOnDevice(torch.autograd.Function):

    @staticmethod
    def forward(ctx, model, lat_t, zs_t, pos_t, anchor):
        ctx.model = model
# ... 44 lines not shown
```

Measured before the change: 59230.

## Compute c2 projection once per atom pair in a separate kernel

Adds a pair table that maps each edge and its reverse edge to one atom pair. A new c2_pairs kernel computes the c2 node-product projection and its norms once per pair into a scratch buffer. The edge_block_ps kernel then loads those rows instead of fetching both node rows and running the c2 MFMA per edge, which removes two DMA requests and an in-loop matrix product. The cost is an extra kernel launch, a global write and read of the pair rows, and a dependence on bufA being large enough to hold them.

```diff
diff --git a/include/rn_potgnn.h b/include/rn_potgnn.h
--- a/include/rn_potgnn.h
+++ b/include/rn_potgnn.h
@@ -212,6 +212,9 @@
 int rn_potgnn_debug_plan(const rn_potgnn_config *cfg, const int32_t *edge_a, const int32_t *edge_b,
                          const int32_t *atom_types, int32_t num_cus, int32_t *out, size_t capacity, size_t *count);
 
+int rn_potgnn_debug_plan_pairs(const rn_potgnn_config *cfg, const int32_t *edge_a, const int32_t *edge_b,
+                               const int32_t *atom_types, int32_t num_cus, int32_t *out, size_t capacity, size_t *count);
+
 int rn_potgnn_debug_plan_lds(const rn_potgnn_config *cfg, const int32_t *edge_a, const int32_t *edge_b,
                              const int32_t *atom_types, int32_t num_cus, int64_t *out, size_t capacity, size_t *count);
 
diff --git a/ramannoodle_amd/_lib.py b/ramannoodle_amd/_lib.py
--- a/ramannoodle_amd/_lib.py
+++ b/ramannoodle_amd/_lib.py
@@ -86,6 +86,7 @@
     "rn_potgnn_debug_triplets": (C.c_int, [_P, _P, _P, _P, _P, _P]),
     "rn_potgnn_debug_ps_schedule": (C.c_int, [_P, _P, C.c_int32, C.c_int32, C.c_int32, _P]),
     "rn_potgnn_debug_plan": (C.c_int, [C.POINTER(Config), _P, _P, _P, C.c_int32, _P, C.c_size_t, C.POINTER(C.c_size_t)]),
+    "rn_potgnn_debug_plan_pairs": (C.c_int, [C.POINTER(Config), _P, _P, _P, C.c_int32, _P, C.c_size_t, C.POINTER(C.c_size_t)]),
     "rn_potgnn_debug_plan_lds": (C.c_int, [C.POINTER(Config), _P, _P, _P, C.c_int32, _P, C.c_size_t, C.POINTER(C.c_size_t)]),
     "rn_potgnn_debug_pack_weights": (C.c_int, [C.POINTER(Config), _P, C.c_size_t, _P, _P, _P, _P, C.c_size_t, C.POINTER(C.c_size_t)]),
     "rn_potgnn_debug_unpack_weights": (C.c_int, [C.POINTER(Config), _P, C.c_size_t, C.c_int, _P, C.c_size_t, C.POINTER(C.c_size_t)]),
diff --git a/ramannoodle_amd/csrc/api.hip b/ramannoodle_amd/csrc/api.hip
--- a/ramannoodle_amd/csrc/api.hip
+++ b/ramannoodle_amd/csrc/api.hip
@@ -57,11 +57,11 @@
 
 enum KernelId {
   K_GEOM = 0, K_NODE_INIT, K_PROJ_NODE, K_PROJ_EDGE_C1, K_NODE_AGG, K_PROJ_EDGE_C3, K_PROJ_C2,
-  K_EDGE_AGG, K_READOUT_MLP, K_READOUT_REDUCE, K_COUNT
+  K_EDGE_AGG, K_READOUT_MLP, K_READOUT_REDUCE, K_C2_PAIRS, K_COUNT
 };
 const char *kKernelNames[K_COUNT] = {
     "geom_rbf", "node_init", "proj_node", "proj_edge_c1", "node_agg", "proj_edge_c3",
-    "proj_c2", "edge_agg", "readout_mlp", "readout_reduce"};
+    "proj_c2", "edge_agg", "readout_mlp", "readout_reduce", "c2_pairs"};
 
 template <typename T>
 struct Lane {
@@ -107,10 +107,13 @@
   int chunk = 1;
   size_t f64_budget = 0;
   bool keep_stages = false;
+  bool snap_pairs = false;
+  bool last_pair_rows = false;
   bool debug_sync = false;
   GraphPlan plan;
   bool split_projections = true;
   bool want_pair_rows = true;
+  bool want_c2_pairs = true;
   DeviceBuf step_seg, step_stage;
   float *step_host = nullptr;
   bool tape_ps = true;
@@ -223,6 +226,10 @@
 size_t bufA_width(const rn_potgnn *h, bool lean) {
   return lean ? 32 : std::max<size_t>(std::max(2 * h->d.FnP, 2 * h->d.FeP), 32);
 }
+bool c2_rows_fit(const rn_potgnn *h) {
+  return edge_ps_takes_c2_rows(h->g, true, h->mfma_f16) &&
+         (size_t)h->g.NP * h->d.FeP <= (size_t)h->g.E * bufA_width(h, lean_workspace(h));
+}
 size_t per_structure_elems(const rn_potgnn *h, bool lean) {
   const size_t N = h->cfg.num_atoms, E = h->cfg.num_edges;
   const size_t FnP = h->d.FnP, FeP = h->d.FeP;
@@ -311,7 +318,7 @@
     ln.bufA.ensure(S * E * bufA * sizeof(T));
     if (!lean) ln.bufB.ensure(S * E * 4 * FeP * sizeof(T));
   }
-  if (h->keep_stages) {
+  if (h->keep_stages || h->snap_pairs) {
     const int np = h->cfg.num_message_passes + 1;
     P.snap_node.resize(np);
     P.snap_edge.resize(np);
@@ -422,7 +429,7 @@
   }
   void snapshot(int p) {
     Precision<T> &P = prec<T>(h);
-    if (!h->keep_stages) return;
+    if (!h->keep_stages && !h->snap_pairs) return;
     HIP_TRY(hipMemcpyAsync(P.snap_node[p].p, node[cur], (size_t)MN * h->d.FnP * sizeof(T),
                            hipMemcpyDeviceToDevice, st()));
     HIP_TRY(hipMemcpyAsync(P.snap_edge[p].p, edge[cur], (size_t)ME * h->d.FeP * sizeof(T),
@@ -450,6 +457,7 @@
       }
       if (!done) launch_geom_rbf<T>(io.pos, S, h->g, lat, lat_stride, P.offsets, gauss, h->d, unit4, edge[0], st(), narrow());
       h->last_in_order = narrow();
+      h->last_pair_rows = pair_rows();
     }
     {
       Timer t(h, st(), K_NODE_INIT);
@@ -533,11 +541,19 @@
   void stage_aggregate(int p) {
     const PassW<T> &w = prec<T>(h).pass[p];
     const int nxt = cur ^ 1;
+    const float *c2_rows = nullptr;
+    if constexpr (sizeof(T) == 4) {
+      if (c2_pairs(w)) {
+        Timer t(h, st(), K_C2_PAIRS);
+        launch_c2_pairs(node[nxt], bufA, S, h->g, h->d, w, st());
+        c2_rows = bufA;
+      }
+    }
     {
       Timer t(h, st(), K_EDGE_AGG);
       if constexpr (sizeof(T) == 4) {
         if (narrow()) launch_edge_narrow(edge[cur], edge[nxt], node[nxt], S, h->g, h->d, w, st());
-        else if (role_split(w)) launch_edge_ps(edge[cur], edge[nxt], node[nxt], np3, tape_agg(p), S, h->g, h->d, w, h->ps_fail.as<int>(), st(), pair_rows(), h->mfma_f16);
+        else if (role_split(w)) launch_edge_ps(edge[cur], edge[nxt], node[nxt], np3, tape_agg(p), S, h->g, h->d, w, h->ps_fail.as<int>(), st(), pair_rows(), h->mfma_f16, c2_rows);
         else if (fused()) edge_unfused_in_blocks(p);
         else HIP_TRY(launch_edge_agg<T>(bufB, np3, bufA, edge[cur], edge[nxt], S, h->g, h->d, w, tape_agg(p), st()));
       } else {
@@ -627,6 +643,10 @@
       if (!role_split(w)) return false;
     return true;
   }
+  bool c2_pairs(const PassW<T> &w) const {
+    if (sizeof(T) != 4 || !h->want_c2_pairs || !role_split(w) || !pair_rows()) return false;
+    return c2_rows_fit(h);
+  }
   T *tape_agg(int p) {
     Precision<T> &P = prec<T>(h);
     return P.tape_on ? P.tape_agg[p].template as<T>() : nullptr;
@@ -733,7 +753,7 @@
   h->train_S = 0;
   while (done < S) {
     const int64_t left = S - done;
-    if (lanes == 2 && h->interleave && !h->keep_stages && left > 1) {
+    if (lanes == 2 && h->interleave && !h->keep_stages && !h->snap_pairs && left > 1) {
       const int64_t both = std::min<int64_t>(left, 2 * (int64_t)chunk);
       const int sa = (int)((both + 1) / 2), sb = (int)(both - sa);
       ChunkRun<T> a = make(0, done, sa), b = make(1, done + sa, sb);
@@ -1526,7 +1546,8 @@
   const size_t o_a = push(plan.edge_a), o_b = push(plan.edge_b), o_op = push(plan.out_ptr),
                o_ip = push(plan.in_ptr), o_ie = push(plan.in_edge), o_at = push(plan.atom_type),
                o_tb = push(plan.tile.begin), o_to = push(plan.trip_off), o_rv = push(plan.rev_edge),
-               o_nt = push(plan.nt.begin), o_bt = push(plan.bt.begin), o_pt = push(plan.pt.begin), o_ipos = push(plan.in_pos);
+               o_nt = push(plan.nt.begin), o_bt = push(plan.bt.begin), o_pt = push(plan.pt.begin), o_ipos = push(plan.in_pos),
+               o_pe = push(plan.pair_of_edge), o_pa = push(plan.pair_a), o_pb = push(plan.pair_b);
   buf.ensure(ints.size() * sizeof(int));
   HIP_TRY(hipMemcpy(buf.p, ints.data(), ints.size() * sizeof(int), hipMemcpyHostToDevice));
   const int *base = buf.as<int>();
@@ -1539,6 +1560,9 @@
   g.in_pos = base + o_ipos;
   g.atom_type = base + o_at;
   g.rev_edge = base + o_rv;
+  g.pair_of_edge = base + o_pe;
+  g.pair_a = base + o_pa;
+  g.pair_b = base + o_pb;
   g.tile_begin = base + o_tb;
   g.trip_off = base + o_to;
   g.nt_begin = base + o_nt;
@@ -1594,7 +1618,8 @@
   std::memcpy(h->lattice, lattice, sizeof(h->lattice));
   std::memcpy(h->mean, mean, sizeof(h->mean));
   std::memcpy(h->stdv, stddev, sizeof(h->stdv));
-  h->keep_stages = getenv("RN_POTGNN_KEEP_STAGES") && atoi(getenv("RN_POTGNN_KEEP_STAGES")) != 0;
+  h->snap_pairs = getenv("RN_POTGNN_KEEP_STAGES") && atoi(getenv("RN_POTGNN_KEEP_STAGES")) == 2;
+  h->keep_stages = getenv("RN_POTGNN_KEEP_STAGES") && atoi(getenv("RN_POTGNN_KEEP_STAGES")) != 0 && !h->snap_pairs;
   h->debug_sync = getenv("RN_POTGNN_DEBUG_SYNC") && atoi(getenv("RN_POTGNN_DEBUG_SYNC")) != 0;
   if (const char *e = getenv("RN_POTGNN_INTERLEAVE")) h->interleave = atoi(e) != 0;
   if (const char *e = getenv("RN_POTGNN_MFMA")) h->mfma_f16_requested = !(e[0] == 'f' && e[1] == '3');
@@ -1603,6 +1628,7 @@
   if (const char *e = getenv("RN_POTGNN_TAPE_PS")) h->tape_ps = atoi(e) != 0;
   h->split_projections = getenv("RN_POTGNN_SPLIT_PROJ") ? atoi(getenv("RN_POTGNN_SPLIT_PROJ")) != 0 : true;
   h->want_pair_rows = !(getenv("RN_POTGNN_PAIR_ROWS") && atoi(getenv("RN_POTGNN_PAIR_ROWS")) == 0);
+  h->want_c2_pairs = !(getenv("RN_POTGNN_C2_PAIRS") && atoi(getenv("RN_POTGNN_C2_PAIRS")) == 0);
 
   const PlanKnobs knobs = read_plan_knobs();
   h->d = plan_dims(*cfg, knobs);
@@ -1649,6 +1675,32 @@
     *count = flat.size();
     if (!out || capacity < flat.size()) {
       set_error(nullptr, "out holds %zu values, the plan has %zu", out ? capacity : (size_t)0, flat.size());
+      return RN_ERR_INVALID_ARGUMENT;
+    }
+    std::memcpy(out, flat.data(), flat.size() * sizeof(int32_t));
+    return RN_OK;
+  } catch (const std::bad_alloc &) {
+    set_error(nullptr, "host allocation failed");
+    return RN_ERR_OUT_OF_MEMORY;
+  }
+}
+
+int rn_potgnn_debug_plan_pairs(const rn_potgnn_config *cfg, const int32_t *edge_a, const int32_t *edge_b,
+                               const int32_t *atom_types, int32_t num_cus, int32_t *out, size_t capacity, size_t *count) {
+  if (!count || num_cus <= 0) return RN_ERR_INVALID_ARGUMENT;
+  *count = 0;
+  std::string invalid;
+  const int rc = validate_create_args(cfg, edge_a, edge_b, atom_types, false, nullptr, invalid);
+  if (rc != RN_OK) {
+    set_error(nullptr, "%s", invalid.c_str());
+    return rc;
+  }
+  try {
+    const PlanKnobs knobs = read_plan_knobs();
+    const std::vector<int32_t> flat = plan_graph(*cfg, plan_dims(*cfg, knobs), edge_a, edge_b, atom_types, num_cus, knobs).flat_pairs();
+    *count = flat.size();
+    if (!out || capacity < flat.size()) {
+      set_error(nullptr, "out holds %zu values, the pair table has %zu", out ? capacity : (size_t)0, flat.size());
       return RN_ERR_INVALID_ARGUMENT;
     }
     std::memcpy(out, flat.data(), flat.size() * sizeof(int32_t));
@@ -2584,6 +2636,7 @@
     const bool atom = h->plan.use_fused && h->plan.use_node_fused && h->mfma_f16 && centred && h->g.na_num > 0;
     flags |= atom ? 512 : 0;
     flags |= (atom && (flags & 256) && h->plan.use_readout_fused && h->want_pair_rows && !h->keep_stages) ? 1024 : 0;
+    flags |= ((flags & 1024) && h->want_c2_pairs && c2_rows_fit(h)) ? 2048 : 0;
   }
   bool fast = !h->f32.pass.empty();
   for (const auto &p : h->f32.pass) fast = fast && !h->plan.use_narrow && (p.c3_fast & (h->plan.use_fused ? 1 : 2));
@@ -2637,8 +2690,8 @@
     if (stage == 0) {
       src = P.lanes[0].unit4.as<float>(); r = ME; c = 4; ld = 4;
     } else if (stage == 1 || stage == 2) {
-      if (!h->keep_stages || index < 0 || index > h->cfg.num_message_passes)
-        throw HipError{hipErrorInvalidValue, "stage snapshots need RN_POTGNN_KEEP_STAGES=1"};
+      if ((!h->keep_stages && !h->snap_pairs) || index < 0 || index > h->cfg.num_message_passes)
+        throw HipError{hipErrorInvalidValue, "stage snapshots need RN_POTGNN_KEEP_STAGES=1 or 2"};
       if (stage == 1) { src = P.snap_node[index].as<float>(); r = MN; c = h->d.Fn; ld = h->d.FnP; }
       else { src = P.snap_edge[index].as<float>(); r = ME; c = h->d.Fe; ld = h->d.FeP; }
     } else if (stage == 3) {
@@ -2647,6 +2700,18 @@
       throw HipError{hipErrorInvalidValue, "unknown stage"};
     }
     if ((size_t)(r * c) > out_capacity) throw HipError{hipErrorInvalidValue, "out_capacity too small"};
+    if (stage == 2 && h->snap_pairs && h->last_pair_rows) {
+      std::vector<_Float16> raw((size_t)r * 128);
+      HIP_TRY(hipMemcpy(raw.data(), src, raw.size() * sizeof(_Float16), hipMemcpyDeviceToHost));
+      for (int64_t i = 0; i < r; ++i)
+        for (int64_t k = 0; k < c; ++k) {
+          const _Float16 *grp = raw.data() + i * 128 + (k >> 3) * 16;
+          out[i * c + k] = (float)grp[k & 7] + (float)grp[8 + (k & 7)];
+        }
+      *rows = r;
+      *cols = c;
+      return;
+    }
     HIP_TRY(hipMemcpy2D(out, c * sizeof(float), src, ld * sizeof(float), c * sizeof(float), r,
                         hipMemcpyDeviceToHost));
     if (h->last_in_order && r == ME && stage != 1) {
diff --git a/ramannoodle_amd/csrc/graph_plan.hip b/ramannoodle_amd/csrc/graph_plan.hip
--- a/ramannoodle_amd/csrc/graph_plan.hip
+++ b/ramannoodle_amd/csrc/graph_plan.hip
@@ -269,6 +269,19 @@
     if (it != hi && *it == ad) g.rev_edge[e] = (int)(it - edge_b);
   }
   g.T = g.trip_off[E];
+  g.pair_of_edge.assign(E, -1);
+  g.pair_a.clear();
+  g.pair_b.clear();
+  for (int e = 0; e < E; ++e) {
+    const int r = g.rev_edge[e];
+    if (r >= 0 && r < e) {
+      g.pair_of_edge[e] = g.pair_of_edge[r];
+    } else {
+      g.pair_of_edge[e] = (int)g.pair_a.size();
+      g.pair_a.push_back(edge_a[e]);
+      g.pair_b.push_back(edge_b[e]);
+    }
+  }
 }
 
 }
@@ -420,6 +433,7 @@
 Graph GraphPlan::scalars() const {
   Graph s{};
   s.N = N, s.E = E, s.T = T;
+  s.NP = (int)pair_a.size();
   s.num_tiles = tile.num(), s.max_tile_out_rows = tile.max_out_rows, s.max_tile_in_rows = tile.max_in_rows, s.max_tile_nodes = tile.max_nodes;
   s.nt_num = nt.num(), s.nt_max_in_rows = nt.max_in_rows, s.nt_max_nodes = nt.max_nodes, s.nt_narrow = nt_narrow ? 1 : 0;
   s.na_num = na_num, s.na_max_deg = na_max_deg;
@@ -457,4 +471,10 @@
   return o;
 }
 
-}
+std::vector<int32_t> GraphPlan::flat_pairs() const {
+  std::vector<int32_t> o = {(int32_t)pair_a.size()};
+  for (const std::vector<int> *v : {&pair_of_edge, &pair_a, &pair_b}) o.insert(o.end(), v->begin(), v->end());
+  return o;
+}
+
+}
diff --git a/ramannoodle_amd/csrc/graph_plan.hpp b/ramannoodle_amd/csrc/graph_plan.hpp
--- a/ramannoodle_amd/csrc/graph_plan.hpp
+++ b/ramannoodle_amd/csrc/graph_plan.hpp
@@ -53,6 +53,8 @@
   std::vector<int> in_edge, in_pos;
   std::vector<int> rev_edge;
   std::vector<int> trip_off;
+  std::vector<int> pair_of_edge;
+  std::vector<int> pair_a, pair_b;
   int64_t T = 0;
   Partition tile, nt, bt, pt;
   bool nt_narrow = false;
@@ -68,6 +70,7 @@
   Graph scalars() const;
   std::vector<int64_t> lds_requests() const;
   std::vector<int32_t> flat() const;
+  std::vector<int32_t> flat_pairs() const;
 };
 
 GraphPlan plan_graph(const rn_potgnn_config &cfg, Dims d, const int32_t *edge_a, const int32_t *edge_b,
diff --git a/ramannoodle_amd/csrc/kernels.hpp b/ramannoodle_amd/csrc/kernels.hpp
--- a/ramannoodle_amd/csrc/kernels.hpp
+++ b/ramannoodle_amd/csrc/kernels.hpp
@@ -16,6 +16,9 @@
   const int *in_pos;
   const int *atom_type;
   const int *rev_edge;
+  int NP;
+  const int *pair_of_edge;
+  const int *pair_a, *pair_b;
   int num_tiles;
   const int *tile_begin;
   int max_tile_out_rows;
@@ -261,7 +264,11 @@
 bool edge_ps_tile_ok(const int *rb, const int *re, int D, int back, int ring, int *window);
 void launch_edge_ps(const float *edge_in, float *edge_out, const float *node, const float *np3, float *agg_out, int S,
                     const Graph &g, Dims d, const PassW<float> &w, int *fail, hipStream_t st, bool pair_rows = false,
-                    bool f16 = true );
+                    bool f16 = true ,
+                    const float *c2_rows = nullptr );
+bool edge_ps_takes_c2_rows(const Graph &g, bool pair_rows, bool f16);
+
+void launch_c2_pairs(const float *node, float *out, int S, const Graph &g, Dims d, const PassW<float> &w, hipStream_t st);
 
 struct DerivedOp {
   int kind;
diff --git a/ramannoodle_amd/csrc/kernels_c2_pairs.hip b/ramannoodle_amd/csrc/kernels_c2_pairs.hip
--- /dev/null
+++ b/ramannoodle_amd/csrc/kernels_c2_pairs.hip
@@ -0,0 +1,147 @@
+#include "fused_common.hpp"
+
+namespace rn {
+
+struct C2PairArgs {
+  const float *node;
+  float *out;
+  int64_t M;
+  int N, NP;
+  const int *pair_a, *pair_b;
+  Dims d;
+  PassW<float> w;
+};
+
+namespace {
+constexpr int C2P_THREADS = 256;
+}
+
+__global__ __launch_bounds__(C2P_THREADS, 2) void c2_pairs_kernel(C2PairArgs a) {
+  __shared__ __attribute__((aligned(16))) float s_bias[2 * FP], s_g1[2 * FP], s_b1[2 * FP], s_g2[FP], s_b2[FP];
+  const int tid = threadIdx.x, lane = tid & 63, wave = tid >> 6;
+  const int l15 = lane & 15, quad = lane >> 4;
+  const float sc2 = a.w.mfma_scale_c[4];
+  for (int c = tid; c < 2 * FP; c += C2P_THREADS) {
+    s_bias[c] = a.w.c2_bias_c[c] * sc2;
+    s_g1[c] = a.w.c2_norm_1.g[c];
+    s_b1[c] = a.w.c2_norm_1.b[c];
+    if (c < FP) {
+      s_g2[c] = a.w.c2_norm_2.g[c];
+      s_b2[c] = a.w.c2_norm_2.b[c];
+    }
+  }
+  WaveB<true> bW[4];
+#pragma unroll
+  for (int p = 0; p < 4; ++p) bW[p].load(a.w.c2_WT_c, 2 * FP, 32 * p, l15, quad, sc2);
+  __syncthreads();
+
+  const float inv2n = 1.0f / (float)(2 * a.d.Fe), invn = 1.0f / (float)a.d.Fe;
+  const float eps_c2 = 1e-5f * sc2 * sc2;
+  const int64_t ntiles = (a.M + 15) / 16, stride = (int64_t)gridDim.x * (C2P_THREADS / 64);
+
+  f32x4 xb[4], xa[4];
+  auto fetch = [&](int64_t tile) {
+    int64_t row = tile * 16 + l15;
+    if (row >= a.M) row = a.M - 1;
+    const int64_t s = row / a.NP;
+    const int p = (int)(row - s * a.NP);
+    const float *nb = a.node + (s * a.N + a.pair_b[p]) * FP + 16 * quad, *na = a.node + (s * a.N + a.pair_a[p]) * FP + 16 * quad;
+#pragma unroll
+    for (int j = 0; j < 4; ++j) {
+      xb[j] = *reinterpret_cast<const f32x4 *>(nb + 4 * j);
+      xa[j] = *reinterpret_cast<const f32x4 *>(na + 4 * j);
+    }
+  };
+  int64_t tile = (int64_t)blockIdx.x * (C2P_THREADS / 64) + wave;
+  if (tile < ntiles) fetch(tile);
+  for (; tile < ntiles; tile += stride) {
+    float af[KS];
+#pragma unroll
+    for (int j = 0; j < 4; ++j) {
+      const f32x4 pr = xb[j] * xa[j];
+#pragma unroll
+      for (int i = 0; i < 4; ++i) af[4 * j + i] = pr[i];
+    }
+    f16x8 ah[2], al[2];
+    split_f16x8(af, ah[0], al[0]);
+    split_f16x8(af + 8, ah[1], al[1]);
+    if (tile + stride < ntiles) fetch(tile + stride);
+
+    const int lq = launder(lane >> 4);
+    f32x4 acc[4][2];
+#pragma unroll
+    for (int p = 0; p < 4; ++p) {
+#pragma unroll
+      for (int t = 0; t < 2; ++t) acc[p][t] = *reinterpret_cast<const f32x4 *>(s_bias + 32 * p + 16 * t + 4 * lq);
+      bW[p].product_split(ah, al, acc[p]);
+    }
+    float q = 0.f;
+#pragma unroll
+    for (int p = 0; p < 4; ++p)
+#pragma unroll
+      for (int t = 0; t < 2; ++t)
+#pragma unroll
+        for (int i = 0; i < 4; ++i) q = fmaf(acc[p][t][i], acc[p][t][i], q);
+    q = sum_xor32(sum_xor16(q));
+    const float rstd2 = fast_rsq(q * inv2n + eps_c2);
+    float gv[2][2][4], sum = 0.f;
+#pragma unroll
+    for (int p = 0; p < 2; ++p)
+#pragma unroll
+      for (int t = 0; t < 2; ++t) {
+        const int c = 32 * p + 16 * t + 4 * lq;
+        const Vec4<float> gf = load4<float>(s_g1 + c), bf = load4<float>(s_b1 + c);
+        const Vec4<float> gc = load4<float>(s_g1 + FP + c), bc = load4<float>(s_b1 + FP + c);
+#pragma unroll
+        for (int i = 0; i < 4; ++i) {
+          gv[p][t][i] = gate(acc[p][t][i] * rstd2 * gf.v[i] + bf.v[i], acc[p + 2][t][i] * rstd2 * gc.v[i] + bc.v[i]);
+          sum += gv[p][t][i];
+        }
+      }
+    const float mean = sum_xor32(sum_xor16(sum)) * invn;
+    float qq = 0.f;
+#pragma unroll
+    for (int p = 0; p < 2; ++p)
+#pragma unroll
+      for (int t = 0; t < 2; ++t)
+#pragma unroll
+        for (int i = 0; i < 4; ++i) {
+          const int c = 32 * p + 16 * t + 4 * lq + i;
+          gv[p][t][i] = c < a.d.Fe ? gv[p][t][i] - mean : 0.f;
+          qq = fmaf(gv[p][t][i], gv[p][t][i], qq);
+        }
+    const float rstd = fast_rsq(sum_xor32(sum_xor16(qq)) * invn + 1e-5f);
+    const int64_t row = tile * 16 + l15;
+    if (row < a.M) {
+#pragma unroll
+      for (int p = 0; p < 2; ++p)
+#pragma unroll
+        for (int t = 0; t < 2; ++t) {
+          const int c = 32 * p + 16 * t + 4 * lq;
+          const Vec4<float> g2 = load4<float>(s_g2 + c), b2 = load4<float>(s_b2 + c);
+          f32x4 y;
+#pragma unroll
+          for (int i = 0; i < 4; ++i) y[i] = gv[p][t][i] * rstd * g2.v[i] + b2.v[i];
+          *reinterpret_cast<f32x4 *>(a.out + row * FP + c) = y;
+        }
+    }
+  }
+}
+
+void launch_c2_pairs(const float *node, float *out, int S, const Graph &g, Dims d, const PassW<float> &w, hipStream_t st) {
+  const int64_t M = (int64_t)S * g.NP;
+  if (M == 0) return;
+  C2PairArgs a{node, out, M, g.N, g.NP, g.pair_a, g.pair_b, d, w};
+  static int cus = 0;
+  if (cus == 0) {
+    int dev = 0;
+    hipDeviceProp_t prop;
+    if (hipGetDevice(&dev) == hipSuccess && hipGetDeviceProperties(&prop, dev) == hipSuccess) cus = prop.multiProcessorCount;
+    if (cus <= 0) cus = 256;
+  }
+  const int64_t ntiles = (M + 15) / 16, per_wg = C2P_THREADS / 64;
+  const int64_t grid = std::min<int64_t>((ntiles + per_wg - 1) / per_wg, (int64_t)2 * cus);
+  c2_pairs_kernel<<<(unsigned)grid, C2P_THREADS, 0, st>>>(a);
+}
+
+}
diff --git a/ramannoodle_amd/csrc/kernels_edge_ps.hip b/ramannoodle_amd/csrc/kernels_edge_ps.hip
--- a/ramannoodle_amd/csrc/kernels_edge_ps.hip
+++ b/ramannoodle_amd/csrc/kernels_edge_ps.hip
@@ -12,6 +12,7 @@
   const float *np3;
   float *agg_out;
   int *fail;
+  const float *c2;
   int S;
   Graph g;
   Dims d;
@@ -239,9 +240,11 @@
 }
 }
 
-template <bool PAD, bool PRE, bool GRAM, bool F16 = true>
+template <bool PAD, bool PRE, bool GRAM, bool F16 = true, bool C2G = false>
 __global__ __launch_bounds__(PS_THREADS) void edge_block_ps_kernel(EdgePsArgs a) {
   static_assert(F16 || (!PRE && !GRAM), "the exact-f32 instantiation keeps float32 rows and the in-loop cross term");
+  static_assert(!C2G || (F16 && PRE && !GRAM && RN_PS_LG8), "c2 rows are taken by the pair-row, eight-lane form only");
+  constexpr int NREQ = C2G ? 3 : 5;
   extern __shared__ __attribute__((aligned(16))) unsigned char smem_raw[];
   constexpr int NRT = GRAM ? PS_NRT_GRAM : PS_NRT, RING = NRT * 16;
   constexpr bool LG8 = RN_PS_LG8 && !GRAM;
@@ -353,7 +356,7 @@
     WaveB<F16> bW4, bW5, bWc;
     bW4.load(a.w.c3_WeT_c, 4 * FP, colbase, l15, quad, s4);
     bW5.load(a.w.c3_WeT_c + 2 * FP, 4 * FP, colbase, l15, quad, s5);
-    bWc.load(a.w.c2_WT_c, 2 * FP, colbase, l15, quad, sc2);
+    if constexpr (!C2G) bWc.load(a.w.c2_WT_c, 2 * FP, colbase, l15, quad, sc2);
     const float qscale = uni(inv5 * inv5 / (float)(2 * a.d.Fe));
 
     auto request = [&](const PsStep &st, int buf, int ln) {
@@ -369,8 +372,10 @@
       const float *eb1 = a.edge_in + (int64_t)(sg + min(st.tu1, nunits - 1) * nsg) * g.E * FP;
       const unsigned r0 = (unsigned)(eo0 + min(st.tt0 * 16 + row, R - 1)), r1 = (unsigned)(eo0 + min(st.tt1 * 16 + row, R - 1));
       dma16(eb + ((unsigned)de * FP + 4 * piece), dst);
-      dma16(nb + ((unsigned)db * FP + 4 * piece), dst + PS_TILE);
-      dma16(nb + ((unsigned)da * FP + 4 * piece), na_tile + wave * 256);
+      if constexpr (!C2G) {
+        dma16(nb + ((unsigned)db * FP + 4 * piece), dst + PS_TILE);
+        dma16(nb + ((unsigned)da * FP + 4 * piece), na_tile + wave * 256);
+      }
       dma16(eb0 + (r0 * FP + 4 * piece), dst + 2 * PS_TILE);
       dma16(eb1 + (r1 * FP + 4 * piece), dst + 3 * PS_TILE);
     };
@@ -385,12 +390,14 @@
         write_pair(tb + 2 * PS_TILE * 4, row, phys, v);
         write_pair(tb + 3 * PS_TILE * 4, row, phys, w);
       }
-      lds_read2(sa + PS_TILE * 4, atile_a + (unsigned)(2 * PS_BUF + wave * 256 + ln * 4) * 4u, u, v);
-      if constexpr (F16) {
-        write_pair(tb + PS_TILE * 4, row, phys, u * v);
-      } else {
-        const f32x4 pr = u * v;
-        lds_write4(sa + PS_TILE * 4, float4{pr[0], pr[1], pr[2], pr[3]});
+      if constexpr (!C2G) {
+        lds_read2(sa + PS_TILE * 4, atile_a + (unsigned)(2 * PS_BUF + wave * 256 + ln * 4) * 4u, u, v);
+        if constexpr (F16) {
+          write_pair(tb + PS_TILE * 4, row, phys, u * v);
+        } else {
+          const f32x4 pr = u * v;
+          lds_write4(sa + PS_TILE * 4, float4{pr[0], pr[1], pr[2], pr[3]});
+        }
       }
     };
     static_assert(PS_MAXNEW == 2, "split_landed / request are written for two source tiles per step");
@@ -447,7 +454,7 @@
         if (RN_PS_PROBE & 32)
           asm volatile("s_waitcnt vmcnt(0)" : "+v"(kP[0]), "+v"(kP[1]), "+v"(jP[0]), "+v"(jP[1]), "+v"(acc[0]), "+v"(acc[1])::"memory");
         else
-          asm volatile("s_waitcnt vmcnt(5)" : "+v"(kP[0]), "+v"(kP[1]), "+v"(jP[0]), "+v"(jP[1]), "+v"(acc[0]), "+v"(acc[1])::"memory");
+          asm volatile("s_waitcnt vmcnt(%6)" : "+v"(kP[0]), "+v"(kP[1]), "+v"(jP[0]), "+v"(jP[1]), "+v"(acc[0]), "+v"(acc[1]) : "n"(NREQ) : "memory");
       };
       PS_TICK(4);
       if (cur.has_dest)
@@ -484,7 +491,7 @@
         asm volatile("global_load_dwordx4 %0, %1, off" : "=v"(qS[0]) : "v"(q_src) : "memory");
         asm volatile("global_load_dwordx4 %0, %1, off" : "=v"(qS[1]) : "v"(q_src + 16) : "memory");
       }
-      if (cur.has_dest) {
+      if constexpr (!C2G) if (cur.has_dest) {
         f32x4 accC[2];
         if constexpr (F16) {
           f16x8 ah[2], al[2];
@@ -704,7 +711,9 @@
         spe = lg_sum<8>(sp) * spscale + 1e-5f;
       }
       Vec4<float> c2v[2];
-      {
+      int c2pair = 0;
+      if constexpr (C2G) c2pair = g.pair_of_edge[d_edge[i]];
+      if constexpr (!C2G) {
         const float *crow = bufC + ((int)(gr & 1u) * PS_ND + slot) * LDQ;
         Vec4<float> xf[2], xc[2];
         float q = 0.f;
@@ -819,6 +828,11 @@
         } else {
           old4[j] = *reinterpret_cast<const f32x4 *>(a.edge_in + drow * FP + cj);
         }
+      }
+      if constexpr (C2G) {
+        const float *crow = a.c2 + ((int64_t)(sg + u * nsg) * g.NP + c2pair) * FP;
+#pragma unroll
+        for (int j = 0; j < 2; ++j) c2v[j] = load4<float>(crow + 4 * l7 + 32 * j);
       }
       poisoned |= (ps_wait_ge(sync_a + ((gr & 1u) ? C_RD1 : C_RD0), CPR * (gr >> 1), sync_a + C_READY, a.fail, 6) & PS_FAILBIT) != 0;
       ps_arrive(sync_a + ((gr & 1u) ? C_RD1 : C_RD0), lane);
@@ -1161,10 +1175,16 @@
   return true;
 }
 
+bool edge_ps_takes_c2_rows(const Graph &g, bool pair_rows, bool f16) {
+  return RN_PS_LG8 != 0 && f16 && pair_rows && g.pt_gram == 0 && g.NP > 0;
+}
+
 void launch_edge_ps(const float *edge_in, float *edge_out, const float *node, const float *np3, float *agg_out, int S,
-                    const Graph &g, Dims d, const PassW<float> &w, int *fail, hipStream_t st, bool pair_rows, bool f16) {
+                    const Graph &g, Dims d, const PassW<float> &w, int *fail, hipStream_t st, bool pair_rows, bool f16,
+                    const float *c2_rows) {
   if (S == 0 || g.E == 0) return;
-  EdgePsArgs a{edge_in, edge_out, node, np3, agg_out, fail, S, g, d, w};
+  if (!edge_ps_takes_c2_rows(g, pair_rows, f16)) c2_rows = nullptr;
+  EdgePsArgs a{edge_in, edge_out, node, np3, agg_out, fail, c2_rows, S, g, d, w};
   const bool gram = g.pt_gram != 0 && f16;
   if (!f16) pair_rows = false;
   const size_t lds = ps_lds(g.pt_max_out_rows, g.pt_max_in_rows, gram).total;
@@ -1174,6 +1194,9 @@
                                   : (pad ? &edge_block_ps_kernel<true, false, true> : &edge_block_ps_kernel<false, false, true>))
                      : (pair_rows ? (pad ? &edge_block_ps_kernel<true, true, false> : &edge_block_ps_kernel<false, true, false>)
                                   : (pad ? &edge_block_ps_kernel<true, false, false> : &edge_block_ps_kernel<false, false, false>));
+#if RN_PS_LG8
+  if (c2_rows) kern = pad ? &edge_block_ps_kernel<true, true, false, true, true> : &edge_block_ps_kernel<false, true, false, true, true>;
+#endif
   (void)hipFuncSetAttribute(reinterpret_cast<const void *>(kern), hipFuncAttributeMaxDynamicSharedMemorySize, (int)lds);
   static int cus = 0;
   if (cus == 0) {
diff --git a/ramannoodle_amd/pmodel/potgnn.py b/ramannoodle_amd/pmodel/potgnn.py
--- a/ramannoodle_amd/pmodel/potgnn.py
+++ b/ramannoodle_amd/pmodel/potgnn.py
@@ -927,7 +927,7 @@
                 "split_f16_mfma": bool(flags & 4), "narrow_kernels": bool(flags & 8),
                 "mfma_range_fallback": bool(flags & 16),
                 "role_split_edge_block": bool(flags & 256), "atom_owning_node_block": bool(flags & 512),
-                "split_f16_pair_rows": bool(flags & 1024)}
+                "split_f16_pair_rows": bool(flags & 1024), "c2_per_atom_pair": bool(flags & 2048)}
 
     def set_profiling(self, mode: int) -> None:
         self._profiling = int(mode)
```

Result: faster. 60780, median of 6 (+2.6%).
